# Wells-Group/pmg-dolfinx

Measured on AMD Instinct MI355X. Metric: DoFs/sec per p-MG V-cycle (Poisson, hex, p=4), higher is better.
Workload: dtype f64; 1 GPU; Poisson p=4 V-cycle p=4->2->1, Chebyshev(3)/Jacobi, 64^3 hexes per GPU; fine_dofs_global=16974593, partition=1x1x1 bricks, 1 ghost-cell layer, exchange=none (single rank), rccl_ranks=1, comm_ranks=1

## Files before the change

include/pmg_amd.h:

```cpp
#ifndef PMG_AMD_H
#define PMG_AMD_H

#include <stddef.h>
#include <stdint.h>

#ifdef __cplusplus
extern "C" {
#endif

#define PMG_OK 0
#define PMG_ERR_INVALID -1
#define PMG_ERR_HIP -2
#define PMG_ERR_NUMERIC -3
#define PMG_MAX_DEGREE 8

typedef void* pmg_stream;

typedef struct pmg_layout_s* pmg_layout;
typedef struct pmg_comm_s* pmg_comm;
typedef struct pmg_laplacian_s* pmg_laplacian;
typedef struct pmg_chebyshev_s* pmg_chebyshev;
typedef struct pmg_cg_s* pmg_cg;
typedef struct pmg_interpolator_s* pmg_interpolator;
typedef struct pmg_multigrid_s* pmg_multigrid;
// ... 23 lines not shown
int pmg_layout_create(pmg_layout* out, int32_t size_local, int32_t num_ghosts, int32_t n_send,
                      const int32_t* send_indices, double* send_buffer, int32_t n_recv,
                      const int32_t* recv_indices, double* recv_buffer, pmg_exchange_fn exchange,
                      pmg_allreduce_fn allreduce_sum, void* user);
int pmg_layout_destroy(pmg_layout l);
int32_t pmg_layout_size_local(pmg_layout l);
int32_t pmg_layout_num_ghosts(pmg_layout l);
int pmg_layout_set_allreduce_max(pmg_layout l, pmg_allreduce_fn allreduce_max);

#define PMG_COMM_ID_BYTES 128
int pmg_comm_unique_id(char* id );
int pmg_comm_create(pmg_comm* out, int rank, int nranks, const char* id);
int pmg_comm_destroy(pmg_comm comm);
int pmg_comm_capture_overlaps(void);
int pmg_comm_allgather(pmg_comm comm, const void* send, size_t bytes, void* recv);
int pmg_comm_allreduce_sum(pmg_comm comm, double* values, int n, pmg_stream stream);
int pmg_comm_rank(pmg_comm comm);
int pmg_comm_size(pmg_comm comm);
int pmg_layout_set_comm(pmg_layout l, pmg_comm comm, int32_t n_neighbors, const int32_t* neighbor_ranks,
                        const int32_t* send_counts, const int32_t* recv_counts);

#define PMG_WINDOW_HANDLE_BYTES 64
#define PMG_WINDOW_MAX_NEIGHBORS 64
#define PMG_WINDOW_FLAG_WORDS (4 * PMG_WINDOW_MAX_NEIGHBORS + 8)
#define PMG_WINDOW_ERR_NO_ARRIVAL 1
#define PMG_WINDOW_ERR_SLOT_BUSY 2
int pmg_window_alloc(size_t bytes, void** ptr, char* handle );
int pmg_window_fine_grained(void);
int pmg_window_open(const char* handle, void** ptr);
int pmg_window_close(void* ptr);
int pmg_window_free(void* ptr);
#define PMG_COMM_WINDOW_MAX_RANKS 16
#define PMG_COMM_WINDOW_CHUNK 16384
#define PMG_COMM_WINDOW_BYTES \
  (8 * (2 * PMG_COMM_WINDOW_MAX_RANKS + 8 + 2 * PMG_COMM_WINDOW_MAX_RANKS * PMG_COMM_WINDOW_CHUNK))
int pmg_comm_create_windows(pmg_comm* out, int rank, int nranks, void* const* windows );
int pmg_layout_window_describe(int32_t n_neighbors, const int32_t* send_counts, const int32_t* recv_counts,
                               int64_t* window_doubles, int64_t* fwd_offsets, int64_t* rev_offsets);
int pmg_layout_set_windows(pmg_layout l, int32_t n_neighbors, const int32_t* send_counts, const int32_t* recv_counts,
                           double* window, uint64_t* flags, double* const* nb_window, uint64_t* const* nb_flags,
                           const int64_t* nb_window_doubles, const int64_t* nb_fwd_offset, const int64_t* nb_rev_offset,
                           const int32_t* nb_slot);

int pmg_scatter_fwd_begin(pmg_layout l, const double* x, pmg_stream stream);
long long pmg_layout_forward_scatters(pmg_layout l);
int pmg_scatter_fwd_end(pmg_layout l, double* x, pmg_stream stream);
int pmg_scatter_rev_begin(pmg_layout l, const double* x, pmg_stream stream);
int pmg_scatter_rev_end(pmg_layout l, double* x, pmg_stream stream);

int pmg_vec_set(pmg_layout l, double* x, double value, pmg_stream stream);
int pmg_vec_scale(pmg_layout l, double* x, double alpha, pmg_stream stream);
int pmg_vec_copy(pmg_layout l, double* dst, const double* src, pmg_stream stream);
int pmg_vec_axpy(pmg_layout l, double* r, double alpha, const double* x, const double* y,
                 pmg_stream stream);
int pmg_vec_pointwise_mult(pmg_layout l, double* w, const double* x, const double* y,
                           pmg_stream stream);
int pmg_vec_inner_product(pmg_layout l, const double* a, const double* b, double* result,
                          pmg_stream stream);
int pmg_vec_squared_norm(pmg_layout l, const double* a, double* result, pmg_stream stream);
int pmg_vec_norm(pmg_layout l, const double* a, int norm_type, double* result, pmg_stream stream);

int pmg_laplacian_create(pmg_laplacian* out, pmg_layout layout, int degree, int32_t ncells,
                         const double* kappa, const int32_t* dofmap, const double* xgeom,
                         int32_t npoints, const int32_t* geom_dofmap, const int32_t* lcells,
                         int32_t n_lcells, const int32_t* bcells, int32_t n_bcells,
                         const int8_t* bc_marker, pmg_stream stream);
int pmg_laplacian_create_with_tables(pmg_laplacian* out, pmg_layout layout, int degree,
                                     int32_t ncells, const double* kappa, const int32_t* dofmap,
                                     const double* xgeom, int32_t npoints,
                                     const int32_t* geom_dofmap, const double* dphi_geometry,
                                     const double* G_weights, const int32_t* lcells,
                                     int32_t n_lcells, const int32_t* bcells, int32_t n_bcells,
                                     const int8_t* bc_marker, pmg_stream stream);
int pmg_laplacian_create_ordered(pmg_laplacian* out, pmg_layout layout, int degree, int32_t ncells,
                                 const double* kappa, const int32_t* dofmap, const double* xgeom, int32_t npoints,
                                 const int32_t* geom_dofmap, const double* dphi_geometry, const double* G_weights,
                                 const int32_t* lcells, int32_t n_lcells, const int32_t* bcells, int32_t n_bcells,
                                 const int8_t* bc_marker, int node_order, const int32_t* custom_perm1d,
                                 pmg_stream stream);
int pmg_laplacian_node_order(pmg_laplacian op);
int pmg_laplacian_destroy(pmg_laplacian op);
int pmg_laplacian_apply(pmg_laplacian op, double* in, double* out, pmg_stream stream);
int pmg_laplacian_apply_f32(pmg_laplacian op, float* in, float* out, pmg_stream stream);
int pmg_laplacian_get_diag_inverse(pmg_laplacian op, double* diag_inv, pmg_stream stream);
int pmg_laplacian_set_diag_inverse(pmg_laplacian op, const double* diag_inv, pmg_stream stream);
int pmg_laplacian_compute_diag_inverse(pmg_laplacian op, pmg_stream stream);
int pmg_laplacian_get_geometry(pmg_laplacian op, double* G_out, pmg_stream stream);
int pmg_laplacian_set_coefficient_field(pmg_laplacian op, const double* kq, pmg_stream stream);
int pmg_laplacian_has_coefficient_field(pmg_laplacian op);
int pmg_laplacian_set_coefficient_tensor(pmg_laplacian op, const double* kt, pmg_stream stream);
int pmg_laplacian_has_coefficient_tensor(pmg_laplacian op);
int pmg_laplacian_set_reaction(pmg_laplacian op, const double* sigma, pmg_stream stream);
int pmg_laplacian_has_reaction(pmg_laplacian op);
int pmg_laplacian_assemble_rhs(pmg_laplacian op, const double* f, double* b, pmg_stream stream);
int pmg_laplacian_apply_lifting(pmg_laplacian op, double* g, const double* x0, double alpha, double* b, pmg_stream stream);
int pmg_laplacian_set_bc(pmg_laplacian op, const double* g, const double* x0, double alpha, double* b, pmg_stream stream);
int pmg_laplacian_assemble_neumann(pmg_laplacian op, int32_t nfacets, const int32_t* facet_cells,
                                   const int8_t* facet_local, const double* h, double* b, pmg_stream stream);
int pmg_laplacian_lift_cell_count(pmg_laplacian op);
int pmg_laplacian_degree(pmg_laplacian op);
int pmg_laplacian_is_affine(pmg_laplacian op);
int pmg_laplacian_set_geometry_mode(pmg_laplacian op, int mode);
int pmg_laplacian_set_geometry_batch(pmg_laplacian op, long long batch_cells);
long long pmg_laplacian_geometry_bytes(pmg_laplacian op);
int pmg_laplacian_launches_per_apply(pmg_laplacian op);
int pmg_laplacian_apply_streams(pmg_laplacian op);
int pmg_laplacian_chain_available(pmg_laplacian op);
int pmg_laplacian_chain_form(pmg_laplacian op);
int pmg_laplacian_set_chain_form(pmg_laplacian op, int on);
int pmg_set_merge_threshold(long long patch_dofs);
int pmg_laplacian_time_kernel(pmg_laplacian op, const double* in, double* out, int reps,
                              double* ms_per_launch, pmg_stream stream);

int pmg_laplacian_set_profiling(pmg_laplacian op, int flag);
int pmg_laplacian_read_profile(pmg_laplacian op, double* total_ms, long long* launches);

int pmg_chebyshev_create(pmg_chebyshev* out, pmg_layout layout, double eig_min, double eig_max);
int pmg_chebyshev_destroy(pmg_chebyshev s);
int pmg_chebyshev_set_max_iterations(pmg_chebyshev s, int max_iter);
int pmg_chebyshev_solve(pmg_chebyshev s, pmg_laplacian A, double* x, const double* b,
                        pmg_stream stream);

int pmg_cg_create(pmg_cg* out, pmg_layout layout);
int pmg_cg_destroy(pmg_cg s);
int pmg_cg_set_max_iterations(pmg_cg s, int max_iter);
int pmg_cg_set_tolerance(pmg_cg s, double rtol);
int pmg_cg_store_coefficients(pmg_cg s, int flag);
int pmg_cg_solve(pmg_cg s, pmg_laplacian A, double* x, const double* b, pmg_multigrid precond,
                 int* iterations, pmg_stream stream);
int pmg_cg_set_flexible(pmg_cg s, int flag);
int pmg_cg_coefficients(pmg_cg s, double* alphas, double* betas, int capacity);
int pmg_cg_compute_eigenvalues(pmg_cg s, double* eigs, int capacity);
int pmg_cg_residual(pmg_cg s, double* rnorm);

int pmg_matrix_create_from_laplacian(pmg_matrix* out, pmg_laplacian op, pmg_stream stream);
int pmg_matrix_destroy(pmg_matrix M);
int pmg_matrix_update_values(pmg_matrix M, pmg_stream stream);
int pmg_matrix_apply(pmg_matrix M, const double* in, double* out, pmg_stream stream);
int pmg_matrix_get_diag_inverse(pmg_matrix M, double* diag_inv, pmg_stream stream);
long long pmg_matrix_rows(pmg_matrix M);
long long pmg_matrix_nnz(pmg_matrix M);
long long pmg_matrix_bytes(pmg_matrix M);
int pmg_matrix_frobenius_norm(pmg_matrix M, double* norm);
int pmg_matrix_export(pmg_matrix M, long long* rows, long long* nnz, int32_t* row_ptr, int32_t* cols, double* values);
int pmg_chebyshev_solve_matrix(pmg_chebyshev s, pmg_matrix M, double* x, const double* b, pmg_stream stream);
int pmg_cg_solve_matrix(pmg_cg s, pmg_matrix M, double* x, const double* b, pmg_multigrid precond, int* iterations,
                        pmg_stream stream);

int pmg_interpolator_create(pmg_interpolator* out, pmg_layout layout_coarse,
                            pmg_layout layout_fine, int degree_coarse, int degree_fine,
                            int32_t ncells, const int32_t* dofmap_coarse,
                            const int32_t* dofmap_fine, const int32_t* lcells, int32_t n_lcells,
                            const int32_t* bcells, int32_t n_bcells, pmg_stream stream);
int pmg_interpolator_create_with_operator(pmg_interpolator* out, pmg_layout layout_coarse,
                                          pmg_layout layout_fine, int degree_coarse,
                                          int degree_fine, int32_t ncells,
                                          const int32_t* dofmap_coarse, const int32_t* dofmap_fine,
                                          const int32_t* lcells, int32_t n_lcells,
                                          const int32_t* bcells, int32_t n_bcells,
                                          pmg_laplacian fine_operator, pmg_stream stream);
int pmg_interpolator_create_ordered(pmg_interpolator* out, pmg_layout layout_coarse, pmg_layout layout_fine,
                                    int degree_coarse, int degree_fine, int32_t ncells,
                                    const int32_t* dofmap_coarse, const int32_t* dofmap_fine,
                                    const int32_t* lcells, int32_t n_lcells, const int32_t* bcells,
                                    int32_t n_bcells, pmg_laplacian fine_operator, int node_order,
                                    const int32_t* custom_coarse, const int32_t* custom_fine, pmg_stream stream);
int pmg_interpolator_destroy(pmg_interpolator ip);
int pmg_interpolator_interpolate(pmg_interpolator ip, double* coarse, double* fine,
                                 pmg_stream stream);
int pmg_interpolator_interpolate_add(pmg_interpolator ip, double* coarse, double* fine,
                                     pmg_stream stream);
int pmg_interpolator_reverse_interpolate(pmg_interpolator ip, double* fine, double* coarse,
                                         pmg_stream stream);
int pmg_interpolator_restrict_residual(pmg_interpolator ip, pmg_laplacian op, const double* z, const double* r,
                                       double* coarse, pmg_stream stream);
int pmg_interpolator_interpolate_add_f32(pmg_interpolator ip, const float* coarse, float* fine, pmg_stream stream);
int pmg_interpolator_reverse_interpolate_f32(pmg_interpolator ip, const float* fine, const float* fine_sub,
                                             float* coarse, pmg_stream stream);

int pmg_multigrid_create(pmg_multigrid* out, int nlevels, const pmg_layout* layouts,
                         const int8_t* bc_marker_coarsest);
int pmg_multigrid_destroy(pmg_multigrid mg);
int pmg_multigrid_set_operators(pmg_multigrid mg, const pmg_laplacian* ops);
int pmg_multigrid_set_solvers(pmg_multigrid mg, const pmg_chebyshev* smoothers);
int pmg_multigrid_set_interpolators(pmg_multigrid mg, const pmg_interpolator* interp);
int pmg_multigrid_set_coarse_solver(pmg_multigrid mg, pmg_cg coarse);
typedef int (*pmg_coarse_solve_fn)(void* user, double* x, double* b, pmg_stream stream);
int pmg_multigrid_set_coarse_callback(pmg_multigrid mg, pmg_coarse_solve_fn solve, void* user);
int pmg_amg_create(pmg_amg* out, pmg_laplacian op, pmg_stream stream);
int pmg_amg_create_replicated(pmg_amg* out, pmg_laplacian op, const int64_t* global_index, int64_t n_global,
                              pmg_stream stream);
int pmg_amg_create_distributed(pmg_amg* out, pmg_laplacian op, const int64_t* global_index, int64_t n_global,
                               pmg_stream stream);
int pmg_amg_destroy(pmg_amg amg);
int pmg_amg_set_smoother_iterations(pmg_amg amg, int k);
int pmg_amg_set_cycles(pmg_amg amg, int cycles);
int pmg_amg_set_krylov(pmg_amg amg, int max_iter, double rtol);
int pmg_amg_set_distributed_fine_level(pmg_amg amg, int enable);
int pmg_amg_solve(pmg_amg amg, double* x, const double* b, int* iterations, pmg_stream stream);
int pmg_amg_cycle(pmg_amg amg, double* x, const double* b, pmg_stream stream);
int pmg_amg_num_levels(pmg_amg amg);
int pmg_amg_level_info(pmg_amg amg, int level, long long* rows, long long* nnz, double* lambda_max);
int pmg_amg_export(pmg_amg amg, int level, int which, long long* rows, long long* cols, long long* nnz,
                   int32_t* rowptr, int32_t* colidx, double* values);
int pmg_multigrid_set_coarse_amg(pmg_multigrid mg, pmg_amg amg);

int pmg_multigrid_apply(pmg_multigrid mg, const double* rhs, double* y, double* rnorm,
                        pmg_stream stream);
int pmg_multigrid_set_graph(pmg_multigrid mg, int enable);
long long pmg_multigrid_graph_replays(pmg_multigrid mg);
int pmg_multigrid_apply_counts(pmg_multigrid mg, int* counts, int capacity);
int pmg_multigrid_set_fused_restriction(pmg_multigrid mg, int mode);
int pmg_multigrid_fused_restrictions(pmg_multigrid mg);
#define PMG_PRECISION_FP64 0
#define PMG_PRECISION_FP32 1
int pmg_multigrid_set_precision(pmg_multigrid mg, int precision);
int pmg_multigrid_set_level_matrix(pmg_multigrid mg, int level, pmg_matrix M);
int pmg_multigrid_precision(pmg_multigrid mg);

#ifdef __cplusplus
}
#endif
#endif
```

pmg-dolfinx_amd/_lib.py:

```python
from __future__ import annotations

import ctypes as C
import os

_HERE = os.path.dirname(os.path.abspath(__file__))
LIB_PATH = os.environ.get("PMG_AMD_LIB") or os.path.join(_HERE, "lib", "libpmg_amd.so")

c_dp = C.POINTER(C.c_double)
c_ip = C.POINTER(C.c_int32)
c_bp = C.POINTER(C.c_int8)
c_lp = C.POINTER(C.c_int64)
vp = C.c_void_p

EXCHANGE_FN = C.CFUNCTYPE(C.c_int, vp, C.c_int, vp)
ALLREDUCE_FN = C.CFUNCTYPE(C.c_int, vp, c_dp, C.c_int)
COARSE_FN = C.CFUNCTYPE(C.c_int, vp, vp, vp, vp)


class PmgError(RuntimeError):
    """A pmg_* call returned non-zero; the message is ``pmg_last_error()``."""


_SIGS = {
    "pmg_last_error": (C.c_char_p, []),
# ... 91 lines not shown
    "pmg_set_merge_threshold": (C.c_int, [C.c_longlong]),
    "pmg_laplacian_set_profiling": (C.c_int, [vp, C.c_int]),
    "pmg_laplacian_read_profile": (C.c_int, [vp, c_dp, C.POINTER(C.c_longlong)]),
    "pmg_laplacian_time_kernel": (C.c_int, [vp, vp, vp, C.c_int, c_dp, vp]),
    "pmg_chebyshev_create": (C.c_int, [C.POINTER(vp), vp, C.c_double, C.c_double]),
    "pmg_chebyshev_destroy": (C.c_int, [vp]),
    "pmg_chebyshev_set_max_iterations": (C.c_int, [vp, C.c_int]),
    "pmg_chebyshev_solve": (C.c_int, [vp, vp, vp, vp, vp]),
    "pmg_cg_create": (C.c_int, [C.POINTER(vp), vp]),
    "pmg_cg_destroy": (C.c_int, [vp]),
    "pmg_cg_set_max_iterations": (C.c_int, [vp, C.c_int]),
    "pmg_cg_set_tolerance": (C.c_int, [vp, C.c_double]),
    "pmg_cg_store_coefficients": (C.c_int, [vp, C.c_int]),
    "pmg_cg_set_flexible": (C.c_int, [vp, C.c_int]),
    "pmg_cg_solve": (C.c_int, [vp, vp, vp, vp, vp, C.POINTER(C.c_int), vp]),
    "pmg_cg_coefficients": (C.c_int, [vp, c_dp, c_dp, C.c_int]),
    "pmg_cg_compute_eigenvalues": (C.c_int, [vp, c_dp, C.c_int]),
    "pmg_cg_residual": (C.c_int, [vp, c_dp]),
    "pmg_interpolator_create": (
        C.c_int,
        [C.POINTER(vp), vp, vp, C.c_int, C.c_int, C.c_int32, vp, vp, c_ip, C.c_int32, c_ip, C.c_int32, vp],
    ),
    "pmg_interpolator_create_with_operator": (
        C.c_int,
        [C.POINTER(vp), vp, vp, C.c_int, C.c_int, C.c_int32, vp, vp, c_ip, C.c_int32, c_ip, C.c_int32, vp, vp],
    ),
    "pmg_interpolator_create_ordered": (
        C.c_int,
        [C.POINTER(vp), vp, vp, C.c_int, C.c_int, C.c_int32, vp, vp, c_ip, C.c_int32, c_ip, C.c_int32, vp, C.c_int,
         c_ip, c_ip, vp],
    ),
    "pmg_interpolator_interpolate_add": (C.c_int, [vp, vp, vp, vp]),
    "pmg_interpolator_destroy": (C.c_int, [vp]),
    "pmg_interpolator_interpolate": (C.c_int, [vp, vp, vp, vp]),
    "pmg_interpolator_reverse_interpolate": (C.c_int, [vp, vp, vp, vp]),
    "pmg_interpolator_restrict_residual": (C.c_int, [vp, vp, vp, vp, vp, vp]),
    "pmg_interpolator_interpolate_add_f32": (C.c_int, [vp, vp, vp, vp]),
    "pmg_interpolator_reverse_interpolate_f32": (C.c_int, [vp, vp, vp, vp, vp]),
    "pmg_multigrid_create": (C.c_int, [C.POINTER(vp), C.c_int, C.POINTER(vp), vp]),
    "pmg_multigrid_destroy": (C.c_int, [vp]),
    "pmg_multigrid_set_operators": (C.c_int, [vp, C.POINTER(vp)]),
    "pmg_multigrid_set_solvers": (C.c_int, [vp, C.POINTER(vp)]),
    "pmg_multigrid_set_interpolators": (C.c_int, [vp, C.POINTER(vp)]),
    "pmg_multigrid_set_coarse_solver": (C.c_int, [vp, vp]),
    "pmg_multigrid_set_coarse_callback": (C.c_int, [vp, COARSE_FN, vp]),
    "pmg_multigrid_set_coarse_amg": (C.c_int, [vp, vp]),
    "pmg_multigrid_set_precision": (C.c_int, [vp, C.c_int]),
    "pmg_multigrid_precision": (C.c_int, [vp]),
    "pmg_amg_create": (C.c_int, [C.POINTER(vp), vp, vp]),
    "pmg_amg_create_replicated": (C.c_int, [C.POINTER(vp), vp, C.POINTER(C.c_int64), C.c_int64, vp]),
    "pmg_amg_create_distributed": (C.c_int, [C.POINTER(vp), vp, C.POINTER(C.c_int64), C.c_int64, vp]),
    "pmg_amg_destroy": (C.c_int, [vp]),
    "pmg_amg_set_smoother_iterations": (C.c_int, [vp, C.c_int]),
    "pmg_amg_set_cycles": (C.c_int, [vp, C.c_int]),
    "pmg_amg_set_krylov": (C.c_int, [vp, C.c_int, C.c_double]),
    "pmg_amg_set_distributed_fine_level": (C.c_int, [vp, C.c_int]),
    "pmg_amg_solve": (C.c_int, [vp, vp, vp, C.POINTER(C.c_int), vp]),
    "pmg_amg_cycle": (C.c_int, [vp, vp, vp, vp]),
    "pmg_amg_num_levels": (C.c_int, [vp]),
    "pmg_amg_level_info": (C.c_int, [vp, C.c_int, C.POINTER(C.c_longlong), C.POINTER(C.c_longlong), c_dp]),
    "pmg_amg_export": (C.c_int, [vp, C.c_int, C.c_int, C.POINTER(C.c_longlong), C.POINTER(C.c_longlong),
                                 C.POINTER(C.c_longlong), c_ip, c_ip, c_dp]),
    "pmg_laplacian_set_geometry_batch": (C.c_int, [vp, C.c_longlong]),
    "pmg_laplacian_geometry_bytes": (C.c_longlong, [vp]),
    "pmg_multigrid_apply": (C.c_int, [vp, vp, vp, c_dp, vp]),
    "pmg_multigrid_apply_counts": (C.c_int, [vp, C.POINTER(C.c_int), C.c_int]),
    "pmg_multigrid_set_graph": (C.c_int, [vp, C.c_int]),
    "pmg_multigrid_graph_replays": (C.c_longlong, [vp]),
    "pmg_multigrid_set_fused_restriction": (C.c_int, [vp, C.c_int]),
    "pmg_multigrid_fused_restrictions": (C.c_int, [vp]),
    "pmg_matrix_create_from_laplacian": (C.c_int, [C.POINTER(vp), vp, vp]),
    "pmg_matrix_destroy": (C.c_int, [vp]),
    "pmg_matrix_update_values": (C.c_int, [vp, vp]),
    "pmg_matrix_apply": (C.c_int, [vp, vp, vp, vp]),
    "pmg_matrix_get_diag_inverse": (C.c_int, [vp, vp, vp]),
    "pmg_matrix_rows": (C.c_longlong, [vp]),
    "pmg_matrix_nnz": (C.c_longlong, [vp]),
    "pmg_matrix_bytes": (C.c_longlong, [vp]),
    "pmg_matrix_frobenius_norm": (C.c_int, [vp, c_dp]),
    "pmg_matrix_export": (C.c_int, [vp, C.POINTER(C.c_longlong), C.POINTER(C.c_longlong), c_ip, c_ip, c_dp]),
    "pmg_chebyshev_solve_matrix": (C.c_int, [vp, vp, vp, vp, vp]),
    "pmg_cg_solve_matrix": (C.c_int, [vp, vp, vp, vp, vp, C.POINTER(C.c_int), vp]),
    "pmg_multigrid_set_level_matrix": (C.c_int, [vp, C.c_int, vp]),
}

_COUNT_FUNCS = {"pmg_multigrid_graph_replays", "pmg_amg_num_levels", "pmg_laplacian_geometry_bytes", "pmg_comm_rank", "pmg_comm_size", "pmg_comm_capture_overlaps", "pmg_cg_coefficients", "pmg_cg_compute_eigenvalues", "pmg_multigrid_apply_counts", "pmg_version",
                "pmg_laplacian_degree", "pmg_multigrid_precision", "pmg_laplacian_launches_per_apply", "pmg_laplacian_apply_streams", "pmg_laplacian_is_affine",
                "pmg_laplacian_has_coefficient_field", "pmg_laplacian_has_coefficient_tensor", "pmg_laplacian_has_reaction", "pmg_laplacian_lift_cell_count",
                "pmg_laplacian_chain_available", "pmg_laplacian_chain_form",
                "pmg_laplacian_node_order", "pmg_layout_forward_scatters",
                "pmg_matrix_rows", "pmg_matrix_nnz", "pmg_matrix_bytes", "pmg_multigrid_fused_restrictions"}

_lib = None


def exported_symbols():
    return sorted(_SIGS)


def lib():
    global _lib
    if _lib is None:
        if not os.path.exists(LIB_PATH):
            raise RuntimeError(
                f"{LIB_PATH} is missing: the HIP library has not been built. "
                "Run `python -c 'import __graft_entry__ as g; g.build()'` at the repo root. "
                "There is no CPU fallback."
            )
        import torch

        L = C.CDLL(LIB_PATH)
        for name, (res, args) in _SIGS.items():
            if os.environ.get("PMG_AMD_LIB_ALLOW_MISSING") and not hasattr(L, name):
                continue
            f = getattr(L, name)
            f.restype = res
            f.argtypes = args
        _lib = L
    return _lib


def check(rc: int, what: str = ""):
    if rc != 0:
        msg = lib().pmg_last_error().decode("utf-8", "replace")
        raise PmgError(f"{what}: {msg} (code {rc})" if what else f"{msg} (code {rc})")


def call(name: str, *args):
    rc = getattr(lib(), name)(*args)
    if name in _COUNT_FUNCS:
        if rc < 0:
            check(rc, name)
        return rc
    check(rc, name)
    return rc


def ptr(t):
    if t is None:
        return vp(0)
    if hasattr(t, "data_ptr"):
        return vp(t.data_ptr())
    return vp(t.ctypes.data)


def current_stream():
    import torch

    return vp(torch.cuda.current_stream().cuda_stream)
```

pmg-dolfinx_amd/chebyshev.py:

```python
from __future__ import annotations

import ctypes as C

from . import _lib
from ._lib import call, current_stream, ptr, vp
from .vector import Layout, Vector


class Chebyshev:
    def __init__(self, layout: Layout, eig_range, bs: int = 1):
        self.layout = layout
        self.eig_range = (float(eig_range[0]), float(eig_range[1]))
        h = vp()
        call("pmg_chebyshev_create", C.byref(h), layout.handle, self.eig_range[0], self.eig_range[1])
        self._handle = h

    @property
    def handle(self):
        return self._handle

    def set_max_iterations(self, max_iter: int):
        call("pmg_chebyshev_set_max_iterations", self._handle, int(max_iter))

    def solve(self, A, x: Vector, b: Vector, verbose: bool = False):
        from .matrix import MatrixOperator

        fn = "pmg_chebyshev_solve_matrix" if isinstance(A, MatrixOperator) else "pmg_chebyshev_solve"
        call(fn, self._handle, A.handle, ptr(x.data), ptr(b.data), current_stream())

    def __del__(self):
        try:
            if getattr(self, "_handle", None) is not None:
                _lib.lib().pmg_chebyshev_destroy(self._handle)
                self._handle = None
        except Exception:
            pass
```

pmg-dolfinx_amd/csrc/common.hpp:

```cpp
#pragma once

#include "../../include/pmg_amd.h"

#include <hip/hip_runtime.h>

#include <cstdarg>
#include <cstdio>
#include <functional>
#include <string>
#include <type_traits>
#include <vector>

namespace pmg
{
extern thread_local std::string g_last_error;

int fail(int code, const char* fmt, ...);

#define PMG_HIP(call)                                                                              \
  do                                                                                               \
  {                                                                                                \
    hipError_t e_ = (call);                                                                        \
    if (e_ != hipSuccess)                                                                          \
      return pmg::fail(PMG_ERR_HIP, "%s failed: %s (%s:%d)", #call, hipGetErrorString(e_),         \
// ... 102 lines not shown
  hipStream_t stream = nullptr;
  hipEvent_t ev_in = nullptr, ev_out = nullptr;
  bool reduced_eagerly = false;
};

struct pmg_layout_s
{
  int32_t size_local = 0, num_ghosts = 0, n_send = 0, n_recv = 0;
  pmg_comm_s* comm = nullptr;
  std::vector<int32_t> nb_rank, nb_send, nb_recv;
  hipEvent_t ev_packed = nullptr, ev_arrived = nullptr;
  double *c_send = nullptr, *c_recv = nullptr;
  int32_t *send_pos = nullptr, *recv_pos = nullptr;
  std::vector<size_t> send_off, recv_off;
  pmg_window_s* win = nullptr;
  bool exchange_inline = false;
  bool exchanged_eagerly = false;
  const int32_t* send_idx = nullptr;
  const int32_t* recv_idx = nullptr;
  double* send_buf = nullptr;
  double* recv_buf = nullptr;
  pmg_exchange_fn exchange = nullptr;
  pmg_allreduce_fn allreduce = nullptr;
  pmg_allreduce_fn allreduce_max = nullptr;
  void* user = nullptr;
  double* d_partials = nullptr;
  double* h_result = nullptr;
  long long fwd_scatters = 0;
  bool multi_rank() const { return comm != nullptr || allreduce != nullptr; }
  int32_t total() const { return size_local + num_ghosts; }
};

namespace pmg
{
constexpr int RED_BLOCKS = 1024;
constexpr int RED_THREADS = 256;
constexpr int RED_SLOTS = 8;

int comm_exchange_begin(pmg_layout l, bool reverse, hipStream_t s);
int comm_exchange_end(pmg_layout l, hipStream_t s);
int comm_allreduce(pmg_layout l, double* d_values, int n, bool max, hipStream_t s);
int comm_allreduce(pmg_comm c, double* d_values, int n, bool max, hipStream_t s);
bool comm_capture_ready(pmg_layout l, bool with_allreduce);

int window_exchange_begin(pmg_layout l, bool reverse, const double* x, hipStream_t s);
int window_exchange_end(pmg_layout l, bool reverse, double* x, hipStream_t s);
int window_exchange_whole(pmg_layout l, double* x, hipStream_t s);
int scatter_fwd_whole(pmg_layout l, double* x, hipStream_t s);
bool layout_exchanges_whole(pmg_layout l);
void window_destroy(pmg_layout l);
int wcomm_allreduce(pmg_comm c, double* d_values, int n, bool max, hipStream_t s);
int wcomm_allgather(pmg_comm c, const void* send, size_t bytes, void* recv);
void wcomm_destroy(pmg_comm c);

void range_push(const char* name);
void range_pop();
struct Range
{
  explicit Range(const char* name) { range_push(name); }
  Range(const Range&) = delete;
  Range& operator=(const Range&) = delete;
  ~Range() { range_pop(); }
};

template <typename T>
struct ChebWork
{
  T *r = nullptr, *z = nullptr, *q = nullptr;
};
template <typename T>
using ApplyFnT = std::function<int(T* in, T* out)>;
using ApplyFn = ApplyFnT<double>;
using PrecondFn = std::function<int(double* z, const double* r)>;
int cg_iterate(pmg_cg cg, const ApplyFn& A, const double* dinv, const PrecondFn* M, bool flexible, double* x,
               const double* b, int* iterations, hipStream_t s);
enum : int
{
  ResidualNone = 0,
  ResidualUpdated = 1,
  ResidualSplit = 2,
  ResidualFused = 3
};
template <typename T>
int cheb_iterate(const ChebWork<T>& w, const ApplyFnT<T>& A, const T* dinv, int n, double lmax, int max_iter, T* x,
                 const T* b, int need_r, bool x_zero, hipStream_t s, bool* split = nullptr,
                 const ApplyFnT<T>* A_zeroed = nullptr, int n_total = 0, bool track_ghosts = false,
                 const ApplyFnT<T>* A_first = nullptr);

int dot_async(pmg_layout l, const double* a, const double* b, int slot, hipStream_t s);
double* red_slot(pmg_layout l, int slot);
int reduce_slots_async(pmg_layout l, int slot, int n, bool max, hipStream_t s);
int fetch_slots(pmg_layout l, int slot, int n, double* host_out, hipStream_t s);
int dot_host(pmg_layout l, const double* a, const double* b, double* result, hipStream_t s);
void launch_axpy(int n, double* r, double alpha, const double* x, const double* y, hipStream_t s);
void launch_pointwise(int n, double* w, const double* x, const double* y, hipStream_t s);
void launch_cheb_init(int n, double* r, double* z, const double* b, const double* q, const double* dinv, double c0,
                      hipStream_t s, double* clear_q = nullptr, int n_total = 0);
void launch_cheb_step(int n, double* x, double* r, double* z, const double* q, const double* dinv, double c1, double c2,
                      bool both, int x_final, hipStream_t s, double* clear_q = nullptr, int n_total = 0);
void launch_cheb_first(int n, double* x, double* r, double* z, const double* q, const double* dinv, double c1,
                       double c2, int x_final, hipStream_t s, double* clear_q = nullptr, int n_total = 0);
void launch_cheb_residual(int n, double* r, const double* q, hipStream_t s);
void launch_add(int n, double* x, const double* z, hipStream_t s);
void launch_cheb_last(int n, double* x, double* r, const double* z, const double* q, bool assign, hipStream_t s);
void launch_zero(int n, double* x, hipStream_t s);
void launch_mask_bc(int n, double* b, const int8_t* bc, hipStream_t s);
void launch_cheb_init(int n, float* r, float* z, const float* b, const float* q, const float* dinv, float c0,
                      hipStream_t s, float* clear_q = nullptr, int n_total = 0);
void launch_cheb_step(int n, float* x, float* r, float* z, const float* q, const float* dinv, float c1, float c2,
                      bool both, int x_final, hipStream_t s, float* clear_q = nullptr, int n_total = 0);
void launch_cheb_first(int n, float* x, float* r, float* z, const float* q, const float* dinv, float c1,
                       float c2, int x_final, hipStream_t s, float* clear_q = nullptr, int n_total = 0);
void launch_cheb_residual(int n, float* r, const float* q, hipStream_t s);
void launch_add(int n, float* x, const float* z, hipStream_t s);
void launch_cheb_last(int n, float* x, float* r, const float* z, const float* q, bool assign, hipStream_t s);
void launch_zero(int n, float* x, hipStream_t s);
void launch_mask_bc(int n, float* b, const int8_t* bc, hipStream_t s);
void launch_cg_update(int n, double* x, double* r, double* y, const double* p, const double* dinv,
                      double rnorm, const double* d_py, hipStream_t s);
void launch_cg_update2(int n, double* x, double* r, const double* p, const double* y, double rnorm,
                       const double* d_py, hipStream_t s);
void launch_cg_direction(int n, double* p, const double* y, double rnorm, const double* d_new,
                         const double* d_sub, hipStream_t s);

int laplacian_apply(pmg_laplacian op, double* in, double* out, hipStream_t s);
int laplacian_apply_zeroed(pmg_laplacian op, double* in, double* out, hipStream_t s);
int laplacian_apply_ghosts_current(pmg_laplacian op, double* in, double* out, hipStream_t s);
bool laplacian_wants_zeroed_output(pmg_laplacian op);
const double* laplacian_diag_inv(pmg_laplacian op);
const double* laplacian_reaction(pmg_laplacian op);
pmg_layout laplacian_layout(pmg_laplacian op);
long long laplacian_launches(pmg_laplacian op);
long long laplacian_capture_state(pmg_laplacian op);
int laplacian_geometry_ascending(pmg_laplacian op, double* G_out, hipStream_t s);
struct LaplacianInputs
{
  int degree;
  int32_t ncells;
  const int32_t* dofmap;
  const int8_t* bc;
  const double* kappa;
};
LaplacianInputs laplacian_inputs(pmg_laplacian op);
int interp_prolong(pmg_interpolator ip, double* coarse, double* fine, hipStream_t s);
int interp_restrict(pmg_interpolator ip, double* fine, double* coarse, hipStream_t s);
int interp_prolong_add(pmg_interpolator ip, double* coarse, double* fine, hipStream_t s);
bool interp_is_patched(pmg_interpolator ip);
bool interp_restricts_difference(pmg_interpolator ip);
int interp_restrict_difference(pmg_interpolator ip, double* fine, const double* fine_sub, double* coarse,
                               hipStream_t s);
bool interp_fuses_residual(pmg_interpolator ip, pmg_laplacian op);
int interp_restrict_residual(pmg_interpolator ip, pmg_laplacian op, const double* z, const double* r, double* coarse,
                             hipStream_t s);
int amg_solve(pmg_amg amg, double* x, const double* b, hipStream_t s);
pmg_layout amg_layout(pmg_amg amg);
long long amg_capture_state(pmg_amg amg);
int matrix_apply(pmg_matrix M, const double* in, double* out, hipStream_t s);
const double* matrix_diag_inv(pmg_matrix M);
pmg_layout matrix_layout(pmg_matrix M);

int laplacian_f32_supported(pmg_laplacian op, const char* who);
int laplacian_f32_prepare(pmg_laplacian op, hipStream_t s);
int laplacian_f32_reaction(pmg_laplacian op, hipStream_t s);
int laplacian_f32_refresh(pmg_laplacian op, hipStream_t s);
int laplacian_f32_diag(pmg_laplacian op, const float** d, hipStream_t s, bool* changed);
long long laplacian_diag_version(pmg_laplacian op);
int laplacian_apply_f32(pmg_laplacian op, const float* in, float* out, hipStream_t s);
int transfer_f32_prepare(pmg_interpolator ip, const float** M1);
int prolong_add_f32(pmg_interpolator ip, const float* M1, const float* coarse, float* fine, hipStream_t s);
int restrict_f32(pmg_interpolator ip, const float* M1, const float* fine, const float* fine_sub, float* coarse,
                 hipStream_t s);
void launch_to_f32(int n, const double* in, const double* sub, float* out, hipStream_t s);
void launch_from_f32(int n, const float* in, double* out, bool add, hipStream_t s);
}
```

pmg-dolfinx_amd/csrc/laplacian.hip:

```cpp
#include "laplacian.hpp"
#include "stiffness_layer.hpp"

#include <algorithm>
#include <cmath>
#include <cstdlib>
#include <type_traits>

using namespace pmg;


namespace
{
#include "geometry_kernels.hpp"
#include "stiffness_column.hpp"
#include "stiffness_chain.hpp"
#include "stiffness_restrict.hpp"

__global__ void zero_list_kernel(int n, const int32_t* __restrict__ idx, double* __restrict__ y)
{
  for (int i = blockIdx.x * blockDim.x + threadIdx.x; i < n; i += gridDim.x * blockDim.x)
    y[idx[i]] = 0.0;
}

const double2* batch_geometry(pmg_laplacian op, int first, int count, hipStream_t s)
{
  double2* base = op->G - (size_t)first * gpatch(op->nd, op->K);
  const long long nslots = (long long)count * op->K, n = nslots * op->N;
  if (n > 0)
    geometry_kernel<<<(unsigned)((n + 255) / 256), 256, 0, s>>>((long long)first * op->K, nslots, op->nd, op->K,
                                                              op->pcell, op->xgeom, op->geom_dofmap,
                                                              op->dphi_geom, op->gweights, op->kfield, op->dofmap,
                                                              op->ktensor, base);
  return base;
}

template <typename F>
int for_each_geometry_chunk(pmg_laplacian op, hipStream_t s, F f)
{
  if (op->npatch == 0)
    return PMG_OK;
  if (op->batch_patches <= 0)
    f(0, op->npatch, op->G);
  else
    for (int first = 0; first < op->npatch; first += op->batch_patches)
    {
      const int count = std::min(op->batch_patches, op->npatch - first);
      f(first, count, batch_geometry(op, first, count, s));
    }
  PMG_HIP(hipGetLastError());
  return PMG_OK;
}

template <int P, bool AFFINE_NT, typename F>
void apply_variant(pmg_laplacian op, F launch)
{
  if (op->geometry_mode == 1)
    launch(std::true_type{}, std::bool_constant<AFFINE_NT>{});
  else if (P >= NT_FROM && op->stream_policy)
    launch(std::false_type{}, std::true_type{});
  else
    launch(std::false_type{}, std::false_type{});
}

template <int P>
int launch_stiffness(pmg_laplacian op, const double* x, double* y, int first, int count,
                     int atomic_out, hipStream_t s)
{
  if (count <= 0)
    return PMG_OK;
  if (op->batch_patches > 0 && op->geometry_mode == 0 && count > op->batch_patches)
  {
    for (int f = first; f < first + count; f += op->batch_patches)
      PMG_TRY(launch_stiffness<P>(op, x, y, f, std::min(op->batch_patches, first + count - f), atomic_out, s));
    return PMG_OK;
  }
  const double2* G = op->G;
  if (op->batch_patches > 0 && op->geometry_mode == 0)
    G = batch_geometry(op, first, count, s);
  apply_variant<P, (P >= NT_FROM)>(op, [&](auto aff, auto nt) {
    constexpr bool AFF = decltype(aff)::value, NT = decltype(nt)::value;
    stiffness_column_kernel<P, AFF, NT><<<count, Shape<P>::WTHREADS, 0, s>>>(
        x, y, G, op->Gaff, op->W1, op->poff, op->pdofs, op->lmap_id, op->lmaps, op->pcell, op->pncell, op->kappa, op->D,
        op->react, first, atomic_out);
  });
  op->launches++;
  return PMG_OK;
}

static int launch_chains(pmg_laplacian op, const double* x, double* y, int first, int count, hipStream_t s)
{
  if constexpr (chain_form(4))
  {
    if (op->P != 4)
      return fail(PMG_ERR_INVALID, "internal: chain form at degree %d", op->P);
    auto launch = [&](auto nt) {
      stiffness_chain_kernel<4, decltype(nt)::value><<<count, ChainShape<4>::THREADS, 0, s>>>(
          x, y, op->G, op->poff, op->cdofs, op->ccar, op->lmap_id, op->lmaps, op->pcell, op->pncell, op->kappa, op->D,
          op->chain_off, op->chain_patch, first);
    };
    op->stream_policy ? launch(std::true_type{}) : launch(std::false_type{});
    op->launches++;
  }
  return PMG_OK;
}

ApplyForm apply_form(pmg_laplacian op)
{
  const bool resident = op->batch_patches == 0;
  return {resident && !op->launch_stream.empty(),
          resident && op->chain_on && op->geometry_mode == 0 && !op->react, resident};
}

int run_launches(pmg_laplacian op, const double* x, double* y, int l0, int l1, hipStream_t s)
{
  return walk_launches(op, l0, l1, apply_form(op), s, [&](const LaunchStep& st, hipStream_t sl) {
    if (st.kind == LaunchStep::CHAINS)
      return launch_chains(op, x, y, st.first, st.count, sl);
    return with_degree(op->P, [&](auto P) {
      return launch_stiffness<decltype(P)::value>(op, x, y, st.first, st.count, st.atomic_out, sl);
    });
  });
}

#define PMG_FOR_FUSED_PAIRS(X) X(2, 1) X(4, 2) X(3, 1) X(6, 3)

template <int P, int PC>
int launch_stiffness_restrict(pmg_laplacian op, const TransferView& tv, const double* z, const double* r,
                              double* coarse, hipStream_t s)
{
  constexpr int cm = RestrictShape<P, PC>::CM;
  PMG_REQUIRE(tv.cmax_m <= cm, "internal: a patch holds %d coarse dofs, the fused kernel %d", tv.cmax_m, cm);
  const RestrictLists R{tv.cpoff, tv.clmap_id, tv.cpdofs, tv.clmaps, tv.pmult, tv.M1};
  apply_variant<P, false>(op, [&](auto aff, auto nt) {
    constexpr bool AFF = decltype(aff)::value, NT = decltype(nt)::value;
    stiffness_restrict_kernel<P, PC, AFF, NT><<<op->npatch, Shape<P>::WTHREADS, 0, s>>>(
        z, r, coarse, op->G, op->Gaff, op->W1, op->poff, op->pdofs, op->lmap_id, op->lmaps, op->pcell, op->pncell,
        op->kappa, op->D, op->react, R);
  });
  PMG_HIP(hipGetLastError());
  return PMG_OK;
}

}

namespace pmg
{
bool streams_past_the_cache(long long tensor_bytes)
{
  if (const char* e = std::getenv("PMG_STREAM_POLICY"))
    return e[0] != '0';
  return tensor_bytes > (128LL << 20);
}

bool laplacian_fuses_restriction(pmg_laplacian op, int coarse_degree)
{
  if (op->layout->num_ghosts != 0 || op->batch_patches != 0)
    return false;
#define X(F, C)                                                                                                      \
  if (op->P == F && coarse_degree == C)                                                                              \
    return true;
  PMG_FOR_FUSED_PAIRS(X)
#undef X
  return false;
}

int laplacian_apply_restrict(pmg_laplacian op, const TransferView& tv, const double* z, const double* r,
                             double* coarse, hipStream_t s)
{
  PMG_REQUIRE(laplacian_fuses_restriction(op, tv.ndc - 1) && tv.ndf == op->nd && tv.fv.pdofs == op->pdofs
// ... 26 lines not shown
  const long long field = op->batch_patches > 0 ? (op->kfield_epoch & 0x3fff) << 44 : 0;
  return ((long long)op->geometry_mode << 40) ^ ((long long)op->batch_patches << 8) ^ (long long)(op->have_diag ? 1 : 0)
         ^ (long long)(op->chain_on ? 2 : 0) ^ (long long)(op->react ? 4 : 0) ^ field;
}

PatchView laplacian_patches(pmg_laplacian op)
{
  PatchView v;
  v.P = op->P;
  v.K = op->K;
  v.N = op->N;
  v.npatch = op->npatch;
  v.max_m = op->max_m;
  v.pcell_h = &op->pcell_h;
  v.pncell_h = &op->pncell_h;
  v.launch_first = &op->launch_first;
  v.launch_count = &op->launch_count;
  v.n_launch_l = op->n_launch_l;
  v.merged = op->n_plain == 0;
  v.pcell = op->pcell;
  v.pncell = op->pncell;
  v.poff = op->poff;
  v.pdofs = op->pdofs;
  v.lmap_id = op->lmap_id;
  v.lmaps = op->lmaps;
  v.npdofs = op->npdofs;
  return v;
}

bool laplacian_wants_zeroed_output(pmg_laplacian op)
{
  return zero_fills_output(op->needs_zero, op->launch_first.size(), op->n_bzero, op->layout->total());
}

bool laplacian_single_launch(pmg_laplacian op)
{
  if (op->launch_first.size() != 2)
    return false;
  int steps = 0, all = 0;
  for_each_launch_step(*op, op->chain_first, op->chain_count, 0, 2, apply_form(op), [&](const LaunchStep& st) {
    steps += st.launches();
    all += st.kind == LaunchStep::PATCHES && st.atomic_out && st.count == op->npatch;
    return PMG_OK;
  });
  return steps == 1 && all == 1 && layout_exchanges_whole(op->layout);
}

static int apply_impl(pmg_laplacian op, double* in, double* out, bool out_is_zero, hipStream_t s,
                      bool exchange = true)
{
  pmg_layout l = op->layout;
  const int nl = (int)op->launch_first.size();
  const bool zero_all = laplacian_wants_zeroed_output(op);
  if (zero_all && !out_is_zero)
    launch_zero(l->total(), out, s);
  if (op->n_bzero > 0 && !zero_all)
    zero_list_kernel<<<(op->n_bzero + 255) / 256 > 1024 ? 1024 : (op->n_bzero + 255) / 256, 256, 0, s>>>(
        op->n_bzero, op->bzero, out);
  if (laplacian_single_launch(op))
  {
    if (exchange)
      PMG_TRY(scatter_fwd_whole(l, in, s));
    PMG_TRY(run_launches(op, in, out, 0, nl, s));
    op->applies++;
    return PMG_OK;
  }
  if (exchange)
    PMG_TRY(pmg_scatter_fwd_begin(l, in, (pmg_stream)s));
  PMG_TRY(run_launches(op, in, out, 0, op->n_launch_l, s));
  if (exchange)
    PMG_TRY(pmg_scatter_fwd_end(l, in, (pmg_stream)s));
  PMG_TRY(run_launches(op, in, out, op->n_launch_l, nl, s));
  op->applies++;
  return PMG_OK;
}
int laplacian_apply(pmg_laplacian op, double* in, double* out, hipStream_t s) { return apply_impl(op, in, out, false, s); }
int laplacian_apply_ghosts_current(pmg_laplacian op, double* in, double* out, hipStream_t s)
{
  return apply_impl(op, in, out, false, s, false);
}
int laplacian_apply_zeroed(pmg_laplacian op, double* in, double* out, hipStream_t s)
{
  return apply_impl(op, in, out, laplacian_wants_zeroed_output(op), s);
}
}

extern "C" int pmg_laplacian_create_ordered(
    pmg_laplacian* out, pmg_layout layout, int degree, int32_t ncells, const double* kappa,
    const int32_t* dofmap, const double* xgeom, int32_t npoints, const int32_t* geom_dofmap,
    const double* dphi_geometry, const double* G_weights, const int32_t* lcells, int32_t n_lcells,
    const int32_t* bcells, int32_t n_bcells, const int8_t* bc_marker, int node_order, const int32_t* custom_perm1d,
    pmg_stream stream)
{
  PMG_REQUIRE(out && layout, "pmg_laplacian_create: NULL handle");
  if (degree < 1 || degree > PMG_MAX_DEGREE)
    return fail(PMG_ERR_INVALID, "Unsupported degree");
  PMG_REQUIRE(ncells >= 0 && n_lcells >= 0 && n_bcells >= 0 && n_lcells + n_bcells <= ncells,
              "pmg_laplacian_create: cell lists (%d + %d) exceed ncells (%d)", n_lcells, n_bcells,
              ncells);
  PMG_REQUIRE(ncells == 0 || (kappa && dofmap && xgeom && geom_dofmap && bc_marker),
              "pmg_laplacian_create: NULL array");
  PMG_REQUIRE((n_lcells == 0 || lcells) && (n_bcells == 0 || bcells),
              "pmg_laplacian_create: NULL cell list");
  PMG_REQUIRE(npoints >= 0, "pmg_laplacian_create: negative npoints");
  {
    std::vector<char> seen(ncells, 0);
    for (int set = 0; set < 2; ++set)
    {
      const int32_t* list = set ? bcells : lcells;
      const int n = set ? n_bcells : n_lcells;
      for (int i = 0; i < n; ++i)
      {
        PMG_REQUIRE(list[i] >= 0 && list[i] < ncells,
                    "pmg_laplacian_create: cell list entry %d out of range", list[i]);
        PMG_REQUIRE(!seen[list[i]], "pmg_laplacian_create: cell %d listed twice", list[i]);
        seen[list[i]] = 1;
      }
    }
  }

  hipStream_t s = S(stream);
  auto* op = new pmg_laplacian_s;
  HandleGuard<pmg_laplacian> guard(op, pmg_laplacian_destroy);
  op->layout = layout;
  op->P = degree;
  op->nd = degree + 1;
  op->N = op->nd * op->nd * op->nd;
  op->K = patch_shape(degree).K();
  {
    const int kk[9] = {0, Shape<1>::K, Shape<2>::K, Shape<3>::K, Shape<4>::K, Shape<5>::K,
                       Shape<6>::K, Shape<7>::K, Shape<8>::K};
    PMG_REQUIRE(kk[degree] == op->K, "internal: patch shape / kernel shape mismatch");
  }
  op->ncells = ncells;
  op->npoints = npoints;
  op->kappa = kappa;
  op->dofmap = dofmap;
  op->xgeom = xgeom;
  op->geom_dofmap = geom_dofmap;
  op->bc = bc_marker;
  const int nd = op->nd, N = op->N;
  const int total = layout->total();

  std::vector<int32_t> perm1d;
  PMG_TRY(node_permutation(node_order, degree, custom_perm1d, perm1d));
  op->node_order = node_order;
  if (!is_identity(perm1d))
  {
    const std::vector<int32_t> p3 = cell_permutation(nd, perm1d);
    PMG_TRY(upload(&op->qperm, p3.data(), p3.size(), s));
    PMG_HIP(hipMalloc(&op->dofmap_own, sizeof(int32_t) * ((size_t)ncells * N ? (size_t)ncells * N : 1)));
    PMG_TRY(permute_rows_i32(ncells, N, op->qperm, dofmap, op->dofmap_own, s));
    PMG_HIP(hipStreamSynchronize(s));
    op->dofmap = dofmap = op->dofmap_own;
  }

  std::vector<double> pts(nd), wts(nd), D(nd * nd);
  gll_table(nd, pts.data(), wts.data());
  lagrange_derivative_table(nd, pts.data(), D.data());
  PMG_TRY(upload(&op->D, D.data(), D.size(), s));

  if (dphi_geometry && G_weights)
  {
    PMG_HIP(hipMalloc(&op->dphi_geom, sizeof(double) * 24 * N));
    PMG_HIP(hipMalloc(&op->gweights, sizeof(double) * N));
    if (op->qperm)
// ... 23 lines not shown
            for (int j = 0; j < 2; ++j)
              for (int k = 0; k < 2; ++k)
              {
                int v = i * 4 + j * 2 + k;
                dphi[((size_t)0 * N + q) * 8 + v] = dp[i] * ph[1][j] * ph[2][k];
                dphi[((size_t)1 * N + q) * 8 + v] = ph[0][i] * dp[j] * ph[2][k];
                dphi[((size_t)2 * N + q) * 8 + v] = ph[0][i] * ph[1][j] * dp[k];
              }
        }
    PMG_TRY(upload(&op->dphi_geom, dphi.data(), dphi.size(), s));
    PMG_TRY(upload(&op->gweights, w3.data(), w3.size(), s));
    PMG_HIP(hipStreamSynchronize(s));
  }

  PatchPlan plan;
  ChainPlan cplan;
  {
    std::vector<int32_t> h_dofmap((size_t)ncells * N), h_gd((size_t)ncells * 8);
    std::vector<int8_t> h_bc(total);
    std::vector<double> h_x((size_t)npoints * 3);
    PMG_HIP(hipMemcpyAsync(h_dofmap.data(), dofmap, sizeof(int32_t) * h_dofmap.size(),
                           hipMemcpyDeviceToHost, s));
    PMG_HIP(hipMemcpyAsync(h_gd.data(), geom_dofmap, sizeof(int32_t) * h_gd.size(),
                           hipMemcpyDeviceToHost, s));
    PMG_HIP(hipMemcpyAsync(h_bc.data(), bc_marker, sizeof(int8_t) * h_bc.size(),
                           hipMemcpyDeviceToHost, s));
    PMG_HIP(hipMemcpyAsync(h_x.data(), xgeom, sizeof(double) * h_x.size(), hipMemcpyDeviceToHost, s));
    PMG_HIP(hipStreamSynchronize(s));
    std::vector<float> centroid((size_t)ncells * 3);
    for (int32_t c = 0; c < ncells; ++c)
      for (int a = 0; a < 3; ++a)
      {
        double v = 0;
        for (int k = 0; k < 8; ++k)
        {
          int32_t g = h_gd[(size_t)c * 8 + k];
          PMG_REQUIRE(g >= 0 && g < npoints, "pmg_laplacian_create: geometry dofmap entry %d out of range", g);
          v += h_x[3 * (size_t)g + a];
        }
        centroid[(size_t)c * 3 + a] = (float)(v * 0.125);
      }
    PMG_TRY(build_patch_plan(plan, degree, ncells, h_dofmap.data(), h_bc.data(), total,
                             centroid.data(), lcells, n_lcells, bcells, n_bcells));
    op->all_affine = (n_lcells + n_bcells) > 0;
    for (int set = 0; set < 2 && op->all_affine; ++set)
    {
      const int32_t* list = set ? bcells : lcells;
      const int n = set ? n_bcells : n_lcells;
      for (int i = 0; i < n && op->all_affine; ++i)
      {
        const int32_t* gd = h_gd.data() + (size_t)list[i] * 8;
        const double* v[8];
        for (int k = 0; k < 8; ++k)
          v[k] = h_x.data() + 3 * (size_t)gd[k];
        double diam = 0, dev = 0;
        for (int a = 0; a < 3; ++a)
        {
          const double e1 = v[4][a] - v[0][a], e2 = v[2][a] - v[0][a], e3 = v[1][a] - v[0][a];
          diam += std::fabs(e1) + std::fabs(e2) + std::fabs(e3);
          dev += std::fabs(v[3][a] - (v[0][a] + e2 + e3)) + std::fabs(v[5][a] - (v[0][a] + e1 + e3))
                 + std::fabs(v[6][a] - (v[0][a] + e1 + e2)) + std::fabs(v[7][a] - (v[0][a] + e1 + e2 + e3));
        }
        if (dev > 1e-12 * diam)
          op->all_affine = false;
      }
    }
    if (chain_form(degree) && (unsigned long long)plan.npatch * (unsigned long long)gpatch(nd, op->K) < (1ull << 32))
    {
      const char* e = std::getenv("PMG_CHAIN");
      const int mode = e ? std::atoi(e) : 0;
      if (mode > 0)
      {
        int dev = 0, cus = 256;
        if (hipGetDevice(&dev) == hipSuccess)
          (void)hipDeviceGetAttribute(&cus, hipDeviceAttributeMultiprocessorCount, dev);
        PMG_TRY(build_chain_plan(cplan, plan, total, h_bc.data(), centroid.data(), mode >= 2 ? 1 : (cus * 3) / 4));
      }
    }
    std::vector<char> touched(total, 0);
    for (uint32_t v : plan.pdofs)
      touched[v & PD_MASK] = 1;
    for (int i = 0; i < total && !op->needs_zero; ++i)
      op->needs_zero = !touched[i];
  }
  op->npatch = plan.npatch;
  op->pcell_h = plan.pcell;
  op->pncell_h = plan.pncell;
  op->npdofs = (long long)plan.pdofs.size();
  op->max_m = plan.max_M;
  op->launch_first = plan.launch_first;
  op->launch_count = plan.launch_count;
  op->n_launch_l = plan.n_launch_l;
  op->n_plain = plan.n_plain;
  op->launch_stream = plan.launch_stream;
  op->launch_signal = plan.launch_signal;
  op->launch_wait = plan.launch_wait;
  if (!op->launch_stream.empty())
  {
    PMG_HIP(hipStreamCreateWithFlags(&op->stream2, hipStreamNonBlocking));
    PMG_HIP(hipEventCreateWithFlags(&op->ev_fork, hipEventDisableTiming));
    PMG_HIP(hipEventCreateWithFlags(&op->ev_order, hipEventDisableTiming));
    PMG_HIP(hipEventCreateWithFlags(&op->ev_join, hipEventDisableTiming));
  }
  PMG_TRY(upload(&op->pcell, plan.pcell.data(), plan.pcell.size(), s));
  PMG_TRY(upload(&op->pncell, plan.pncell.data(), plan.pncell.size(), s));
  op->n_bzero = (int32_t)plan.bzero.size();
  PMG_TRY(upload(&op->bzero, plan.bzero.data(), plan.bzero.size(), s));
  PMG_TRY(upload(&op->poff, plan.poff.data(), plan.poff.size(), s));
  PMG_TRY(upload(&op->pdofs, plan.pdofs.data(), plan.pdofs.size(), s));
  PMG_TRY(upload(&op->lmap_id, plan.lmap_id.data(), plan.lmap_id.size(), s));
  PMG_TRY(upload(&op->lmaps, plan.lmaps.data(), plan.lmaps.size(), s));
  if (cplan.ok)
  {
    PMG_TRY(upload(&op->cdofs, cplan.cdofs.data(), cplan.cdofs.size(), s));
    PMG_TRY(upload(&op->ccar, cplan.ccar.data(), cplan.ccar.size(), s));
    PMG_TRY(upload(&op->chain_off, cplan.chain_off.data(), cplan.chain_off.size(), s));
    PMG_TRY(upload(&op->chain_patch, cplan.chain_patch.data(), cplan.chain_patch.size(), s));
    op->chain_first = cplan.launch_first;
    op->chain_count = cplan.launch_count;
    op->chain_ok = op->chain_on = true;
  }

  const long long nslots = (long long)plan.npatch * op->K;
  const long long nq_total = nslots * N;
  PMG_TRY(upload(&op->W1, wts.data(), wts.size(), s));
  PMG_HIP(hipMalloc(&op->Gaff, sizeof(double) * 6 * (nslots ? nslots : 1)));
  if (nslots > 0)
    affine_geometry_kernel<<<(unsigned)((nslots + 255) / 256), 256, 0, s>>>(nslots, op->pcell, xgeom,
                                                                           geom_dofmap, nullptr, op->Gaff);
  {
    const size_t gsize = (size_t)op->npatch * gpatch(nd, op->K);
    PMG_HIP(hipMalloc(&op->G, sizeof(double2) * (gsize ? gsize : 1)));
    PMG_HIP(hipMemsetAsync(op->G, 0, sizeof(double2) * (gsize ? gsize : 1), s));
  }
  op->stream_policy = streams_past_the_cache((long long)sizeof(double2) * gpatch(nd, op->K) * op->npatch);
  PMG_HIP(hipMalloc(&op->diag_inv, sizeof(double) * (total ? total : 1)));
  PMG_HIP(hipEventCreate(&op->ev0));
  PMG_HIP(hipEventCreate(&op->ev1));
  if (nq_total > 0)
  {
    batch_geometry(op, 0, op->npatch, s);
    PMG_HIP(hipGetLastError());
  }
  PMG_HIP(hipStreamSynchronize(s));
  *out = guard.release();
  return PMG_OK;
}

extern "C" int pmg_laplacian_create_with_tables(
    pmg_laplacian* out, pmg_layout layout, int degree, int32_t ncells, const double* kappa,
    const int32_t* dofmap, const double* xgeom, int32_t npoints, const int32_t* geom_dofmap,
    const double* dphi_geometry, const double* G_weights, const int32_t* lcells, int32_t n_lcells,
    const int32_t* bcells, int32_t n_bcells, const int8_t* bc_marker, pmg_stream stream)
{
  return pmg_laplacian_create_ordered(out, layout, degree, ncells, kappa, dofmap, xgeom, npoints, geom_dofmap,
                                      dphi_geometry, G_weights, lcells, n_lcells, bcells, n_bcells, bc_marker,
                                      PMG_NODES_ASCENDING, nullptr, stream);
}

extern "C" int pmg_laplacian_node_order(pmg_laplacian op) { return op ? op->node_order : -1; }

extern "C" int pmg_laplacian_create(pmg_laplacian* out, pmg_layout layout, int degree,
                                    int32_t ncells, const double* kappa, const int32_t* dofmap,
                                    const double* xgeom, int32_t npoints,
                                    const int32_t* geom_dofmap, const int32_t* lcells,
                                    int32_t n_lcells, const int32_t* bcells, int32_t n_bcells,
                                    const int8_t* bc_marker, pmg_stream stream)
{
  return pmg_laplacian_create_with_tables(out, layout, degree, ncells, kappa, dofmap, xgeom,
                                          npoints, geom_dofmap, nullptr, nullptr, lcells, n_lcells,
                                          bcells, n_bcells, bc_marker, stream);
}

extern "C" int pmg_laplacian_destroy(pmg_laplacian op)
{
  if (!op)
    return PMG_OK;
  (void)hipFree(op->G);
  (void)hipFree(op->dofmap_own);
  (void)hipFree(op->qperm);
  (void)hipFree(op->D);
  (void)hipFree(op->Gaff);
  (void)hipFree(op->kfield);
  (void)hipFree(op->ktensor);
  (void)hipFree(op->react_buf);
  (void)hipFree(op->react32_buf);
  (void)hipFree(op->W1);
  (void)hipFree(op->dphi_geom);
  (void)hipFree(op->gweights);
  (void)hipFree(op->pcell);
  (void)hipFree(op->pncell);
  (void)hipFree(op->bzero);
  (void)hipFree(op->poff);
  (void)hipFree(op->pdofs);
  (void)hipFree(op->lmap_id);
  (void)hipFree(op->lmaps);
  (void)hipFree(op->cdofs);
  (void)hipFree(op->ccar);
  (void)hipFree(op->chain_off);
  (void)hipFree(op->chain_patch);
  (void)hipFree(op->diag_inv);
  (void)hipFree(op->G32);
  (void)hipFree(op->D32);
  (void)hipFree(op->diag32);
  (void)hipFree(op->lift_cells);
  for (hipEvent_t e : op->prof_events)
    (void)hipEventDestroy(e);
  for (hipEvent_t e : {op->ev_fork, op->ev_order, op->ev_join})
    if (e)
      (void)hipEventDestroy(e);
  if (op->stream2)
    (void)hipStreamDestroy(op->stream2);
  if (op->ev0)
    (void)hipEventDestroy(op->ev0);
  if (op->ev1)
    (void)hipEventDestroy(op->ev1);
  delete op;
  return PMG_OK;
}

#ifdef PMG_STAMPS
extern "C" int pmg_debug_set_stamp_buffer(unsigned long long* buffer, int workgroups)
{
  PMG_HIP(hipMemcpyToSymbol(HIP_SYMBOL(g_stamp_buffer), &buffer, sizeof(buffer)));
  PMG_HIP(hipMemcpyToSymbol(HIP_SYMBOL(g_stamp_capacity), &workgroups, sizeof(workgroups)));
  return PMG_OK;
}
#endif

extern "C" int pmg_laplacian_degree(pmg_laplacian op) { return op ? op->P : -1; }

extern "C" int pmg_laplacian_is_affine(pmg_laplacian op) { return op ? (op->all_affine ? 1 : 0) : -1; }

extern "C" int pmg_laplacian_set_geometry_mode(pmg_laplacian op, int mode)
{
  PMG_REQUIRE(op && (mode == 0 || mode == 1), "pmg_laplacian_set_geometry_mode: bad argument");
  if (mode == 1)
  {
    PMG_REQUIRE(op->all_affine, "pmg_laplacian_set_geometry_mode: the mesh has non-affine cells");
    PMG_REQUIRE(!op->kfield, "pmg_laplacian_set_geometry_mode: the affine mode streams one tensor per cell and cannot "
                             "carry the coefficient field (remove it with pmg_laplacian_set_coefficient_field(op, "
                             "NULL, stream) first)");
  }
  op->geometry_mode = mode;
  return PMG_OK;
}

extern "C" int pmg_laplacian_apply(pmg_laplacian op, double* in, double* out, pmg_stream stream)
{
  PMG_REQUIRE(op && in && out, "pmg_laplacian_apply: NULL argument");
  PMG_REQUIRE(in != out, "pmg_laplacian_apply: in and out alias");
  return laplacian_apply(op, in, out, S(stream));
}

extern "C" int pmg_laplacian_get_diag_inverse(pmg_laplacian op, double* diag_inv,
                                              pmg_stream stream)
{
  PMG_REQUIRE(op && diag_inv, "pmg_laplacian_get_diag_inverse: NULL argument");
  PMG_REQUIRE(op->have_diag, "pmg_laplacian_get_diag_inverse: diagonal not set");
  PMG_HIP(hipMemcpyAsync(diag_inv, op->diag_inv, sizeof(double) * op->layout->total(),
                         hipMemcpyDeviceToDevice, S(stream)));
  return PMG_OK;
}

extern "C" int pmg_laplacian_set_diag_inverse(pmg_laplacian op, const double* diag_inv,
                                              pmg_stream stream)
{
  PMG_REQUIRE(op && diag_inv, "pmg_laplacian_set_diag_inverse: NULL argument");
  PMG_HIP(hipMemcpyAsync(op->diag_inv, diag_inv, sizeof(double) * op->layout->total(),
                         hipMemcpyDeviceToDevice, S(stream)));
  op->have_diag = true;
  op->diag_computed = false;
  op->diag_version++;
  return PMG_OK;
}

extern "C" int pmg_laplacian_compute_diag_inverse(pmg_laplacian op, pmg_stream stream)
{
  PMG_REQUIRE(op, "pmg_laplacian_compute_diag_inverse: NULL argument");
  hipStream_t s = S(stream);
  const int total = op->layout->total();
  PMG_HIP(hipMemsetAsync(op->diag_inv, 0, sizeof(double) * total, s));
  PMG_TRY(for_each_geometry_chunk(op, s, [&](int first, int count, const double2* G) {
    const long long nslots = (long long)count * op->K, n = nslots * op->N;
    diagonal_kernel<<<(unsigned)((n + 255) / 256), 256, 0, s>>>((long long)first * op->K, nslots, op->nd, op->K,
                                                              op->pcell, G, op->dofmap, op->bc, op->kappa, op->D,
                                                              op->diag_inv);
  }));
  if (total > 0)
    diag_invert_kernel<<<(total + 255) / 256, 256, 0, s>>>(total, op->bc, op->react, op->diag_inv);
  PMG_HIP(hipGetLastError());
  op->have_diag = true;
  op->diag_computed = true;
  op->diag_version++;
  return PMG_OK;
}

__global__ void coefficient_check_kernel(int n, const double* __restrict__ kq, double* __restrict__ bad)
{
  int mine = 0;
  for (long long i = (long long)blockIdx.x * blockDim.x + threadIdx.x; i < n; i += (long long)gridDim.x * blockDim.x)
  {
    const double v = kq[i];
    mine += !(v > 0.0 && v <= 1.79769313486231570e308);
  }
  if (mine)
    atomicAdd(bad, (double)mine);
}

extern "C" int pmg_laplacian_has_coefficient_field(pmg_laplacian op) { return op ? (op->kfield ? 1 : 0) : -1; }

extern "C" int pmg_laplacian_set_coefficient_field(pmg_laplacian op, const double* kq, pmg_stream stream)
{
  PMG_REQUIRE(op, "pmg_laplacian_set_coefficient_field: NULL argument");
  hipStream_t s = S(stream);
  hipStreamCaptureStatus cap = hipStreamCaptureStatusNone;
  PMG_HIP(hipStreamIsCapturing(s, &cap));
  PMG_REQUIRE(cap == hipStreamCaptureStatusNone,
              "pmg_laplacian_set_coefficient_field: not inside a stream capture (it allocates and synchronises)");
  pmg_layout l = op->layout;
  double* released = nullptr;
  if (!kq)
  {
    if (!op->kfield)
      return PMG_OK;
    released = op->kfield;
    op->kfield = nullptr;
    op->kfield_epoch++;
  }
  else
  {
    PMG_REQUIRE(op->geometry_mode == 0,
                "pmg_laplacian_set_coefficient_field: the affine mode streams one tensor per cell and cannot carry a "
                "field (return to the stored tensor with pmg_laplacian_set_geometry_mode(op, 0) first)");
    double* bad = red_slot(l, 0);
// ... 333 lines not shown
```

pmg-dolfinx_amd/csrc/laplacian.hpp:

```cpp
#pragma once

#include "common.hpp"
#include "patches.hpp"

struct pmg_laplacian_s
{
  pmg_layout layout = nullptr;
  int P = 0, nd = 0, N = 0, K = 0;
  int32_t ncells = 0, npoints = 0;
  const double* kappa = nullptr;
  const int32_t* dofmap = nullptr;
  const double* xgeom = nullptr;
  const int32_t* geom_dofmap = nullptr;
  const int8_t* bc = nullptr;
  int node_order = PMG_NODES_ASCENDING;
  int32_t* dofmap_own = nullptr;
  int32_t* qperm = nullptr;
  double2* G = nullptr;
  double* kfield = nullptr;
  long long kfield_epoch = 0;
  double* ktensor = nullptr;
  double* react = nullptr;
  float* react32 = nullptr;
  double* react_buf = nullptr;
  float* react32_buf = nullptr;
  bool diag_computed = false;
  double* Gaff = nullptr;
  double* W1 = nullptr;
  bool all_affine = false;
  int geometry_mode = 0;
  double* D = nullptr;
  double* dphi_geom = nullptr;
  double* gweights = nullptr;
  int32_t* pcell = nullptr;
  int32_t* pncell = nullptr;
  int32_t* bzero = nullptr;
  int32_t n_bzero = 0;
  int32_t* poff = nullptr;
  uint32_t* pdofs = nullptr;
  int32_t* lmap_id = nullptr;
  uint16_t* lmaps = nullptr;
  int32_t npatch = 0;
  std::vector<int32_t> launch_first, launch_count;
  std::vector<int8_t> launch_stream;
  int launch_signal = -1, launch_wait = -1;
  hipStream_t stream2 = nullptr;
  hipEvent_t ev_fork = nullptr, ev_order = nullptr, ev_join = nullptr;
  std::vector<int32_t> pcell_h, pncell_h;
  long long npdofs = 0;
  int max_m = 0;
  int n_launch_l = 0;
  int n_plain = 0;
  bool needs_zero = false;
  bool chain_ok = false, chain_on = false;
  uint32_t* cdofs = nullptr;
  uint32_t* ccar = nullptr;
  int32_t* chain_off = nullptr;
  int32_t* chain_patch = nullptr;
  std::vector<int32_t> chain_first, chain_count;
  bool stream_policy = true;
  bool stream_policy32 = false;
  double* diag_inv = nullptr;
  bool have_diag = false;
  hipEvent_t ev0 = nullptr, ev1 = nullptr;
  long long launches = 0;
  long long applies = 0;
  int32_t batch_patches = 0;
  bool profiling = false;
  std::vector<hipEvent_t> prof_events;
  size_t prof_used = 0;
  long long prof_launches = 0;
  float2* G32 = nullptr;
  float* D32 = nullptr;
  float* diag32 = nullptr;
  long long diag_version = 0;
  long long diag32_version = -1;
  int32_t* lift_cells = nullptr;
  int32_t n_lift = -1;
  std::vector<char> listed;
};

namespace pmg
{
bool streams_past_the_cache(long long tensor_bytes);

template <typename L>
int walk_launches(pmg_laplacian op, int l0, int l1, ApplyForm form, hipStream_t s, L&& launch)
{
  const bool prof = op->profiling && l1 > l0;
  if (prof)
  {
    while (op->prof_events.size() < op->prof_used + 2)
    {
      hipEvent_t e;
      PMG_HIP(hipEventCreate(&e));
      op->prof_events.push_back(e);
    }
    PMG_HIP(hipEventRecord(op->prof_events[op->prof_used], s));
  }
  int issued = 0;
  PMG_TRY(for_each_launch_step(*op, op->chain_first, op->chain_count, l0, l1, form, [&](const LaunchStep& st) -> int {
    switch (st.kind)
    {
    case LaunchStep::FORK:
      PMG_HIP(hipEventRecord(op->ev_fork, s));
      PMG_HIP(hipStreamWaitEvent(op->stream2, op->ev_fork, 0));
      break;
    case LaunchStep::WAIT_ORDER:
      PMG_HIP(hipStreamWaitEvent(s, op->ev_order, 0));
      break;
    case LaunchStep::RECORD_ORDER:
      PMG_HIP(hipEventRecord(op->ev_order, op->stream2));
      break;
    case LaunchStep::JOIN:
      PMG_HIP(hipEventRecord(op->ev_join, op->stream2));
      PMG_HIP(hipStreamWaitEvent(s, op->ev_join, 0));
      break;
    default:
      PMG_TRY(launch(st, st.stream ? op->stream2 : s));
      ++issued;
    }
    return PMG_OK;
  }));
  PMG_HIP(hipGetLastError());
  if (prof)
  {
    PMG_HIP(hipEventRecord(op->prof_events[op->prof_used + 1], s));
    op->prof_used += 2;
    op->prof_launches += issued;
  }
  return PMG_OK;
}

__device__ inline void jacobian(const double* __restrict__ xgeom,
                                const int32_t* __restrict__ gdofs, const double* __restrict__ dphi,
                                int nq, int q, double K[3][3], double& detJ)
{
  double J[3][3] = {{0, 0, 0}, {0, 0, 0}, {0, 0, 0}};
  for (int k = 0; k < 8; ++k)
  {
    const double* xk = xgeom + 3 * (size_t)gdofs[k];
    double x0 = xk[0], x1 = xk[1], x2 = xk[2];
// ... 43 lines not shown
```

pmg-dolfinx_amd/csrc/solvers.hip:

```cpp
#include "common.hpp"

#include <cstdlib>

#include <algorithm>
#include <cmath>
#include <cstring>

using namespace pmg;

struct pmg_chebyshev_s
{
  pmg_layout layout = nullptr;
  double eig_min = 0, eig_max = 1;
  int max_iter = 1;
  double *r = nullptr, *z = nullptr, *q = nullptr;
};

struct pmg_cg_s
{
  pmg_layout layout = nullptr;
  int max_iter = 0;
  double rtol = 0;
  bool store = false;
  double *r = nullptr, *y = nullptr, *p = nullptr;
  double* zold = nullptr;
  bool flexible = false;
  std::vector<double> alphas, betas, residuals;
};

struct pmg_multigrid_s
{
  int L = 0;
  std::vector<pmg_layout> layouts;
  const int8_t* bc0 = nullptr;
  std::vector<pmg_laplacian> ops;
  std::vector<pmg_chebyshev> smoothers;
  std::vector<pmg_interpolator> interps;
  std::vector<double*> u, b;
  std::vector<int> counts;
  pmg_cg coarse = nullptr;
  pmg_coarse_solve_fn coarse_fn = nullptr;
  void* coarse_user = nullptr;
  pmg_amg coarse_amg = nullptr;
  std::vector<pmg_matrix> mats;
  std::vector<long long> mat_applies;
  struct GraphEntry
  {
    const double* rhs;
    double* y;
    bool y_zero;
    uint64_t config;
    hipGraphExec_t exec;
    std::vector<int> counts;
    int fused_count;
  };
  int graph_mode = -1;
  std::vector<GraphEntry> graphs;
  hipStream_t capture_stream = nullptr;
  long long graph_replays = 0;
  int fused_mode = -1;
  int fused_count = 0;
  int precision = PMG_PRECISION_FP64;
  std::vector<float*> u32, b32;
  std::vector<ChebWork<float>> w32;
  std::vector<const float*> dinv32;
  std::vector<const float*> M1_32;
};

namespace pmg
{
template <typename T>
int cheb_iterate(const ChebWork<T>& w, const ApplyFnT<T>& A, const T* dinv, int n, double lmax, int max_iter, T* x,
                 const T* b, int need_r, bool x_zero, hipStream_t s, bool* split, const ApplyFnT<T>* A_zeroed,
                 int n_total, bool track_ghosts, const ApplyFnT<T>* A_first)
{
  PMG_REQUIRE(sizeof(T) == 8 || !A_zeroed, "cheb_iterate: the FP32 passes have no zeroed-output form");
  if (split)
    *split = false;
  T* const clear_q = A_zeroed ? w.q : nullptr;
  const ApplyFnT<T>& An = A_zeroed ? *A_zeroed : A;
  const T c0 = (T)(4.0 / (3.0 * lmax));
  const int ng = track_ghosts && n_total > n ? n_total - n : 0;
  if (x_zero)
  {
    launch_cheb_init(n, w.r, w.z, b, nullptr, dinv, c0, s, clear_q, n_total);
    if (ng > 0)
      launch_zero(ng, x + n, s);
  }
  else
  {
    PMG_TRY(A_first ? (*A_first)(x, w.q) : A(x, w.q));
    launch_cheb_init(n, w.r, w.z, b, w.q, dinv, c0, s, clear_q, n_total);
  }
  for (int i = 1; i <= max_iter; ++i)
  {
    const bool last = (i == max_iter);
    if (last && !need_r)
    {
      if (max_iter == 1)
      {
        if (x_zero)
          PMG_HIP(hipMemcpyAsync(x, w.z, sizeof(T) * n, hipMemcpyDeviceToDevice, s));
        else
          launch_add(n, x, w.z, s);
      }
      break;
    }
    if (last && need_r == ResidualFused && split && max_iter > 1)
    {
      *split = true;
      break;
    }
    PMG_TRY(An(w.z, w.q));
    if (ng > 0)
      launch_add(ng, x + n, w.z + n, s);
    if (last)
    {
      if (max_iter == 1)
        launch_cheb_last(n, x, w.r, w.z, w.q, x_zero, s);
      else if (need_r == ResidualSplit && split)
        *split = true;
      else
        launch_cheb_residual(n, w.r, w.q, s);
      break;
    }
    const T c1 = (T)((2.0 * i - 1.0) / (2.0 * i + 3.0));
    const T c2 = (T)((8.0 * i + 4.0) / (2.0 * i + 3.0) / lmax);
    const int x_final = (i + 1 == max_iter) ? (need_r == ResidualNone ? 2 : 1) : 0;
    if (x_zero && i == 1)
      launch_cheb_first(n, x, w.r, w.z, w.q, dinv, c1, c2, x_final, s, clear_q, n_total);
    else
      launch_cheb_step(n, x, w.r, w.z, w.q, dinv, c1, c2, i == 1, x_final, s, clear_q, n_total);
  }
  if (max_iter == 0 && x_zero)
    launch_zero(n, x, s);
  PMG_HIP(hipGetLastError());
  return PMG_OK;
}
template int cheb_iterate<double>(const ChebWork<double>&, const ApplyFnT<double>&, const double*, int, double, int,
                                  double*, const double*, int, bool, hipStream_t, bool*, const ApplyFnT<double>*, int,
                                  bool, const ApplyFnT<double>*);
template int cheb_iterate<float>(const ChebWork<float>&, const ApplyFnT<float>&, const float*, int, double, int, float*,
                                 const float*, int, bool, hipStream_t, bool*, const ApplyFnT<float>*, int, bool,
                                 const ApplyFnT<float>*);
}

namespace
{
int mg_apply_graph(pmg_multigrid mg, const double* rhs, double* y, bool y_zero, hipStream_t s, bool* done);
bool use_graph(pmg_multigrid mg);
void drop_graphs(pmg_multigrid mg);

template <typename T>
int alloc_vec(pmg_layout l, T** p)
{
  size_t n = l->total() ? l->total() : 1;
  PMG_HIP(hipMalloc(p, sizeof(T) * n));
  PMG_HIP(hipMemset(*p, 0, sizeof(T) * n));
  PMG_HIP(hipStreamSynchronize(nullptr));
  return PMG_OK;
}

int cheb_solve(pmg_chebyshev sm, pmg_laplacian A, double* x, const double* b, int need_r,
               bool x_zero, hipStream_t s, bool* split = nullptr, bool track_ghosts = false,
               bool x_ghosts_current = false)
{
  pmg_layout l = sm->layout;
  PMG_REQUIRE(laplacian_layout(A) == l, "Chebyshev: operator and smoother layouts differ");
  const ChebWork<double> w{sm->r, sm->z, sm->q};
  const ApplyFn apply = [A, s](double* in, double* out) { return laplacian_apply(A, in, out, s); };
  const ApplyFn apply_zeroed = [A, s](double* in, double* out) { return laplacian_apply_zeroed(A, in, out, s); };
  const ApplyFn apply_local = [A, s](double* in, double* out) { return laplacian_apply_ghosts_current(A, in, out, s); };
  return cheb_iterate(w, apply, laplacian_diag_inv(A), l->size_local, sm->eig_max, sm->max_iter, x, b, need_r, x_zero,
                      s, split, laplacian_wants_zeroed_output(A) ? &apply_zeroed : nullptr, l->total(), track_ghosts,
                      x_ghosts_current ? &apply_local : nullptr);
}

int cheb_solve_matrix(pmg_chebyshev sm, pmg_matrix M, double* x, const double* b, int need_r, bool x_zero,
                      hipStream_t s, bool* split = nullptr, long long* applies = nullptr)
{
  pmg_layout l = sm->layout;
  PMG_REQUIRE(matrix_layout(M) == l, "Chebyshev: matrix and smoother layouts differ");
  const ChebWork<double> w{sm->r, sm->z, sm->q};
  const ApplyFn apply = [M, s, applies](double* in, double* out)
  {
    if (applies)
      ++*applies;
    return matrix_apply(M, in, out, s);
  };
  return cheb_iterate(w, apply, matrix_diag_inv(M), l->size_local, sm->eig_max, sm->max_iter, x, b, need_r, x_zero, s,
                      split);
}

bool fuses_restriction(pmg_multigrid mg, int i)
{
  if (mg->fused_mode == 0 || i <= 0 || mg->mats[i] || !interp_fuses_residual(mg->interps[i - 1], mg->ops[i]))
    return false;
  if (const char* e = std::getenv("PMG_FUSED_DEGREES"))
  {
    const int P = pmg_laplacian_degree(mg->ops[i]);
    for (const char* c = e; *c; ++c)
      if (*c - '0' == P)
        return true;
    return false;
  }
  return true;
}

int level_smooth(pmg_multigrid mg, int i, double* x, const double* b, int need_r, bool x_zero, hipStream_t s,
                 bool* split = nullptr, bool track_ghosts = false, bool x_ghosts_current = false)
{
  if (mg->mats[i])
    return cheb_solve_matrix(mg->smoothers[i], mg->mats[i], x, b, need_r, x_zero, s, split, &mg->mat_applies[i]);
  return cheb_solve(mg->smoothers[i], mg->ops[i], x, b, need_r, x_zero, s, split, track_ghosts, x_ghosts_current);
}

long long level_applies(pmg_multigrid mg, int i) { return laplacian_launches(mg->ops[i]) + mg->mat_applies[i]; }

bool local_correction(pmg_multigrid mg, int level)
{
  if (const char* e = std::getenv("PMG_LOCAL_CORRECTION"))
    if (e[0] == '0')
      return false;
  return level > 0 && mg->layouts[level]->num_ghosts > 0 && interp_is_patched(mg->interps[level - 1]);
}

int mg_check_f32(pmg_multigrid mg, const char* who)
{
  for (int i = 0; i < mg->L; ++i)
  {
    pmg_layout l = mg->layouts[i];
    PMG_REQUIRE(l->num_ghosts == 0 && !l->multi_rank() && !l->win,
                "%s: the FP32 cycle is single-domain only (level %d's layout has ghosts or a communicator)", who, i);
  }
  for (size_t i = 0; i < mg->interps.size(); ++i)
    PMG_REQUIRE(interp_is_patched(mg->interps[i]),
                "%s: the FP32 cycle needs patch-form interpolators (pmg_interpolator_create_with_operator; level %zu)",
                who, i);
  for (pmg_laplacian op : mg->ops)
    PMG_TRY(laplacian_f32_supported(op, who));
  return PMG_OK;
}

void free_f32(pmg_multigrid mg)
{
  for (float* p : mg->u32)
    (void)hipFree(p);
  for (float* p : mg->b32)
    (void)hipFree(p);
  for (const ChebWork<float>& w : mg->w32)
  {
    (void)hipFree(w.r);
    (void)hipFree(w.z);
    (void)hipFree(w.q);
  }
  mg->u32.clear();
  mg->b32.clear();
  mg->w32.clear();
}

int mg_prepare_f32(pmg_multigrid mg, hipStream_t s)
{
  const int L = mg->L;
  PMG_TRY(mg_check_f32(mg, "pmg_multigrid_apply"));
  if ((int)mg->u32.size() != L)
  {
    mg->u32.assign(L, nullptr);
    mg->b32.assign(L, nullptr);
    mg->w32.assign(L, ChebWork<float>{});
    for (int i = 0; i < L; ++i)
    {
      PMG_TRY(alloc_vec(mg->layouts[i], &mg->u32[i]));
      PMG_TRY(alloc_vec(mg->layouts[i], &mg->b32[i]));
      PMG_TRY(alloc_vec(mg->layouts[i], &mg->w32[i].r));
      PMG_TRY(alloc_vec(mg->layouts[i], &mg->w32[i].z));
      PMG_TRY(alloc_vec(mg->layouts[i], &mg->w32[i].q));
    }
  }
  mg->M1_32.assign(L - 1, nullptr);
  for (int i = 0; i < L - 1; ++i)
    PMG_TRY(transfer_f32_prepare(mg->interps[i], &mg->M1_32[i]));
  mg->dinv32.assign(L, nullptr);
  for (int i = 0; i < L; ++i)
  {
    PMG_TRY(laplacian_f32_prepare(mg->ops[i], s));
    PMG_TRY(laplacian_f32_diag(mg->ops[i], &mg->dinv32[i], s, nullptr));
  }
  return PMG_OK;
}

int level_smooth_f32(pmg_multigrid mg, int i, int need_r, bool x_zero, hipStream_t s, bool* split)
{
  pmg_laplacian op = mg->ops[i];
  const ApplyFnT<float> apply = [op, s](float* in, float* out) { return laplacian_apply_f32(op, in, out, s); };
  return cheb_iterate(mg->w32[i], apply, mg->dinv32[i], mg->layouts[i]->size_local, mg->smoothers[i]->eig_max,
                      mg->smoothers[i]->max_iter, mg->u32[i], mg->b32[i], need_r, x_zero, s, split);
}
// ... 110 lines not shown
    }
    else if (split)
      PMG_TRY(interp_restrict_difference(mg->interps[i - 1], mg->smoothers[i]->r, mg->smoothers[i]->q,
                                         mg->b[i - 1], s));
    else
      PMG_TRY(interp_restrict(mg->interps[i - 1], mg->smoothers[i]->r, mg->b[i - 1], s));
  }
  if (L > 1)
    launch_mask_bc(mg->layouts[0]->size_local, mg->b[0], mg->bc0, s);
  {
    Range rg("pmg:coarse_solve");
    const double* b0 = (L == 1) ? rhs : mg->b[0];
    const bool zero = (L == 1) ? y_zero : true;
    if (has_coarse_solver(mg) && L > 1)
      PMG_TRY(coarse_solve(mg, s));
    else
      PMG_TRY(level_smooth(mg, 0, mg->u[0], b0, ResidualNone, zero, s));
  }
  for (int i = 0; i < L - 1; ++i)
  {
    {
      Range rg("pmg:prolong");
      if (interp_is_patched(mg->interps[i]))
        PMG_TRY(interp_prolong_add(mg->interps[i], mg->u[i], mg->u[i + 1], s));
      else
      {
        double* du = mg->smoothers[i + 1]->q;
        PMG_TRY(interp_prolong(mg->interps[i], mg->u[i], du, s));
        launch_add(mg->layouts[i + 1]->size_local, mg->u[i + 1], du, s);
      }
    }
    Range rg("pmg:post_smooth");
    const double* bi = (i + 1 == L - 1) ? rhs : mg->b[i + 1];
    PMG_TRY(level_smooth(mg, i + 1, mg->u[i + 1], bi, ResidualNone, false, s, nullptr, false,
                         local_correction(mg, i + 1)));
  }
  for (int i = 0; i < L; ++i)
    mg->counts[i] = (int)(level_applies(mg, i) - before[i]);
  PMG_HIP(hipGetLastError());
  return PMG_OK;
}
}

extern "C" int pmg_chebyshev_create(pmg_chebyshev* out, pmg_layout layout, double eig_min,
                                    double eig_max)
{
  PMG_REQUIRE(out && layout, "pmg_chebyshev_create: NULL argument");
  PMG_REQUIRE(eig_max > 0.0, "pmg_chebyshev_create: eig_max must be positive");
  auto* sm = new pmg_chebyshev_s;
  HandleGuard<pmg_chebyshev> guard(sm, pmg_chebyshev_destroy);
  sm->layout = layout;
  sm->eig_min = eig_min;
  sm->eig_max = eig_max;
  PMG_TRY(alloc_vec(layout, &sm->r));
  PMG_TRY(alloc_vec(layout, &sm->z));
  PMG_TRY(alloc_vec(layout, &sm->q));
  *out = guard.release();
  return PMG_OK;
}

extern "C" int pmg_chebyshev_destroy(pmg_chebyshev sm)
{
  if (!sm)
    return PMG_OK;
  (void)hipFree(sm->r);
  (void)hipFree(sm->z);
  (void)hipFree(sm->q);
  delete sm;
  return PMG_OK;
}

extern "C" int pmg_chebyshev_set_max_iterations(pmg_chebyshev sm, int max_iter)
{
  PMG_REQUIRE(sm && max_iter >= 0, "pmg_chebyshev_set_max_iterations: bad argument");
  sm->max_iter = max_iter;
  return PMG_OK;
}

extern "C" int pmg_chebyshev_solve(pmg_chebyshev sm, pmg_laplacian A, double* x, const double* b,
                                   pmg_stream stream)
{
  PMG_REQUIRE(sm && A && x && b, "pmg_chebyshev_solve: NULL argument");
  return cheb_solve(sm, A, x, b, ResidualNone, false, S(stream));
}

extern "C" int pmg_chebyshev_solve_matrix(pmg_chebyshev sm, pmg_matrix M, double* x, const double* b,
                                          pmg_stream stream)
{
  PMG_REQUIRE(sm && M && x && b, "pmg_chebyshev_solve_matrix: NULL argument");
  return cheb_solve_matrix(sm, M, x, b, ResidualNone, false, S(stream));
}

extern "C" int pmg_cg_create(pmg_cg* out, pmg_layout layout)
{
  PMG_REQUIRE(out && layout, "pmg_cg_create: NULL argument");
  auto* cg = new pmg_cg_s;
  HandleGuard<pmg_cg> guard(cg, pmg_cg_destroy);
  cg->layout = layout;
  PMG_TRY(alloc_vec(layout, &cg->r));
  PMG_TRY(alloc_vec(layout, &cg->y));
  PMG_TRY(alloc_vec(layout, &cg->p));
  *out = guard.release();
  return PMG_OK;
}

extern "C" int pmg_cg_destroy(pmg_cg cg)
{
  if (!cg)
    return PMG_OK;
  (void)hipFree(cg->r);
  (void)hipFree(cg->y);
  (void)hipFree(cg->p);
  (void)hipFree(cg->zold);
  delete cg;
  return PMG_OK;
}

extern "C" int pmg_cg_set_max_iterations(pmg_cg cg, int max_iter)
{
  PMG_REQUIRE(cg && max_iter >= 0, "pmg_cg_set_max_iterations: bad argument");
  cg->max_iter = max_iter;
  cg->alphas.reserve(max_iter);
  cg->betas.reserve(max_iter);
  cg->residuals.reserve(max_iter);
  return PMG_OK;
}

extern "C" int pmg_cg_set_tolerance(pmg_cg cg, double rtol)
{
  PMG_REQUIRE(cg, "pmg_cg_set_tolerance: NULL argument");
  cg->rtol = rtol;
  return PMG_OK;
}

extern "C" int pmg_cg_store_coefficients(pmg_cg cg, int flag)
{
  PMG_REQUIRE(cg, "pmg_cg_store_coefficients: NULL argument");
  cg->store = flag != 0;
  return PMG_OK;
}

namespace pmg
{
int cg_iterate(pmg_cg cg, const ApplyFn& A, const double* dinv, const PrecondFn* M, bool flexible, double* x,
               const double* b, int* iterations, hipStream_t s)
{
  pmg_layout l = cg->layout;
  const int n = l->size_local;
  double *r = cg->r, *y = cg->y, *p = cg->p;
  const bool precond = M != nullptr;
  auto precondition = [&](double* out_z, const double* in_r) -> int
  {
    if (precond)
      return (*M)(out_z, in_r);
    launch_pointwise(n, out_z, in_r, dinv, s);
    return PMG_OK;
  };
  const bool flex = flexible && precond;
  if (flex && !cg->zold)
    PMG_TRY(alloc_vec(l, &cg->zold));
  PMG_TRY(A(x, y));
  launch_axpy(n, r, -1.0, y, b, s);
  PMG_TRY(precondition(p, r));
  if (flex)
    PMG_HIP(hipMemcpyAsync(cg->zold, p, sizeof(double) * n, hipMemcpyDeviceToDevice, s));
  double rnorm0;
// ... 248 lines not shown
  mg->smoothers.assign(smoothers, smoothers + mg->L);
  return PMG_OK;
}

extern "C" int pmg_multigrid_set_interpolators(pmg_multigrid mg, const pmg_interpolator* interp)
{
  PMG_REQUIRE(mg && (interp || mg->L == 1), "pmg_multigrid_set_interpolators: NULL argument");
  drop_graphs(mg);
  mg->interps.clear();
  for (int i = 0; i < mg->L - 1; ++i)
  {
    PMG_REQUIRE(interp[i], "pmg_multigrid_set_interpolators: level %d is NULL", i);
    mg->interps.push_back(interp[i]);
  }
  return PMG_OK;
}

namespace
{
void drop_graphs(pmg_multigrid mg)
{
  for (auto& g : mg->graphs)
    (void)hipGraphExecDestroy(g.exec);
  mg->graphs.clear();
}

bool use_graph(pmg_multigrid mg)
{
  if (mg->graph_mode >= 0)
    return mg->graph_mode == 1;
  const char* e = std::getenv("PMG_GRAPH_AUTO");
  if (e && e[0] == '0')
    return false;
  const bool rccl_too = e && std::string(e) == "rccl";
  bool several = false;
  for (int i = 0; i < mg->L; ++i)
  {
    pmg_layout l = mg->layouts[i];
    if (!l->multi_rank() && !l->win)
      continue;
    several = true;
    if (l->exchange && !l->comm && !l->win)
      return false;
    if (!l->win && !rccl_too)
      return false;
    if (mg->coarse_amg && i == 0 && l->comm && !l->comm->wcomm && !rccl_too)
      return false;
  }
  return several;
}

long long capture_config(pmg_multigrid mg)
{
  uint64_t h = 1469598103934665603ull;
  auto mix = [&h](uint64_t v) { h = (h ^ v) * 1099511628211ull; };
  for (int i = 0; i < mg->L; ++i)
  {
    pmg_layout l = mg->layouts[i];
    if (l->exchange && !l->comm && !l->win)
      return -1;
    if (!comm_capture_ready(l, i == 0 && mg->coarse_amg != nullptr))
      return -1;
    const long long st = laplacian_capture_state(mg->ops[i]);
    if (st < 0)
      return -1;
    mix((uint64_t)st);
    mix((uint64_t)(uintptr_t)mg->ops[i]);
    mix((uint64_t)(uintptr_t)mg->smoothers[i]);
    mix((uint64_t)(uintptr_t)mg->mats[i]);
    mix((uint64_t)(uintptr_t)l->comm);
    mix((uint64_t)(uintptr_t)l->win);
    if (i + 1 < mg->L)
      mix((uint64_t)(uintptr_t)mg->interps[i]);
    mix((uint64_t)mg->smoothers[i]->max_iter);
    uint64_t bits;
    static_assert(sizeof(bits) == sizeof(double), "");
    memcpy(&bits, &mg->smoothers[i]->eig_max, sizeof(bits));
    mix(bits);
  }
  if (mg->coarse || mg->coarse_fn)
    return -1;
  mix((uint64_t)mg->precision);
  mix((uint64_t)(mg->fused_mode + 1));
  if (mg->precision == PMG_PRECISION_FP32)
    for (int i = 0; i < mg->L; ++i)
      mix((uint64_t)laplacian_diag_version(mg->ops[i]));
  if (mg->coarse_amg)
  {
    const long long st = amg_capture_state(mg->coarse_amg);
    if (st < 0)
      return -1;
    mix((uint64_t)st);
    mix((uint64_t)(uintptr_t)mg->coarse_amg);
  }
  return (long long)(h >> 1);
}

int mg_apply_graph(pmg_multigrid mg, const double* rhs, double* y, bool y_zero, hipStream_t s, bool* done)
{
  *done = false;
  if ((int)mg->ops.size() != mg->L || (int)mg->smoothers.size() != mg->L || (int)mg->interps.size() != mg->L - 1)
    return PMG_OK;
  const long long cfg = capture_config(mg);
  if (cfg < 0)
    return PMG_OK;
  for (auto& g : mg->graphs)
    if (g.rhs == rhs && g.y == y && g.y_zero == y_zero && g.config == (uint64_t)cfg)
    {
      PMG_HIP(hipGraphLaunch(g.exec, s));
      mg->counts = g.counts;
      mg->fused_count = g.fused_count;
      mg->graph_replays++;
      *done = true;
      return PMG_OK;
    }
  if (mg->precision == PMG_PRECISION_FP32)
    PMG_TRY(mg_prepare_f32(mg, s));
  if (!mg->capture_stream)
    PMG_HIP(hipStreamCreateWithFlags(&mg->capture_stream, hipStreamNonBlocking));
  PMG_HIP(hipStreamBeginCapture(mg->capture_stream, hipStreamCaptureModeRelaxed));
  const int rc = mg_apply(mg, rhs, y, y_zero, mg->capture_stream);
  hipGraph_t graph = nullptr;
  const hipError_t e = hipStreamEndCapture(mg->capture_stream, &graph);
  if (rc != PMG_OK)
  {
    if (graph)
      (void)hipGraphDestroy(graph);
    return rc;
  }
  if (e != hipSuccess || !graph)
    return fail(PMG_ERR_HIP, "capturing the V-cycle failed: %s", hipGetErrorString(e));
  pmg_multigrid_s::GraphEntry g{rhs, y, y_zero, (uint64_t)cfg, nullptr, mg->counts, mg->fused_count};
  const hipError_t ei = hipGraphInstantiate(&g.exec, graph, nullptr, nullptr, 0);
  (void)hipGraphDestroy(graph);
  if (ei != hipSuccess)
    return fail(PMG_ERR_HIP, "instantiating the V-cycle graph failed: %s", hipGetErrorString(ei));
  if (mg->graphs.size() >= 16)
    drop_graphs(mg);
  mg->graphs.push_back(g);
  PMG_HIP(hipGraphLaunch(g.exec, s));
  mg->graph_replays++;
  *done = true;
  return PMG_OK;
}
}

extern "C" int pmg_multigrid_set_graph(pmg_multigrid mg, int enable)
{
  PMG_REQUIRE(mg, "pmg_multigrid_set_graph: NULL argument");
  drop_graphs(mg);
  mg->graph_mode = enable < 0 ? -1 : (enable != 0 ? 1 : 0);
  return PMG_OK;
}

extern "C" int pmg_multigrid_set_fused_restriction(pmg_multigrid mg, int mode)
{
  PMG_REQUIRE(mg, "pmg_multigrid_set_fused_restriction: NULL argument");
  PMG_REQUIRE(mode == -1 || mode == 0, "pmg_multigrid_set_fused_restriction: mode %d (-1 automatic, 0 never)", mode);
  drop_graphs(mg);
  mg->fused_mode = mode;
  return PMG_OK;
}

extern "C" int pmg_multigrid_fused_restrictions(pmg_multigrid mg) { return mg ? mg->fused_count : -1; }

extern "C" int pmg_multigrid_set_precision(pmg_multigrid mg, int precision)
{
  PMG_REQUIRE(mg, "pmg_multigrid_set_precision: NULL argument");
  PMG_REQUIRE(precision == PMG_PRECISION_FP64 || precision == PMG_PRECISION_FP32,
              "pmg_multigrid_set_precision: unknown precision %d (PMG_PRECISION_FP64 or PMG_PRECISION_FP32)", precision);
  if (precision == PMG_PRECISION_FP32)
  {
    for (int i = 0; i < mg->L; ++i)
      PMG_REQUIRE(!mg->mats[i],
                  "pmg_multigrid_set_precision: level %d has an assembled matrix and there is no FP32 matrix "
                  "(pmg_multigrid_set_level_matrix(mg, %d, NULL) removes it)", i, i);
    PMG_TRY(mg_check_f32(mg, "pmg_multigrid_set_precision"));
  }
  drop_graphs(mg);
  mg->precision = precision;
  return PMG_OK;
}

extern "C" int pmg_multigrid_set_level_matrix(pmg_multigrid mg, int level, pmg_matrix M)
{
  PMG_REQUIRE(mg, "pmg_multigrid_set_level_matrix: NULL argument");
  PMG_REQUIRE(level >= 0 && level < mg->L, "pmg_multigrid_set_level_matrix: level %d of %d", level, mg->L);
  if (M)
  {
    PMG_REQUIRE(matrix_layout(M) == mg->layouts[level],
                "pmg_multigrid_set_level_matrix: the matrix is not on level %d's layout", level);
    PMG_REQUIRE(mg->precision != PMG_PRECISION_FP32,
                "pmg_multigrid_set_level_matrix: the cycle runs in FP32 and there is no FP32 matrix "
                "(pmg_multigrid_set_precision(mg, PMG_PRECISION_FP64) first)");
  }
  drop_graphs(mg);
  mg->mats[level] = M;
  return PMG_OK;
}

extern "C" int pmg_multigrid_precision(pmg_multigrid mg) { return mg ? mg->precision : PMG_ERR_INVALID; }

extern "C" long long pmg_multigrid_graph_replays(pmg_multigrid mg) { return mg ? mg->graph_replays : -1; }

extern "C" int pmg_multigrid_apply(pmg_multigrid mg, const double* rhs, double* y, double* rnorm,
                                   pmg_stream stream)
{
  PMG_REQUIRE(mg && rhs && y, "pmg_multigrid_apply: NULL argument");
  hipStream_t s = S(stream);
  bool done = false;
  if (use_graph(mg))
    PMG_TRY(mg_apply_graph(mg, rhs, y, false, s, &done));
  if (!done)
    PMG_TRY(mg_apply(mg, rhs, y, false, s));
  if (rnorm)
  {
    const int L = mg->L;
    pmg_chebyshev sm = mg->smoothers[L - 1];
    if (mg->mats[L - 1])
      PMG_TRY(matrix_apply(mg->mats[L - 1], y, sm->q, s));
    else
      PMG_TRY(laplacian_apply(mg->ops[L - 1], y, sm->q, s));
    launch_axpy(mg->layouts[L - 1]->size_local, sm->r, -1.0, sm->q, rhs, s);
    double v;
    PMG_TRY(dot_host(mg->layouts[L - 1], sm->r, sm->r, &v, s));
    *rnorm = std::sqrt(v);
  }
  return PMG_OK;
}

extern "C" int pmg_multigrid_apply_counts(pmg_multigrid mg, int* counts, int capacity)
{
  PMG_REQUIRE(mg && counts, "pmg_multigrid_apply_counts: NULL argument");
  for (int i = 0; i < mg->L && i < capacity; ++i)
    counts[i] = mg->counts[i];
  return mg->L;
}
```

pmg-dolfinx_amd/csrc/stiffness_column.hpp:

```cpp

template <int P>
struct Shape
{
  static constexpr int ND = P + 1;
  static constexpr int N = ND * ND * ND;
  static constexpr PatchShape PS = patch_shape(P);
  static constexpr int K = PS.bx * PS.by * PS.bz;
  static constexpr int MAXM = PS.max_m;
  static constexpr int NQ2 = ND * ND;
  static constexpr bool SHARED_ITEM = P == 5 || P == 8;
  static constexpr int CW = P == 5 ? 7 : P == 8 ? 3 : (NQ2 <= 64 ? 64 / NQ2 : 1);
  static constexpr int WPC = SHARED_ITEM ? 4 : (NQ2 + 63) / 64;
  static_assert(CW * NQ2 <= 64 * WPC, "an item's columns need a lane each");
  static constexpr int ITEMS = (K + CW - 1) / CW;
  static constexpr int NWMAX = (P == 3 || P == 5 || P == 6 || P == 8) ? 4 : 8;
  static constexpr int NG = ITEMS < NWMAX / WPC ? ITEMS : NWMAX / WPC;
  static constexpr int NW = NG * WPC;
  static constexpr int WTHREADS = NW * 64;
  static constexpr int WITER = (MAXM + WTHREADS - 1) / WTHREADS;
  static_assert(MAXM <= 65535, "patch positions are 16-bit");
};

template <int ITER, int THREADS>
__device__ __forceinline__ void patch_list_reload(uint32_t (&mk)[ITER], const uint32_t* __restrict__ pd, int M, int t)
{
#pragma unroll
  for (int k = 0; k < ITER; ++k)
  {
    const int i = t + k * THREADS;
    mk[k] = pd[i < M ? i : M - 1];
  }
}
template <int ITER, int THREADS, bool NT>
__device__ __forceinline__ void patch_write_back(const uint32_t (&mk)[ITER], int M, int t, const double* sy,
                                                 const double* __restrict__ x, double* __restrict__ y, int atomic_out)
{
  bool bc_row = false;
#pragma unroll
  for (int k = 0; k < ITER; ++k)
  {
    const int i = t + k * THREADS;
    const uint32_t dof = mk[k] & PD_MASK;
    const bool mine = i < M;
    if (mine && !(mk[k] & PD_BC))
    {
      const double v = sy[i];
      if (atomic_out)
        atomicAdd(&y[dof], v);
      else if constexpr (NT)
        __builtin_nontemporal_store(v, &y[dof]);
      else
        y[dof] = v;
    }
    bc_row |= mine && (mk[k] & (PD_BC | PD_ACC)) == PD_BC;
  }
  if (__builtin_amdgcn_ballot_w64(bc_row) != 0)
  {
#pragma unroll
    for (int k = 0; k < ITER; ++k)
    {
      const int i = t + k * THREADS;
      if (i < M && (mk[k] & (PD_BC | PD_ACC)) == PD_BC)
        y[mk[k] & PD_MASK] = x[mk[k] & PD_MASK];
    }
  }
}

#ifdef PMG_STAMPS
__device__ unsigned long long* g_stamp_buffer = nullptr;
__device__ int g_stamp_capacity = 0;
#define PMG_STAMP_DECL unsigned long long stamp_[8] = {0, 0, 0, 0, 0, 0, 0, 0}
#define PMG_STAMP(i)                                                                                                  \
  do                                                                                                                  \
  {                                                                                                                   \
    __builtin_amdgcn_sched_barrier(0);                                                                                \
    stamp_[i] = __builtin_amdgcn_s_memrealtime();                                                                     \
    __builtin_amdgcn_sched_barrier(0);                                                                                \
  } while (0)
#define PMG_STAMP_FLUSH(nwaves)                                                                                       \
  do                                                                                                                  \
  {                                                                                                                   \
    asm volatile("s_waitcnt vmcnt(0)" ::: "memory");             \
    PMG_STAMP(7);                                                                                                     \
    if ((threadIdx.x & 63) == 0 && g_stamp_buffer && (int)blockIdx.x < g_stamp_capacity)                              \
      for (int i_ = 0; i_ < 8; ++i_)                                                                                  \
        g_stamp_buffer[((size_t)blockIdx.x * (nwaves) + (threadIdx.x >> 6)) * 8 + i_] = stamp_[i_];                   \
  } while (0)
#else
#define PMG_STAMP_DECL
#define PMG_STAMP(i)
#define PMG_STAMP_FLUSH(nwaves)
#endif

constexpr bool unpaired_slice_reads(int P) { return P == 5 || P == 8; }

constexpr bool list_in_lds(int P) { return P == 5 || P == 7 || P == 8; }
constexpr bool transposes_by_identity(int P) { return P == 5; }
template <int P>
constexpr int min_waves_per_simd()
{
  return P <= 4 ? (2 * Shape<P>::NW + 3) / 4 : transposes_by_identity(P) ? 4 : 1;
}
template <int P, bool AFF, bool NT>
__global__ void __launch_bounds__(Shape<P>::WTHREADS, min_waves_per_simd<P>())
    stiffness_column_kernel(const double* __restrict__ x, double* __restrict__ y,
                            const double2* __restrict__ G, const double* __restrict__ Gaff,
                            const double* __restrict__ W1, const int32_t* __restrict__ poff,
                            const uint32_t* __restrict__ pdofs,
                            const int32_t* __restrict__ lmap_id,
                            const uint16_t* __restrict__ lmaps, const int32_t* __restrict__ pcell,
                            const int32_t* __restrict__ pncell, const double* __restrict__ kappa,
                            const double* __restrict__ Dg, const double* __restrict__ react, int first,
                            int atomic_out)
{
  using Sh = Shape<P>;
  constexpr int ND = Sh::ND, N = Sh::N, K = Sh::K, NQ2 = Sh::NQ2, CW = Sh::CW, NG = Sh::NG, WPC = Sh::WPC;
  constexpr int MAXM = Sh::MAXM, THREADS = Sh::WTHREADS, ITER = Sh::WITER;
  constexpr int WL = CW * NQ2;
  constexpr bool UNPAIRED = unpaired_slice_reads(P);
  constexpr bool SHARED = WPC > 1;
  __shared__ double sD[ND * ND];
  __shared__ double skap[K];
  __shared__ double sx[MAXM];
  __shared__ double sy[MAXM];
  constexpr bool LIST_IN_LDS = list_in_lds(P);
  __shared__ uint32_t sm[LIST_IN_LDS ? MAXM : 1];
  __shared__ double sq[NG * WL];
  __shared__ double sgr[NG * WL];
  __shared__ double sgs[NG * WL];
  constexpr bool FLAT = !AFF && WPC == 1 && gflat(ND);
  constexpr int FL = 3 * WL, NJ = (FL + 63) / 64, LS = gls(ND);
  __shared__ double2 sgb[FLAT ? NG * NJ * 64 : 1];

  PMG_STAMP_DECL;
  PMG_STAMP(0);
  const int p = first + blockIdx.x;
  const int t = threadIdx.x;
  const int off = poff[p];
  const int M = poff[p + 1] - off;
  const int table = lmap_id[p];
  const int nc = pncell[p];

  {
    uint32_t m[ITER];
#pragma unroll
    for (int k = 0; k < ITER; ++k)
    {
      const int i = t + k * THREADS;
      m[k] = pdofs[off + (i < M ? i : M - 1)];
    }
    const int cellk = pcell[(size_t)p * K + (t < K ? t : K - 1)];
    const double dval = Dg[t < ND * ND ? t : ND * ND - 1];
    double xv[ITER], yv[ITER];
#pragma unroll
    for (int k = 0; k < ITER; ++k)
    {
      const uint32_t dof = m[k] & PD_MASK;
      const bool acc = !atomic_out && (m[k] & (PD_ACC | PD_BC)) == PD_ACC;
      xv[k] = x[dof];
      const double* ya = acc ? (const double*)(y + dof) : react ? (react + dof) : (x + dof);
      yv[k] = *ya;
    }
    const double kapk = kappa[cellk >= 0 ? cellk : 0];
#pragma unroll
    for (int k = 0; k < ITER; ++k)
    {
      const int i = t + k * THREADS;
      if (i < M)
      {
        const bool acc = !atomic_out && (m[k] & (PD_ACC | PD_BC)) == PD_ACC;
        sx[i] = (m[k] & PD_BC) ? 0.0 : xv[k];
        const bool starts = react && !(m[k] & (PD_ACC | PD_BC));
        sy[i] = acc ? yv[k] : starts ? yv[k] * xv[k] : 0.0;
        if constexpr (LIST_IN_LDS)
          sm[i] = m[k];
      }
    }
    if (t < ND * ND)
      sD[t] = dval;
    for (int i = t; i < K; i += THREADS)
      skap[i] = (i == t) ? kapk : kappa[pcell[(size_t)p * K + i] >= 0 ? pcell[(size_t)p * K + i] : 0];
  }
  PMG_STAMP(1);
  lds_barrier();
  PMG_STAMP(2);

  const int wave = (t >> 6) / WPC, lane = (t & 63) + 64 * ((t >> 6) % WPC);
  constexpr bool IDT = transposes_by_identity(P);
  const bool lane_ok = lane < WL;
  const int lw = lane_ok ? lane : WL - 1;
  const int cw = lw / NQ2;
  const int ab = lw - cw * NQ2;
  const int a = ab / ND, b = ab - a * ND;
  LaneTables<double, ND> T;
  T.fill((const __attribute__((address_space(3))) double*)sD, a, b);
  double rho_a = 1.0, irho_a = 1.0, d2a = 0.0, rho_b = 1.0, irho_b = 1.0, d2b = 0.0;
  if constexpr (IDT)
  {
    rho_a = a == 0 ? 1.0 : -sD[a] / sD[a * ND];
    rho_b = b == 0 ? 1.0 : -sD[b] / sD[b * ND];
    irho_a = 1.0 / rho_a;
    irho_b = 1.0 / rho_b;
    d2a = 2.0 * sD[a * ND + a];
    d2b = 2.0 * sD[b * ND + b];
  }
  const double wab = AFF ? W1[a] * W1[b] : 0.0;
  double* q_s = sq + wave * WL + cw * NQ2;
  double* gr_s = sgr + wave * WL + cw * NQ2;
  double* gs_s = sgs + wave * WL + cw * NQ2;
  double* gr_w = gr_s + ab;
  const int items = WPC > 1 ? (((nc + CW - 1) / CW + NG - 1) / NG) * NG : (nc + CW - 1) / CW;

  for (int it = wave; it < items; it += NG)
  {
#ifdef PMG_STAMPS
    if (it >= wave + NG)
      PMG_STAMP(3);
#endif
    const int slot = it * CW + cw;
    const int slotc = slot < K ? slot : K - 1;
    const uint16_t* lmb = lmaps + (size_t)table * (K * N);
    const unsigned lmo = (unsigned)(slotc * N + ab);
    int l[ND];
#pragma unroll
    for (int k = 0; k < ND; ++k)
      l[k] = lmb[lmo + (unsigned)(k * NQ2)];
    TensorStream<double2, ND, WL, AFF, FLAT, LS, NT, 1> gs;
    if constexpr (AFF)
      gs.prime_affine(Gaff + ((size_t)p * K + slotc) * 6, 1.0);
    else if constexpr (FLAT)
      gs.prime_flat(G + (size_t)p * gpatch(ND, K) + (size_t)__builtin_amdgcn_readfirstlane(it) * ND * LS,
                    sgb + wave * (NJ * 64), lane, lw);
    else
      gs.prime(G + (size_t)p * ((long long)K * 3 * N), (unsigned)(slotc * 3 * N + ab));
    const double kap = IDT ? 1.0 : skap[slotc];
    double u[ND], Aq[ND];
    {
      const double kin = IDT ? skap[slotc] : 1.0;
#pragma unroll
      for (int k = 0; k < ND; ++k)
      {
        u[k] = IDT ? kin * sx[l[k]] : sx[l[k]];
        Aq[k] = 0.0;
      }
    }
    unsigned lp[IDT ? (ND + 1) / 2 : 1];
    if constexpr (IDT)
      pack_positions(l, lp);
#pragma unroll
    for (int k = 0; k < ND; ++k)
    {
      double2 g01, g23, g45;
      gs.take(k, AFF ? wab * W1[k] : 0.0, g01, g23, g45);
      double fr, fs, ft;
      layer_forward<ND, UNPAIRED, SHARED>(k, u, T, Dg, q_s, a, b, ab, g01, g23, g45, kap, fr, fs, ft);
      if constexpr (IDT)
      {
        *gr_w = fr * irho_a;
        gs_s[ab] = fs * irho_b;
        slice_sync<SHARED>();
        double sx_ = 0.0, sy_ = 0.0;
#pragma unroll
        for (int mm = 0; mm < ND; ++mm)
        {
          sx_ += T.Da[mm] * slice_load<UNPAIRED>(gr_s[mm * ND + b]);
          sy_ += T.Db[mm] * slice_load<UNPAIRED>(gs_s[a * ND + mm]);
          Aq[mm] += Dg[k * ND + mm] * ft;
        }
        Aq[k] += (d2a * fr + d2b * fs) - (rho_a * sx_ + rho_b * sy_);
        slice_sync<SHARED>();
      }
      else
        layer_backward<ND, UNPAIRED, SHARED>(k, fr, fs, ft, T, Dg, gr_s, gs_s, a, b, ab, Aq);
    }
    const bool contributes = lane_ok && slot < nc;
#pragma unroll
    for (int k = 0; k < ND; ++k)
    {
      const int lk = IDT ? (int)packed_position(lp, k) : l[k];
      const double Ak = Aq[k];
      atomicAdd(&sy[lk], contributes ? Ak : 0.0);
    }
  }
  {
    PMG_STAMP(4);
    int tw = t;
    asm volatile("" : "+v"(tw));
    uint32_t mk[ITER];
    if constexpr (!LIST_IN_LDS)
      patch_list_reload<ITER, THREADS>(mk, pdofs + off, M, tw);
    lds_barrier();
    if constexpr (LIST_IN_LDS)
    {
#pragma unroll
      for (int k = 0; k < ITER; ++k)
        mk[k] = sm[tw + k * THREADS < M ? tw + k * THREADS : M - 1];
    }
    PMG_STAMP(5);
    patch_write_back<ITER, THREADS, NT>(mk, M, tw, sy, x, y, atomic_out);
    PMG_STAMP(6);
    PMG_STAMP_FLUSH(Sh::NW);
  }
}
```

pmg-dolfinx_amd/csrc/vector.hip:

```cpp
#include "common.hpp"

#include <cstdlib>

using namespace pmg;

namespace
{
constexpr int EW_THREADS = 256;
constexpr int EW_MAX_BLOCKS = 256 * 8;

inline int ew_blocks(long long work)
{
  long long b = (work + EW_THREADS - 1) / EW_THREADS;
  if (b < 1)
    b = 1;
  return (int)(b > EW_MAX_BLOCKS ? EW_MAX_BLOCKS : b);
}

inline bool aligned16(const void* p) { return (reinterpret_cast<uintptr_t>(p) & 15u) == 0; }

__global__ void pack_kernel(int n, const int32_t* __restrict__ idx, const double* __restrict__ in,
                            double* __restrict__ out)
{
  for (int i = blockIdx.x * blockDim.x + threadIdx.x; i < n; i += gridDim.x * blockDim.x)
// ... 103 lines not shown

#define D2(p) reinterpret_cast<double2*>(p)
#define CD2(p) reinterpret_cast<const double2*>(p)

template <typename T>
struct SetF
{
  T* x;
  T v;
  __device__ void pair(int i) const { D2(x)[i] = make_double2(v, v); }
  __device__ void one(int i) const { x[i] = v; }
};
struct ScaleF
{
  double* x;
  double a;
  __device__ void pair(int i) const
  {
    double2 t = D2(x)[i];
    t.x *= a;
    t.y *= a;
    D2(x)[i] = t;
  }
  __device__ void one(int i) const { x[i] *= a; }
};
struct CopyF
{
  double* d;
  const double* s;
  __device__ void pair(int i) const { D2(d)[i] = CD2(s)[i]; }
  __device__ void one(int i) const { d[i] = s[i]; }
};
struct AxpyF
{
  double* r;
  double a;
  const double* x;
  const double* y;
  __device__ void pair(int i) const
  {
    double2 vx = CD2(x)[i], vy = CD2(y)[i];
    D2(r)[i] = make_double2(vx.x * a + vy.x, vx.y * a + vy.y);
  }
  __device__ void one(int i) const { r[i] = x[i] * a + y[i]; }
};
struct MulF
{
  double* w;
  const double* x;
  const double* y;
  __device__ void pair(int i) const
  {
    double2 vx = CD2(x)[i], vy = CD2(y)[i];
    D2(w)[i] = make_double2(vx.x * vy.x, vx.y * vy.y);
  }
  __device__ void one(int i) const { w[i] = x[i] * y[i]; }
};
typedef double ntv2 __attribute__((ext_vector_type(2)));
template <bool NT>
__device__ __forceinline__ double2 ld2(const double* p, int i)
{
  if constexpr (NT)
  {
    ntv2 v = __builtin_nontemporal_load(reinterpret_cast<const ntv2*>(p) + i);
    return make_double2(v.x, v.y);
  }
  else
    return CD2(p)[i];
}
template <bool NT>
__device__ __forceinline__ void st2(double* p, int i, double2 v)
{
  if constexpr (NT)
  {
    ntv2 w;
    w.x = v.x;
    w.y = v.y;
    __builtin_nontemporal_store(w, reinterpret_cast<ntv2*>(p) + i);
  }
  else
    D2(p)[i] = v;
}

template <typename T, bool NT>
struct ChebInitF
{
  T* r;
  T* z;
  const T* b;
  const T* q;
  const T* dinv;
  T c0;
  __device__ void pair(int i) const
  {
    double2 vb = ld2<NT>(b, i), vd = ld2<NT>(dinv, i);
    double2 vr = vb;
    if (q)
    {
      double2 vq = ld2<NT>(q, i);
      vr.x -= vq.x;
      vr.y -= vq.y;
    }
    st2<NT>(r, i, vr);
    D2(z)[i] = make_double2(c0 * vd.x * vr.x, c0 * vd.y * vr.y);
  }
  __device__ void one(int i) const
  {
    T vr = b[i] - (q ? q[i] : T(0));
    r[i] = vr;
    z[i] = c0 * dinv[i] * vr;
  }
};
template <typename T, bool NT, bool BOTH>
struct ChebStepF
{
  T* x;
  T* r;
  T* z;
  const T* q;
  const T* dinv;
  T c1, c2;
  int x_final;
  __device__ void pair(int i) const
  {
    double2 vx = ld2<NT>(x, i), vr = ld2<NT>(r, i), vz = D2(z)[i];
    double2 vq = ld2<NT>(q, i), vd = ld2<NT>(dinv, i);
    if constexpr (BOTH)
    {
      vx.x += vz.x;
      vx.y += vz.y;
    }
    vr.x -= vq.x;
    vr.y -= vq.y;
    vz.x = c1 * vz.x + c2 * vd.x * vr.x;
    vz.y = c1 * vz.y + c2 * vd.y * vr.y;
    vx.x += vz.x;
    vx.y += vz.y;
    if (x_final)
      D2(x)[i] = vx;
    else
      st2<NT>(x, i, vx);
    if (x_final != 2)
    {
      st2<NT>(r, i, vr);
      D2(z)[i] = vz;
    }
  }
  __device__ void one(int i) const
  {
    T vz = z[i], vx = x[i];
    if constexpr (BOTH)
      vx += vz;
    T vr = r[i] - q[i];
    vz = c1 * vz + c2 * dinv[i] * vr;
    if (x_final != 2)
    {
      r[i] = vr;
      z[i] = vz;
    }
    x[i] = vx + vz;
  }
};
template <typename T, bool NT>
struct ChebFirstF
{
  T* x;
  T* r;
  T* z;
  const T* q;
  const T* dinv;
  T c1, c2;
  int x_final;
  __device__ void pair(int i) const
  {
    double2 vr = ld2<NT>(r, i), vz = D2(z)[i];
    double2 vq = ld2<NT>(q, i), vd = ld2<NT>(dinv, i);
    double2 vx = vz;
    vr.x -= vq.x;
    vr.y -= vq.y;
    vz.x = c1 * vz.x + c2 * vd.x * vr.x;
    vz.y = c1 * vz.y + c2 * vd.y * vr.y;
    if (x_final)
      D2(x)[i] = make_double2(vx.x + vz.x, vx.y + vz.y);
    else
      st2<NT>(x, i, make_double2(vx.x + vz.x, vx.y + vz.y));
    if (x_final != 2)
    {
      st2<NT>(r, i, vr);
      D2(z)[i] = vz;
    }
  }
  __device__ void one(int i) const
  {
    T vz = z[i];
    const T vx = vz;
    T vr = r[i] - q[i];
    vz = c1 * vz + c2 * dinv[i] * vr;
    if (x_final != 2)
    {
      r[i] = vr;
      z[i] = vz;
    }
    x[i] = vx + vz;
  }
};
template <typename T, bool NT>
struct ChebResidualF
{
  T* r;
  const T* q;
  __device__ void pair(int i) const
  {
    double2 vr = ld2<NT>(r, i), vq = ld2<NT>(q, i);
    D2(r)[i] = make_double2(vr.x - vq.x, vr.y - vq.y);
  }
  __device__ void one(int i) const { r[i] -= q[i]; }
};
template <typename T, bool NT>
struct ChebLastF
{
  T* x;
  T* r;
  const T* z;
  const T* q;
  int assign;
  __device__ void pair(int i) const
  {
    double2 vr = ld2<NT>(r, i), vz = ld2<NT>(z, i), vq = ld2<NT>(q, i);
    double2 vx = assign ? make_double2(0.0, 0.0) : ld2<NT>(x, i);
    D2(x)[i] = make_double2(vx.x + vz.x, vx.y + vz.y);
    st2<NT>(r, i, make_double2(vr.x - vq.x, vr.y - vq.y));
  }
  __device__ void one(int i) const
  {
    x[i] = (assign ? T(0) : x[i]) + z[i];
    r[i] -= q[i];
  }
};
template <typename T, bool NT>
struct AddF
{
  T* x;
  const T* z;
  __device__ void pair(int i) const
  {
    double2 vx = ld2<NT>(x, i), vz = ld2<NT>(z, i);
    D2(x)[i] = make_double2(vx.x + vz.x, vx.y + vz.y);
  }
  __device__ void one(int i) const { x[i] += z[i]; }
};
template <typename T>
struct MaskBcF
{
  T* b;
  const int8_t* bc;
  __device__ void pair(int i) const
  {
    if (bc[2 * i])
      b[2 * i] = T(0);
    if (bc[2 * i + 1])
      b[2 * i + 1] = T(0);
  }
  __device__ void one(int i) const
  {
    if (bc[i])
      b[i] = T(0);
  }
};
struct ToF32
{
  float* out;
  const double *in, *sub;
  __device__ void one(int i) const { out[i] = (float)(sub ? in[i] - sub[i] : in[i]); }
};
struct FromF32
{
  double* out;
  const float* in;
  int add;
  __device__ void one(int i) const { out[i] = (add ? out[i] : 0.0) + (double)in[i]; }
};
struct CgUpdateF
{
  double* x;
  double* r;
  double* y;
  const double* p;
  const double* dinv;
  double rnorm;
  const double* d_py;
  __device__ void pair(int i) const
  {
    const double alpha = rnorm / *d_py;
    double2 vx = D2(x)[i], vr = D2(r)[i], vy = D2(y)[i];
    double2 vp = CD2(p)[i], vd = CD2(dinv)[i];
    vx.x += alpha * vp.x;
    vx.y += alpha * vp.y;
    vr.x -= alpha * vy.x;
    vr.y -= alpha * vy.y;
    D2(x)[i] = vx;
    D2(r)[i] = vr;
    D2(y)[i] = make_double2(vd.x * vr.x, vd.y * vr.y);
  }
  __device__ void one(int i) const
  {
    const double alpha = rnorm / *d_py;
    x[i] += alpha * p[i];
    double vr = r[i] - alpha * y[i];
    r[i] = vr;
    y[i] = dinv[i] * vr;
  }
};
struct CgUpdate2F
{
  double* x;
  double* r;
  const double* p;
  const double* y;
  double rnorm;
// ... 42 lines not shown
__device__ inline double wave_max(double v)
{
  for (int off = 32; off > 0; off >>= 1)
    v = nan_max(v, __shfl_down(v, off, 64));
  return v;
}

template <bool MAX>
__device__ inline double block_reduce(double v)
{
  __shared__ double sm[RED_THREADS / 64];
  v = MAX ? wave_max(v) : wave_sum(v);
  int lane = threadIdx.x & 63, w = threadIdx.x >> 6;
  if (lane == 0)
    sm[w] = v;
  __syncthreads();
  if (w == 0)
  {
    v = lane < RED_THREADS / 64 ? sm[lane] : (MAX ? 0.0 : 0.0);
    v = MAX ? wave_max(v) : wave_sum(v);
  }
  return v;
}

__global__ void dot_partial_kernel(int n, const double* __restrict__ a,
                                   const double* __restrict__ b, double* __restrict__ partials,
                                   int vec)
{
  double acc = 0.0;
  if (vec)
  {
    int n2 = n / 2;
    for (int i = blockIdx.x * blockDim.x + threadIdx.x; i < n2; i += gridDim.x * blockDim.x)
    {
      double2 va = CD2(a)[i], vb = CD2(b)[i];
      acc += va.x * vb.x + va.y * vb.y;
    }
    if ((n & 1) && blockIdx.x == 0 && threadIdx.x == 0)
      acc += a[n - 1] * b[n - 1];
  }
  else
    for (int i = blockIdx.x * blockDim.x + threadIdx.x; i < n; i += gridDim.x * blockDim.x)
      acc += a[i] * b[i];
  acc = block_reduce<false>(acc);
  if (threadIdx.x == 0)
    partials[blockIdx.x] = acc;
}

__global__ void absmax_partial_kernel(int n, const double* __restrict__ a,
                                      double* __restrict__ partials)
{
  double acc = 0.0;
  for (int i = blockIdx.x * blockDim.x + threadIdx.x; i < n; i += gridDim.x * blockDim.x)
    acc = nan_max(acc, fabs(a[i]));
  acc = block_reduce<true>(acc);
  if (threadIdx.x == 0)
    partials[blockIdx.x] = acc;
}

template <bool MAX>
__global__ void fold_kernel(int nb, const double* __restrict__ partials, double* __restrict__ out)
{
  double acc = 0.0;
  for (int i = threadIdx.x; i < nb; i += blockDim.x)
    acc = MAX ? nan_max(acc, partials[i]) : acc + partials[i];
  acc = block_reduce<MAX>(acc);
  if (threadIdx.x == 0)
    out[0] = acc;
}
}

namespace pmg
{
static inline bool streams(int n) { return n >= (4 << 20); }

void launch_axpy(int n, double* r, double alpha, const double* x, const double* y, hipStream_t s)
{
  ew_launch(n, aligned16(r) && aligned16(x) && aligned16(y), AxpyF{r, alpha, x, y}, s);
}
void launch_pointwise(int n, double* w, const double* x, const double* y, hipStream_t s)
{
  ew_launch(n, aligned16(w) && aligned16(x) && aligned16(y), MulF{w, x, y}, s);
}
void launch_cheb_init(int n, double* r, double* z, const double* b, const double* q,
                      const double* dinv, double c0, hipStream_t s, double* clear_q, int n_total)
{
  bool v = aligned16(r) && aligned16(z) && aligned16(b) && aligned16(dinv) && (!q || aligned16(q));
  if (clear_q)
  {
    if (streams(n))
      ew_launch_clear(n, n_total, v, ChebInitF<double, true>{r, z, b, q, dinv, c0}, clear_q, s);
    else
      ew_launch_clear(n, n_total, v, ChebInitF<double, false>{r, z, b, q, dinv, c0}, clear_q, s);
  }
  else if (streams(n))
    ew_launch(n, v, ChebInitF<double, true>{r, z, b, q, dinv, c0}, s);
  else
    ew_launch(n, v, ChebInitF<double, false>{r, z, b, q, dinv, c0}, s);
}
void launch_cheb_step(int n, double* x, double* r, double* z, const double* q, const double* dinv,
                      double c1, double c2, bool both, int x_final, hipStream_t s, double* clear_q, int n_total)
{
  bool v = aligned16(x) && aligned16(r) && aligned16(z) && aligned16(q) && aligned16(dinv);
  const int xf = x_final;
  if (clear_q)
  {
    if (both)
      ew_launch_clear(n, n_total, v, ChebStepF<double, false, true>{x, r, z, q, dinv, c1, c2, xf}, clear_q, s);
    else
      ew_launch_clear(n, n_total, v, ChebStepF<double, false, false>{x, r, z, q, dinv, c1, c2, xf}, clear_q, s);
    return;
  }
  if (streams(n))
  {
    if (both)
      ew_launch(n, v, ChebStepF<double, true, true>{x, r, z, q, dinv, c1, c2, xf}, s);
    else
      ew_launch(n, v, ChebStepF<double, true, false>{x, r, z, q, dinv, c1, c2, xf}, s);
  }
  else if (both)
    ew_launch(n, v, ChebStepF<double, false, true>{x, r, z, q, dinv, c1, c2, xf}, s);
  else
    ew_launch(n, v, ChebStepF<double, false, false>{x, r, z, q, dinv, c1, c2, xf}, s);
}
void launch_cheb_residual(int n, double* r, const double* q, hipStream_t s)
{
  if (streams(n))
    ew_launch(n, aligned16(r) && aligned16(q), ChebResidualF<double, true>{r, q}, s);
  else
    ew_launch(n, aligned16(r) && aligned16(q), ChebResidualF<double, false>{r, q}, s);
}
void launch_cheb_first(int n, double* x, double* r, double* z, const double* q, const double* dinv,
                       double c1, double c2, int x_final, hipStream_t s, double* clear_q, int n_total)
{
  bool v = aligned16(x) && aligned16(r) && aligned16(z) && aligned16(q) && aligned16(dinv);
  const int xf = x_final;
  if (clear_q)
    ew_launch_clear(n, n_total, v, ChebFirstF<double, false>{x, r, z, q, dinv, c1, c2, xf}, clear_q, s);
  else if (streams(n))
    ew_launch(n, v, ChebFirstF<double, true>{x, r, z, q, dinv, c1, c2, xf}, s);
  else
    ew_launch(n, v, ChebFirstF<double, false>{x, r, z, q, dinv, c1, c2, xf}, s);
}
void launch_cheb_last(int n, double* x, double* r, const double* z, const double* q, bool assign,
                      hipStream_t s)
{
  bool v = aligned16(x) && aligned16(r) && aligned16(z) && aligned16(q);
  if (streams(n))
    ew_launch(n, v, ChebLastF<double, true>{x, r, z, q, assign ? 1 : 0}, s);
  else
    ew_launch(n, v, ChebLastF<double, false>{x, r, z, q, assign ? 1 : 0}, s);
}
void launch_add(int n, double* x, const double* z, hipStream_t s)
{
  if (streams(n))
    ew_launch(n, aligned16(x) && aligned16(z), AddF<double, true>{x, z}, s);
  else
    ew_launch(n, aligned16(x) && aligned16(z), AddF<double, false>{x, z}, s);
}
void launch_zero(int n, double* x, hipStream_t s) { ew_launch(n, aligned16(x), SetF<double>{x, 0.0}, s); }
void launch_mask_bc(int n, double* b, const int8_t* bc, hipStream_t s)
{
  ew_launch(n, true, MaskBcF<double>{b, bc}, s);
}
static void refuse_clear_q(const float* clear_q)
{
  if (clear_q)
  {
    std::fprintf(stderr, "pmg_amd: the FP32 smoother passes have no zeroed-output form (clear_q given)\n");
    std::abort();
  }
}
void launch_cheb_init(int n, float* r, float* z, const float* b, const float* q, const float* dinv, float c0,
                      hipStream_t s, float* clear_q, int)
{
  refuse_clear_q(clear_q);
  ew_launch1(n, ChebInitF<float, false>{r, z, b, q, dinv, c0}, s);
}
void launch_cheb_step(int n, float* x, float* r, float* z, const float* q, const float* dinv, float c1, float c2,
                      bool both, int x_final, hipStream_t s, float* clear_q, int)
{
  refuse_clear_q(clear_q);
  if (both)
    ew_launch1(n, ChebStepF<float, false, true>{x, r, z, q, dinv, c1, c2, x_final}, s);
  else
    ew_launch1(n, ChebStepF<float, false, false>{x, r, z, q, dinv, c1, c2, x_final}, s);
}
void launch_cheb_first(int n, float* x, float* r, float* z, const float* q, const float* dinv, float c1, float c2,
                       int x_final, hipStream_t s, float* clear_q, int)
{
  refuse_clear_q(clear_q);
  ew_launch1(n, ChebFirstF<float, false>{x, r, z, q, dinv, c1, c2, x_final}, s);
}
void launch_cheb_residual(int n, float* r, const float* q, hipStream_t s)
{
  ew_launch1(n, ChebResidualF<float, false>{r, q}, s);
}
void launch_cheb_last(int n, float* x, float* r, const float* z, const float* q, bool assign, hipStream_t s)
{
  ew_launch1(n, ChebLastF<float, false>{x, r, z, q, assign ? 1 : 0}, s);
}
void launch_add(int n, float* x, const float* z, hipStream_t s) { ew_launch1(n, AddF<float, false>{x, z}, s); }
void launch_zero(int n, float* x, hipStream_t s) { ew_launch1(n, SetF<float>{x, 0.0f}, s); }
void launch_mask_bc(int n, float* b, const int8_t* bc, hipStream_t s) { ew_launch1(n, MaskBcF<float>{b, bc}, s); }
void launch_to_f32(int n, const double* in, const double* sub, float* out, hipStream_t s)
{
  ew_launch1(n, ToF32{out, in, sub}, s);
}
void launch_from_f32(int n, const float* in, double* out, bool add, hipStream_t s)
{
  ew_launch1(n, FromF32{out, in, add ? 1 : 0}, s);
}

void launch_cg_update(int n, double* x, double* r, double* y, const double* p, const double* dinv,
                      double rnorm, const double* d_py, hipStream_t s)
{
  bool v = aligned16(x) && aligned16(r) && aligned16(y) && aligned16(p) && aligned16(dinv);
  ew_launch(n, v, CgUpdateF{x, r, y, p, dinv, rnorm, d_py}, s);
}
void launch_cg_update2(int n, double* x, double* r, const double* p, const double* y, double rnorm,
                       const double* d_py, hipStream_t s)
{
  bool v = aligned16(x) && aligned16(r) && aligned16(y) && aligned16(p);
  ew_launch(n, v, CgUpdate2F{x, r, p, y, rnorm, d_py}, s);
}
void launch_cg_direction(int n, double* p, const double* y, double rnorm, const double* d_new,
                         const double* d_sub, hipStream_t s)
{
  ew_launch(n, aligned16(p) && aligned16(y), CgDirectionF{p, y, rnorm, d_new, d_sub}, s);
}

double* red_slot(pmg_layout l, int slot) { return l->d_partials + RED_BLOCKS + slot; }

int dot_async(pmg_layout l, const double* a, const double* b, int slot, hipStream_t s)
{
  PMG_REQUIRE(slot >= 0 && slot < RED_SLOTS, "dot_async: bad slot");
  int n = l->size_local;
  int nb = ew_blocks((n + 1) / 2);
  if (nb > RED_BLOCKS)
    nb = RED_BLOCKS;
  int vec = aligned16(a) && aligned16(b);
  dot_partial_kernel<<<nb, RED_THREADS, 0, s>>>(n, a, b, l->d_partials, vec);
  fold_kernel<false><<<1, RED_THREADS, 0, s>>>(nb, l->d_partials, red_slot(l, slot));
  PMG_HIP(hipGetLastError());
  return PMG_OK;
}

int reduce_slots_async(pmg_layout l, int slot, int n, bool max, hipStream_t s)
{
  PMG_REQUIRE(slot >= 0 && n >= 1 && slot + n <= RED_SLOTS, "reduce_slots_async: bad slot range");
  if (l->comm)
    return comm_allreduce(l, red_slot(l, slot), n, max, s);
  pmg_allreduce_fn fn = max ? l->allreduce_max : l->allreduce;
  if (!fn)
    return PMG_OK;
  PMG_HIP(hipMemcpyAsync(l->h_result, red_slot(l, slot), sizeof(double) * n, hipMemcpyDeviceToHost, s));
  PMG_HIP(hipStreamSynchronize(s));
  if (fn(l->user, l->h_result, n) != 0)
    return fail(PMG_ERR_INVALID, "allreduce callback failed");
  PMG_HIP(hipMemcpyAsync(red_slot(l, slot), l->h_result, sizeof(double) * n, hipMemcpyHostToDevice, s));
  PMG_HIP(hipStreamSynchronize(s));
  return PMG_OK;
}

int fetch_slots(pmg_layout l, int slot, int n, double* host_out, hipStream_t s)
{
  PMG_REQUIRE(slot >= 0 && n >= 1 && slot + n <= RED_SLOTS, "fetch_slots: bad slot range");
  PMG_HIP(hipMemcpyAsync(l->h_result, red_slot(l, slot), sizeof(double) * n, hipMemcpyDeviceToHost, s));
  PMG_HIP(hipStreamSynchronize(s));
  for (int i = 0; i < n; ++i)
    host_out[i] = l->h_result[i];
  return PMG_OK;
}

int dot_host(pmg_layout l, const double* a, const double* b, double* result, hipStream_t s)
{
  PMG_TRY(dot_async(l, a, b, 0, s));
  PMG_TRY(reduce_slots_async(l, 0, 1, false, s));
  return fetch_slots(l, 0, 1, result, s);
}
}

// ... 275 lines not shown
```

pmg-dolfinx_amd/laplacian.py:

```python
from __future__ import annotations

import ctypes as C

import numpy as np

from . import _lib
from ._lib import call, current_stream, ptr, vp
from .vector import Layout, Vector


def _dev_i32(a, device):
    import torch

    if hasattr(a, "data_ptr"):
        return a
    return torch.from_numpy(np.ascontiguousarray(a, dtype=np.int32)).to(device)


def _dev_f64(a, device):
    import torch

    if hasattr(a, "data_ptr"):
        return a
    return torch.from_numpy(np.ascontiguousarray(a, dtype=np.float64)).to(device)
# ... 7 lines not shown
    return torch.from_numpy(np.ascontiguousarray(a, dtype=np.int8)).to(device)


NODE_ORDERS = {"ascending": 0, "endpoints_first": 1, "basix": 1, "custom": 2}


def node_order_args(node_order, degree, perm1d=None):
    code = NODE_ORDERS[node_order] if isinstance(node_order, str) else int(node_order)
    perm = None
    if code == 2:
        perm = np.ascontiguousarray(perm1d, dtype=np.int32)
        if perm.size != degree + 1:
            raise ValueError("perm1d needs degree + 1 entries")
    return code, perm


def node_permutation(node_order, degree, perm1d=None):
    code, perm = node_order_args(node_order, degree, perm1d)
    out = np.zeros(degree + 1, dtype=np.int32)
    call("pmg_node_permutation", code, int(degree), perm.ctypes.data_as(_lib.c_ip) if perm is not None else None,
         out.ctypes.data_as(_lib.c_ip))
    return out


def set_merge_threshold(patch_dofs: int):
    call("pmg_set_merge_threshold", int(patch_dofs))


class MatFreeLaplacian:

    value_type = np.float64

    def __init__(self, degree, coefficients, dofmap, xgeom, geometry_dofmap, lcells, bcells, bc_marker,
                 layout: Layout, batch_size: int = 0, node_order="ascending", perm1d=None, dphi_geometry=None,
                 G_weights=None):
        if batch_size != 0:
            raise ValueError("geometry batching is not supported: G is kept resident in HBM")
        dev = layout.device
        self.layout = layout
        self.degree = int(degree)
        N = (self.degree + 1) ** 3
        self.dofmap = _dev_i32(dofmap, dev)
        self.ncells = int(self.dofmap.numel() // N) if self.degree >= 1 else 0
        self.kappa = _dev_f64(np.broadcast_to(np.asarray(coefficients, dtype=np.float64), (self.ncells,)).copy()
                              if not hasattr(coefficients, "data_ptr") else coefficients, dev)
        self.xgeom = _dev_f64(xgeom, dev)
        self.geom_dofmap = _dev_i32(geometry_dofmap, dev)
        self.bc_marker = _dev_i8(bc_marker, dev)
        if self.bc_marker.numel() != layout.total:
            raise ValueError("bc_marker must have size_local + num_ghosts entries")
        lc = np.ascontiguousarray(lcells, dtype=np.int32)
        bc_ = np.ascontiguousarray(bcells, dtype=np.int32)
        h = vp()
        self.node_order, perm = node_order_args(node_order, self.degree, perm1d)
        self.dphi_geometry = _dev_f64(dphi_geometry, dev) if dphi_geometry is not None else None
        self.G_weights = _dev_f64(G_weights, dev) if G_weights is not None else None
        if (self.dphi_geometry is None) != (self.G_weights is None):
            raise ValueError("dphi_geometry and G_weights come together (src/laplacian.hpp:293-294)")
        call("pmg_laplacian_create_ordered", C.byref(h), layout.handle, self.degree, self.ncells, ptr(self.kappa),
             ptr(self.dofmap), ptr(self.xgeom), int(self.xgeom.numel() // 3), ptr(self.geom_dofmap),
             ptr(self.dphi_geometry), ptr(self.G_weights),
             lc.ctypes.data_as(_lib.c_ip), lc.size, bc_.ctypes.data_as(_lib.c_ip), bc_.size, ptr(self.bc_marker),
             self.node_order, perm.ctypes.data_as(_lib.c_ip) if perm is not None else None, current_stream())
        self._handle = h

    @property
    def handle(self):
        return self._handle

    def __call__(self, x: Vector, y: Vector):
        call("pmg_laplacian_apply", self._handle, ptr(x.data), ptr(y.data), current_stream())

    def apply_fp32(self, x, y):
        import torch

        n = self.layout.size_local + self.layout.num_ghosts
        for name, t in (("x", x), ("y", y)):
            if not isinstance(t, torch.Tensor) or t.dtype != torch.float32 or not t.is_contiguous():
                raise TypeError(f"{name} must be a contiguous float32 torch tensor")
            if t.numel() != n:
                raise ValueError(f"{name} has {t.numel()} entries, the layout {n}")
        call("pmg_laplacian_apply_f32", self._handle, vp(x.data_ptr()), vp(y.data_ptr()), current_stream())

    def get_diag_inverse(self, diag_inv: Vector):
        call("pmg_laplacian_get_diag_inverse", self._handle, ptr(diag_inv.data), current_stream())

    def set_diag_inverse(self, diag_inv: Vector):
        call("pmg_laplacian_set_diag_inverse", self._handle, ptr(diag_inv.data), current_stream())

    def compute_diag_inverse(self):
        call("pmg_laplacian_compute_diag_inverse", self._handle, current_stream())

    def set_coefficient_field(self, v):
        if v is None:
            call("pmg_laplacian_set_coefficient_field", self._handle, None, current_stream())
            return
        if not isinstance(v, Vector):
            raise TypeError("set_coefficient_field takes a Vector of the operator's layout, or None")
        n = self.layout.size_local + self.layout.num_ghosts
        if v.data.numel() != n:
            raise ValueError(f"the field has {v.data.numel()} entries, the operator's layout {n}")
        call("pmg_laplacian_set_coefficient_field", self._handle, ptr(v.data), current_stream())

    def has_coefficient_field(self) -> bool:
        return bool(call("pmg_laplacian_has_coefficient_field", self._handle))

    def set_coefficient_tensor(self, t):
        import torch

        if t is None:
            call("pmg_laplacian_set_coefficient_tensor", self._handle, None, current_stream())
            return
        if not isinstance(t, (np.ndarray, torch.Tensor)):
            raise TypeError("set_coefficient_tensor takes a float64 numpy array or torch tensor, or None")
        if t.dtype not in (np.float64, torch.float64):
            raise TypeError(f"the coefficient tensor must be float64, not {t.dtype}")
        if tuple(t.shape) != (self.ncells, 6):
            raise ValueError(f"the coefficient tensor has shape {tuple(t.shape)}, the operator needs "
                             f"({self.ncells}, 6)")
        if isinstance(t, np.ndarray):
            t = torch.from_numpy(np.ascontiguousarray(t))
        t = t.to(self.layout.device).contiguous()
        call("pmg_laplacian_set_coefficient_tensor", self._handle, ptr(t), current_stream())

    def has_coefficient_tensor(self) -> bool:
        return bool(call("pmg_laplacian_has_coefficient_tensor", self._handle))

    def set_reaction(self, sigma):
        import torch

        if sigma is None:
            call("pmg_laplacian_set_reaction", self._handle, None, current_stream())
            return
        if not isinstance(sigma, (np.ndarray, torch.Tensor)):
            raise TypeError("set_reaction takes a float64 numpy array or torch tensor, or None")
        if sigma.dtype not in (np.float64, torch.float64):
            raise TypeError(f"the reaction coefficient must be float64, not {sigma.dtype}")
        if tuple(sigma.shape) != (self.ncells,):
            raise ValueError(f"the reaction coefficient has shape {tuple(sigma.shape)}, the operator needs "
                             f"({self.ncells},)")
        if isinstance(sigma, np.ndarray):
            sigma = torch.from_numpy(np.ascontiguousarray(sigma))
        sigma = sigma.to(self.layout.device).contiguous()
        call("pmg_laplacian_set_reaction", self._handle, ptr(sigma), current_stream())

    def has_reaction(self) -> bool:
        return bool(call("pmg_laplacian_has_reaction", self._handle))

    def geometry(self):
        import torch

        N = (self.degree + 1) ** 3
        out = torch.empty((self.ncells, N, 6), dtype=torch.float64, device=self.layout.device)
        call("pmg_laplacian_get_geometry", self._handle, ptr(out), current_stream())
        return out

    def assemble_rhs(self, f: Vector, b: Vector):
        call("pmg_laplacian_assemble_rhs", self._handle, ptr(f.data), ptr(b.data), current_stream())

    def _boundary_vectors(self, what, g, b, x0):
        n = self.layout.size_local + self.layout.num_ghosts
        for name, v in (("g", g), ("b", b)) + ((("x0", x0),) if x0 is not None else ()):
            if not isinstance(v, Vector):
                raise TypeError(f"{what}: {name} must be a Vector of the operator's layout")
            if v.data.numel() != n:
                raise ValueError(f"{what}: {name} has {v.data.numel()} entries, the operator's layout {n}")
# ... 76 lines not shown
```

pmg-dolfinx_amd/pmg.py:

```python
from __future__ import annotations

import ctypes as C

from . import _lib
from ._lib import call, current_stream, ptr, vp
from .laplacian import _dev_i8
from .vector import Vector


class MultigridPreconditioner:

    def __init__(self, layouts, bc_marker_coarsest, bs: int = 1):
        self.layouts = list(layouts)
        self.bc0 = _dev_i8(bc_marker_coarsest, self.layouts[0].device)
        arr = (vp * len(self.layouts))(*[l.handle for l in self.layouts])
        h = vp()
        call("pmg_multigrid_create", C.byref(h), len(self.layouts), arr, ptr(self.bc0))
        self._handle = h
        self._keep = {}

    @property
    def handle(self):
        return self._handle

    def _set(self, fn, objs, key):
        objs = list(objs)
        self._keep[key] = objs
        arr = (vp * max(len(objs), 1))(*[o.handle for o in objs])
        call(fn, self._handle, arr)

    def set_solvers(self, solvers):
        self._set("pmg_multigrid_set_solvers", solvers, "solvers")

    def set_operators(self, operators):
        self._set("pmg_multigrid_set_operators", operators, "operators")

    def set_interpolators(self, interpolators):
        self._set("pmg_multigrid_set_interpolators", interpolators, "interpolators")

    def set_level_matrix(self, level: int, matrix):
        level = int(level)
        if level < 0:
            level += len(self.layouts)
        call("pmg_multigrid_set_level_matrix", self._handle, level, matrix.handle if matrix is not None else None)
        self._keep.setdefault("matrices", {})[level] = matrix

    def set_coarse_solver(self, solver):
        from .amg import AmgSolver
        from .cg import CGSolver

        self._keep["coarse"] = solver
        if solver is None:
            call("pmg_multigrid_set_coarse_callback", self._handle, _lib.COARSE_FN(), None)
            call("pmg_multigrid_set_coarse_solver", self._handle, None)
            call("pmg_multigrid_set_coarse_amg", self._handle, None)
        elif isinstance(solver, AmgSolver):
            call("pmg_multigrid_set_coarse_amg", self._handle, solver.handle)
        elif isinstance(solver, CGSolver):
            call("pmg_multigrid_set_coarse_solver", self._handle, solver.handle)
        elif hasattr(solver, "solve"):
            cx, cb = Vector(self.layouts[0]), Vector(self.layouts[0])
            lay = self.layouts[0].handle

            def bridge(user, x, b, stream):
                try:
                    call("pmg_vec_copy", lay, ptr(cb.data), vp(b), vp(stream))
                    call("pmg_vec_copy", lay, ptr(cx.data), vp(x), vp(stream))
                    solver.solve(cx, cb)
                    call("pmg_vec_copy", lay, vp(x), ptr(cx.data), vp(stream))
                    return 0
                except Exception:
                    import sys
                    import traceback

                    traceback.print_exc(file=sys.stderr)
                    return 1

            self._keep["coarse_cb"] = _lib.COARSE_FN(bridge)
            self._keep["coarse_vecs"] = (cx, cb)
            call("pmg_multigrid_set_coarse_callback", self._handle, self._keep["coarse_cb"], None)
        else:
            raise TypeError("the coarse solver needs a solve(x, b) method")

    def apply(self, x: Vector, y: Vector, verbose: bool = False):
        if verbose:
            rn = C.c_double()
            call("pmg_multigrid_apply", self._handle, ptr(x.data), ptr(y.data), C.byref(rn), current_stream())
            return rn.value
        call("pmg_multigrid_apply", self._handle, ptr(x.data), ptr(y.data), None, current_stream())
        return None

    def set_graph(self, enable=True):
        call("pmg_multigrid_set_graph", self._handle, -1 if enable is None else (1 if enable else 0))

    def set_fused_restriction(self, mode=None):
        code = -1 if mode is None or mode is True else int(mode)
        call("pmg_multigrid_set_fused_restriction", self._handle, code)

    def fused_restrictions(self) -> int:
        return call("pmg_multigrid_fused_restrictions", self._handle)

    PRECISIONS = {"fp64": 0, "fp32": 1}

    def set_precision(self, precision: str):
        if precision not in self.PRECISIONS:
            raise ValueError(f"precision must be one of {sorted(self.PRECISIONS)}, not {precision!r}")
        call("pmg_multigrid_set_precision", self._handle, self.PRECISIONS[precision])

    @property
    def precision(self) -> str:
        code = call("pmg_multigrid_precision", self._handle)
        return {v: k for k, v in self.PRECISIONS.items()}[code]

    def graph_replays(self) -> int:
        return call("pmg_multigrid_graph_replays", self._handle)

    def apply_counts(self):
        n = len(self.layouts)
        arr = (C.c_int * n)()
        call("pmg_multigrid_apply_counts", self._handle, arr, n)
        return list(arr)

    def __del__(self):
        try:
            if getattr(self, "_handle", None) is not None:
                _lib.lib().pmg_multigrid_destroy(self._handle)
                self._handle = None
        except Exception:
            pass
```

Baseline: 3.656 billion DoF/s.

## Add ordered-output stiffness apply with permuted reads in Chebyshev smoother passes

```diff
diff --git a/include/pmg_amd.h b/include/pmg_amd.h
--- a/include/pmg_amd.h
+++ b/include/pmg_amd.h
@@ -129,6 +129,8 @@
 int pmg_laplacian_destroy(pmg_laplacian op);
 int pmg_laplacian_apply(pmg_laplacian op, double* in, double* out, pmg_stream stream);
 int pmg_laplacian_apply_f32(pmg_laplacian op, float* in, float* out, pmg_stream stream);
+int pmg_laplacian_ordered_output(pmg_laplacian op, long long* n_ordered, int32_t* perm, pmg_stream stream);
+int pmg_laplacian_apply_ordered(pmg_laplacian op, const double* in, double* out_ordered, pmg_stream stream);
 int pmg_laplacian_get_diag_inverse(pmg_laplacian op, double* diag_inv, pmg_stream stream);
 int pmg_laplacian_set_diag_inverse(pmg_laplacian op, const double* diag_inv, pmg_stream stream);
 int pmg_laplacian_compute_diag_inverse(pmg_laplacian op, pmg_stream stream);
@@ -167,6 +169,8 @@
 int pmg_chebyshev_set_max_iterations(pmg_chebyshev s, int max_iter);
 int pmg_chebyshev_solve(pmg_chebyshev s, pmg_laplacian A, double* x, const double* b,
                         pmg_stream stream);
+int pmg_chebyshev_smooth(pmg_chebyshev s, pmg_laplacian A, double* x, const double* b, double* residual,
+                         int x_is_zero, int ordered_output, pmg_stream stream);
 
 int pmg_cg_create(pmg_cg* out, pmg_layout layout);
 int pmg_cg_destroy(pmg_cg s);
@@ -259,6 +263,8 @@
 int pmg_multigrid_apply_counts(pmg_multigrid mg, int* counts, int capacity);
 int pmg_multigrid_set_fused_restriction(pmg_multigrid mg, int mode);
 int pmg_multigrid_fused_restrictions(pmg_multigrid mg);
+int pmg_multigrid_set_ordered_output(pmg_multigrid mg, int mode);
+int pmg_multigrid_ordered_levels(pmg_multigrid mg, pmg_stream stream);
 #define PMG_PRECISION_FP64 0
 #define PMG_PRECISION_FP32 1
 int pmg_multigrid_set_precision(pmg_multigrid mg, int precision);
diff --git a/pmg-dolfinx_amd/_lib.py b/pmg-dolfinx_amd/_lib.py
--- a/pmg-dolfinx_amd/_lib.py
+++ b/pmg-dolfinx_amd/_lib.py
@@ -197,6 +197,11 @@
     "pmg_chebyshev_solve_matrix": (C.c_int, [vp, vp, vp, vp, vp]),
     "pmg_cg_solve_matrix": (C.c_int, [vp, vp, vp, vp, vp, C.POINTER(C.c_int), vp]),
     "pmg_multigrid_set_level_matrix": (C.c_int, [vp, C.c_int, vp]),
+    "pmg_laplacian_ordered_output": (C.c_int, [vp, C.POINTER(C.c_longlong), vp, vp]),
+    "pmg_laplacian_apply_ordered": (C.c_int, [vp, vp, vp, vp]),
+    "pmg_chebyshev_smooth": (C.c_int, [vp, vp, vp, vp, vp, C.c_int, C.c_int, vp]),
+    "pmg_multigrid_set_ordered_output": (C.c_int, [vp, C.c_int]),
+    "pmg_multigrid_ordered_levels": (C.c_int, [vp, vp]),
 }
 
 _COUNT_FUNCS = {"pmg_multigrid_graph_replays", "pmg_amg_num_levels", "pmg_laplacian_geometry_bytes", "pmg_comm_rank", "pmg_comm_size", "pmg_comm_capture_overlaps", "pmg_cg_coefficients", "pmg_cg_compute_eigenvalues", "pmg_multigrid_apply_counts", "pmg_version",
@@ -204,7 +209,8 @@
                 "pmg_laplacian_has_coefficient_field", "pmg_laplacian_has_coefficient_tensor", "pmg_laplacian_has_reaction", "pmg_laplacian_lift_cell_count",
                 "pmg_laplacian_chain_available", "pmg_laplacian_chain_form",
                 "pmg_laplacian_node_order", "pmg_layout_forward_scatters",
-                "pmg_matrix_rows", "pmg_matrix_nnz", "pmg_matrix_bytes", "pmg_multigrid_fused_restrictions"}
+                "pmg_matrix_rows", "pmg_matrix_nnz", "pmg_matrix_bytes", "pmg_multigrid_fused_restrictions",
+                "pmg_multigrid_ordered_levels"}
 
 _lib = None
 
diff --git a/pmg-dolfinx_amd/chebyshev.py b/pmg-dolfinx_amd/chebyshev.py
--- a/pmg-dolfinx_amd/chebyshev.py
+++ b/pmg-dolfinx_amd/chebyshev.py
@@ -28,6 +28,11 @@
         fn = "pmg_chebyshev_solve_matrix" if isinstance(A, MatrixOperator) else "pmg_chebyshev_solve"
         call(fn, self._handle, A.handle, ptr(x.data), ptr(b.data), current_stream())
 
+    def smooth(self, A, x: Vector, b: Vector, residual: Vector = None, x_is_zero: bool = False, ordered=None):
+        code = -1 if ordered is None else (1 if ordered else 0)
+        call("pmg_chebyshev_smooth", self._handle, A.handle, ptr(x.data), ptr(b.data),
+             ptr(residual.data) if residual is not None else None, 1 if x_is_zero else 0, code, current_stream())
+
     def __del__(self):
         try:
             if getattr(self, "_handle", None) is not None:
diff --git a/pmg-dolfinx_amd/csrc/common.hpp b/pmg-dolfinx_amd/csrc/common.hpp
--- a/pmg-dolfinx_amd/csrc/common.hpp
+++ b/pmg-dolfinx_amd/csrc/common.hpp
@@ -208,10 +208,17 @@
   ResidualFused = 3
 };
 template <typename T>
+struct ChebOrdered
+{
+  const int32_t* perm = nullptr;
+  T* q = nullptr;
+  const ApplyFnT<T>* A = nullptr;
+};
+template <typename T>
 int cheb_iterate(const ChebWork<T>& w, const ApplyFnT<T>& A, const T* dinv, int n, double lmax, int max_iter, T* x,
                  const T* b, int need_r, bool x_zero, hipStream_t s, bool* split = nullptr,
                  const ApplyFnT<T>* A_zeroed = nullptr, int n_total = 0, bool track_ghosts = false,
-                 const ApplyFnT<T>* A_first = nullptr);
+                 const ApplyFnT<T>* A_first = nullptr, const ChebOrdered<T>* ord = nullptr);
 
 int dot_async(pmg_layout l, const double* a, const double* b, int slot, hipStream_t s);
 double* red_slot(pmg_layout l, int slot);
@@ -221,25 +228,31 @@
 void launch_axpy(int n, double* r, double alpha, const double* x, const double* y, hipStream_t s);
 void launch_pointwise(int n, double* w, const double* x, const double* y, hipStream_t s);
 void launch_cheb_init(int n, double* r, double* z, const double* b, const double* q, const double* dinv, double c0,
-                      hipStream_t s, double* clear_q = nullptr, int n_total = 0);
+                      hipStream_t s, double* clear_q = nullptr, int n_total = 0, const int32_t* q_perm = nullptr);
 void launch_cheb_step(int n, double* x, double* r, double* z, const double* q, const double* dinv, double c1, double c2,
-                      bool both, int x_final, hipStream_t s, double* clear_q = nullptr, int n_total = 0);
+                      bool both, int x_final, hipStream_t s, double* clear_q = nullptr, int n_total = 0,
+                      const int32_t* q_perm = nullptr);
 void launch_cheb_first(int n, double* x, double* r, double* z, const double* q, const double* dinv, double c1,
-                       double c2, int x_final, hipStream_t s, double* clear_q = nullptr, int n_total = 0);
-void launch_cheb_residual(int n, double* r, const double* q, hipStream_t s);
+                       double c2, int x_final, hipStream_t s, double* clear_q = nullptr, int n_total = 0,
+                       const int32_t* q_perm = nullptr);
+void launch_cheb_residual(int n, double* r, const double* q, hipStream_t s, const int32_t* q_perm = nullptr);
 void launch_add(int n, double* x, const double* z, hipStream_t s);
-void launch_cheb_last(int n, double* x, double* r, const double* z, const double* q, bool assign, hipStream_t s);
+void launch_cheb_last(int n, double* x, double* r, const double* z, const double* q, bool assign, hipStream_t s,
+                      const int32_t* q_perm = nullptr);
 void launch_zero(int n, double* x, hipStream_t s);
 void launch_mask_bc(int n, double* b, const int8_t* bc, hipStream_t s);
 void launch_cheb_init(int n, float* r, float* z, const float* b, const float* q, const float* dinv, float c0,
-                      hipStream_t s, float* clear_q = nullptr, int n_total = 0);
+                      hipStream_t s, float* clear_q = nullptr, int n_total = 0, const int32_t* q_perm = nullptr);
 void launch_cheb_step(int n, float* x, float* r, float* z, const float* q, const float* dinv, float c1, float c2,
-                      bool both, int x_final, hipStream_t s, float* clear_q = nullptr, int n_total = 0);
+                      bool both, int x_final, hipStream_t s, float* clear_q = nullptr, int n_total = 0,
+                      const int32_t* q_perm = nullptr);
 void launch_cheb_first(int n, float* x, float* r, float* z, const float* q, const float* dinv, float c1,
-                       float c2, int x_final, hipStream_t s, float* clear_q = nullptr, int n_total = 0);
-void launch_cheb_residual(int n, float* r, const float* q, hipStream_t s);
+                       float c2, int x_final, hipStream_t s, float* clear_q = nullptr, int n_total = 0,
+                       const int32_t* q_perm = nullptr);
+void launch_cheb_residual(int n, float* r, const float* q, hipStream_t s, const int32_t* q_perm = nullptr);
 void launch_add(int n, float* x, const float* z, hipStream_t s);
-void launch_cheb_last(int n, float* x, float* r, const float* z, const float* q, bool assign, hipStream_t s);
+void launch_cheb_last(int n, float* x, float* r, const float* z, const float* q, bool assign, hipStream_t s,
+                      const int32_t* q_perm = nullptr);
 void launch_zero(int n, float* x, hipStream_t s);
 void launch_mask_bc(int n, float* b, const int8_t* bc, hipStream_t s);
 void launch_cg_update(int n, double* x, double* r, double* y, const double* p, const double* dinv,
@@ -253,6 +266,16 @@
 int laplacian_apply_zeroed(pmg_laplacian op, double* in, double* out, hipStream_t s);
 int laplacian_apply_ghosts_current(pmg_laplacian op, double* in, double* out, hipStream_t s);
 bool laplacian_wants_zeroed_output(pmg_laplacian op);
+struct OrderedOutput
+{
+  const int32_t* perm = nullptr;
+  double* q = nullptr;
+  long long n = 0;
+};
+bool laplacian_offers_ordered_output(pmg_laplacian op);
+int laplacian_ordered_prepare(pmg_laplacian op, hipStream_t s);
+bool laplacian_ordered_output(pmg_laplacian op, OrderedOutput* out);
+int laplacian_apply_ordered(pmg_laplacian op, const double* in, double* out_ordered, hipStream_t s);
 const double* laplacian_diag_inv(pmg_laplacian op);
 const double* laplacian_reaction(pmg_laplacian op);
 pmg_layout laplacian_layout(pmg_laplacian op);
diff --git a/pmg-dolfinx_amd/csrc/laplacian.hip b/pmg-dolfinx_amd/csrc/laplacian.hip
--- a/pmg-dolfinx_amd/csrc/laplacian.hip
+++ b/pmg-dolfinx_amd/csrc/laplacian.hip
@@ -1,4 +1,5 @@
 #include "laplacian.hpp"
+#include "output_order.hpp"
 #include "stiffness_layer.hpp"
 
 #include <algorithm>
@@ -85,6 +86,25 @@
   });
   op->launches++;
   return PMG_OK;
+}
+
+template <int P>
+int launch_stiffness_ordered(pmg_laplacian op, const double* x, double* y, int first, int count, hipStream_t s)
+{
+  if constexpr (P <= ORDERED_MAX_DEGREE)
+  {
+    auto launch = [&](auto nt) {
+      stiffness_column_kernel<P, false, decltype(nt)::value, true, const uint32_t*>
+          <<<count, Shape<P>::WTHREADS, 0, s>>>(
+          x, y, op->G, op->Gaff, op->W1, op->poff, op->pdofs, op->lmap_id, op->lmaps, op->pcell, op->pncell, op->kappa,
+          op->D, nullptr, first, 0, (const uint32_t*)op->qpos);
+    };
+    (P >= NT_FROM && op->stream_policy) ? launch(std::true_type{}) : launch(std::false_type{});
+    op->launches++;
+    return PMG_OK;
+  }
+  else
+    return fail(PMG_ERR_INVALID, "internal: ordered form at degree %d", P);
 }
 
 static int launch_chains(pmg_laplacian op, const double* x, double* y, int first, int count, hipStream_t s)
@@ -277,6 +297,75 @@
 int laplacian_apply_zeroed(pmg_laplacian op, double* in, double* out, hipStream_t s)
 {
   return apply_impl(op, in, out, laplacian_wants_zeroed_output(op), s);
+}
+
+bool laplacian_offers_ordered_output(pmg_laplacian op)
+{
+  const ApplyForm f = apply_form(op);
+  return op->order_offered && op->geometry_mode == 0 && op->batch_patches == 0 && !op->react && !f.chains
+         && !f.two_streams;
+}
+
+int laplacian_ordered_prepare(pmg_laplacian op, hipStream_t s)
+{
+  if (!op->order_offered || op->qpos)
+    return PMG_OK;
+  hipStreamCaptureStatus cap = hipStreamCaptureStatusNone;
+  PMG_HIP(hipStreamIsCapturing(s, &cap));
+  if (cap != hipStreamCaptureStatusNone)
+    return PMG_OK;
+  PatchPlan plan;
+  plan.npatch = op->npatch;
+  plan.launch_first = op->launch_first;
+  plan.launch_count = op->launch_count;
+  plan.n_launch_l = op->n_launch_l;
+  plan.n_plain = op->n_plain;
+  plan.launch_stream = op->launch_stream;
+  plan.bzero.assign(op->n_bzero, 0);
+  plan.poff.resize((size_t)op->npatch + 1);
+  plan.pdofs.resize((size_t)op->npdofs);
+  PMG_HIP(hipMemcpyAsync(plan.poff.data(), op->poff, sizeof(int32_t) * plan.poff.size(), hipMemcpyDeviceToHost, s));
+  PMG_HIP(hipMemcpyAsync(plan.pdofs.data(), op->pdofs, sizeof(uint32_t) * plan.pdofs.size(), hipMemcpyDeviceToHost, s));
+  PMG_HIP(hipStreamSynchronize(s));
+  OutputOrder oo;
+  PMG_TRY(build_output_order(oo, plan, op->layout->total()));
+  if (!oo.ok)
+  {
+    op->order_offered = false;
+    return PMG_OK;
+  }
+  PMG_TRY(upload(&op->qpos, oo.qpos.data(), oo.qpos.size(), s));
+  PMG_TRY(upload(&op->order_perm, oo.perm.data(), oo.perm.size(), s));
+  PMG_HIP(hipMalloc(&op->q_ordered, sizeof(double) * (size_t)oo.n_ordered));
+  PMG_HIP(hipMemsetAsync(op->q_ordered, 0, sizeof(double) * (size_t)oo.n_ordered, s));
+  op->n_ordered = oo.n_ordered;
+  PMG_HIP(hipStreamSynchronize(s));
+  return PMG_OK;
+}
+
+bool laplacian_ordered_output(pmg_laplacian op, OrderedOutput* out)
+{
+  if (!op->qpos || !laplacian_offers_ordered_output(op))
+    return false;
+  *out = OrderedOutput{op->order_perm, op->q_ordered, op->n_ordered};
+  return true;
+}
+
+int laplacian_apply_ordered(pmg_laplacian op, const double* in, double* out_ordered, hipStream_t s)
+{
+  PMG_REQUIRE(op->qpos && laplacian_offers_ordered_output(op),
+              "laplacian_apply_ordered: the ordered form is not available on this operator");
+  PMG_TRY(walk_launches(op, 0, (int)op->launch_first.size(), apply_form(op), s,
+                        [&](const LaunchStep& st, hipStream_t sl) {
+                          PMG_REQUIRE(st.kind == LaunchStep::PATCHES && !st.atomic_out,
+                                      "internal: the ordered form met a launch that is not a coloured patch launch");
+                          return with_degree(op->P, [&](auto P) {
+                            return launch_stiffness_ordered<decltype(P)::value>(op, in, out_ordered, st.first,
+                                                                                st.count, sl);
+                          });
+                        }));
+  op->applies++;
+  return PMG_OK;
 }
 }
 
@@ -466,6 +555,8 @@
       touched[v & PD_MASK] = 1;
     for (int i = 0; i < total && !op->needs_zero; ++i)
       op->needs_zero = !touched[i];
+    op->order_offered = plan_offers_output_order(plan) && !op->needs_zero && layout->num_ghosts == 0
+                        && degree <= ORDERED_MAX_DEGREE && total > 0;
   }
   op->npatch = plan.npatch;
   op->pcell_h = plan.pcell;
@@ -584,6 +675,9 @@
   (void)hipFree(op->chain_off);
   (void)hipFree(op->chain_patch);
   (void)hipFree(op->diag_inv);
+  (void)hipFree(op->qpos);
+  (void)hipFree(op->order_perm);
+  (void)hipFree(op->q_ordered);
   (void)hipFree(op->G32);
   (void)hipFree(op->D32);
   (void)hipFree(op->diag32);
@@ -635,6 +729,34 @@
   PMG_REQUIRE(op && in && out, "pmg_laplacian_apply: NULL argument");
   PMG_REQUIRE(in != out, "pmg_laplacian_apply: in and out alias");
   return laplacian_apply(op, in, out, S(stream));
+}
+
+extern "C" int pmg_laplacian_ordered_output(pmg_laplacian op, long long* n_ordered, int32_t* perm, pmg_stream stream)
+{
+  PMG_REQUIRE(op && n_ordered, "pmg_laplacian_ordered_output: NULL argument");
+  PMG_TRY(laplacian_ordered_prepare(op, S(stream)));
+  OrderedOutput oo;
+  if (!laplacian_ordered_output(op, &oo))
+  {
+    *n_ordered = 0;
+    return PMG_OK;
+  }
+  *n_ordered = oo.n;
+  if (perm)
+    PMG_HIP(hipMemcpyAsync(perm, oo.perm, sizeof(int32_t) * op->layout->total(), hipMemcpyDeviceToDevice, S(stream)));
+  return PMG_OK;
+}
+
+extern "C" int pmg_laplacian_apply_ordered(pmg_laplacian op, const double* in, double* out_ordered, pmg_stream stream)
+{
+  PMG_REQUIRE(op && in && out_ordered, "pmg_laplacian_apply_ordered: NULL argument");
+  PMG_REQUIRE(in != out_ordered, "pmg_laplacian_apply_ordered: in and out alias");
+  PMG_TRY(laplacian_ordered_prepare(op, S(stream)));
+  PMG_REQUIRE(op->qpos && laplacian_offers_ordered_output(op),
+              "pmg_laplacian_apply_ordered: this operator does not offer the ordered output (coloured interior "
+              "launches only, no ghosts, stored resident geometry, no reaction term, no chains, one stream, degree <= "
+              "%d)", ORDERED_MAX_DEGREE);
+  return laplacian_apply_ordered(op, in, out_ordered, S(stream));
 }
 
 extern "C" int pmg_laplacian_get_diag_inverse(pmg_laplacian op, double* diag_inv,
diff --git a/pmg-dolfinx_amd/csrc/laplacian.hpp b/pmg-dolfinx_amd/csrc/laplacian.hpp
--- a/pmg-dolfinx_amd/csrc/laplacian.hpp
+++ b/pmg-dolfinx_amd/csrc/laplacian.hpp
@@ -58,6 +58,11 @@
   int32_t* chain_off = nullptr;
   int32_t* chain_patch = nullptr;
   std::vector<int32_t> chain_first, chain_count;
+  bool order_offered = false;
+  uint32_t* qpos = nullptr;
+  int32_t* order_perm = nullptr;
+  double* q_ordered = nullptr;
+  long long n_ordered = 0;
   bool stream_policy = true;
   bool stream_policy32 = false;
   double* diag_inv = nullptr;
diff --git a/pmg-dolfinx_amd/csrc/output_order.hpp b/pmg-dolfinx_amd/csrc/output_order.hpp
--- /dev/null
+++ b/pmg-dolfinx_amd/csrc/output_order.hpp
@@ -0,0 +1,67 @@
+#pragma once
+
+#include "patches.hpp"
+
+namespace pmg
+{
+constexpr int ORDER_ALIGN = 16;
+
+struct OutputOrder
+{
+  bool ok = false;
+  std::vector<int32_t> qoff;
+  std::vector<uint32_t> qpos;
+  std::vector<int32_t> perm;
+  long long n_ordered = 0;
+};
+
+inline bool plan_offers_output_order(const PatchPlan& plan)
+{
+  const int nl = (int)plan.launch_first.size();
+  return plan.n_plain > 1 && plan.n_plain == nl && plan.n_launch_l == nl && plan.bzero.empty()
+         && plan.launch_stream.empty() && plan.npatch > 0;
+}
+
+inline int build_output_order(OutputOrder& oo, const PatchPlan& plan, int32_t ndofs)
+{
+  oo = OutputOrder();
+  if (!plan_offers_output_order(plan) || ndofs <= 0)
+    return PMG_OK;
+  const int np = plan.npatch;
+  oo.qoff.assign(np, 0);
+  oo.qpos.assign(plan.pdofs.size(), 0u);
+  oo.perm.assign(ndofs, -1);
+  long long cursor = 0;
+  for (int p = 0; p < np; ++p)
+  {
+    cursor = (cursor + ORDER_ALIGN - 1) / ORDER_ALIGN * ORDER_ALIGN;
+    if (cursor + (plan.poff[p + 1] - plan.poff[p]) > (long long)PD_MASK)
+      return PMG_OK;
+    oo.qoff[p] = (int32_t)cursor;
+    for (int e = plan.poff[p]; e < plan.poff[p + 1]; ++e)
+    {
+      const uint32_t v = plan.pdofs[e];
+      if (v & PD_ACC)
+        continue;
+      const uint32_t d = v & PD_MASK;
+      if (d >= (uint32_t)ndofs || oo.perm[d] >= 0)
+        return PMG_OK;
+      oo.perm[d] = (int32_t)cursor;
+      oo.qpos[e] = (uint32_t)cursor | (v & ~PD_MASK);
+      ++cursor;
+    }
+  }
+  for (int32_t d = 0; d < ndofs; ++d)
+    if (oo.perm[d] < 0)
+      return PMG_OK;
+  for (size_t e = 0; e < plan.pdofs.size(); ++e)
+  {
+    const uint32_t v = plan.pdofs[e];
+    if (v & PD_ACC)
+      oo.qpos[e] = (uint32_t)oo.perm[v & PD_MASK] | (v & ~PD_MASK);
+  }
+  oo.n_ordered = (cursor + ORDER_ALIGN - 1) / ORDER_ALIGN * ORDER_ALIGN;
+  oo.ok = true;
+  return PMG_OK;
+}
+}
diff --git a/pmg-dolfinx_amd/csrc/solvers.hip b/pmg-dolfinx_amd/csrc/solvers.hip
--- a/pmg-dolfinx_amd/csrc/solvers.hip
+++ b/pmg-dolfinx_amd/csrc/solvers.hip
@@ -60,6 +60,7 @@
   long long graph_replays = 0;
   int fused_mode = -1;
   int fused_count = 0;
+  int ordered_mode = -1;
   int precision = PMG_PRECISION_FP64;
   std::vector<float*> u32, b32;
   std::vector<ChebWork<float>> w32;
@@ -72,13 +73,17 @@
 template <typename T>
 int cheb_iterate(const ChebWork<T>& w, const ApplyFnT<T>& A, const T* dinv, int n, double lmax, int max_iter, T* x,
                  const T* b, int need_r, bool x_zero, hipStream_t s, bool* split, const ApplyFnT<T>* A_zeroed,
-                 int n_total, bool track_ghosts, const ApplyFnT<T>* A_first)
+                 int n_total, bool track_ghosts, const ApplyFnT<T>* A_first, const ChebOrdered<T>* ord)
 {
   PMG_REQUIRE(sizeof(T) == 8 || !A_zeroed, "cheb_iterate: the FP32 passes have no zeroed-output form");
+  PMG_REQUIRE(!ord || (sizeof(T) == 8 && !A_zeroed && n_total <= n && ord->perm && ord->q && ord->A),
+              "cheb_iterate: the ordered output is FP64, without a zeroed-output form and without ghosts");
   if (split)
     *split = false;
+  T* const q = ord ? ord->q : w.q;
+  const int32_t* const q_perm = ord ? ord->perm : nullptr;
   T* const clear_q = A_zeroed ? w.q : nullptr;
-  const ApplyFnT<T>& An = A_zeroed ? *A_zeroed : A;
+  const ApplyFnT<T>& An = ord ? *ord->A : A_zeroed ? *A_zeroed : A;
   const T c0 = (T)(4.0 / (3.0 * lmax));
   const int ng = track_ghosts && n_total > n ? n_total - n : 0;
   if (x_zero)
@@ -89,8 +94,8 @@
   }
   else
   {
-    PMG_TRY(A_first ? (*A_first)(x, w.q) : A(x, w.q));
-    launch_cheb_init(n, w.r, w.z, b, w.q, dinv, c0, s, clear_q, n_total);
+    PMG_TRY(ord ? (*ord->A)(x, q) : A_first ? (*A_first)(x, q) : A(x, q));
+    launch_cheb_init(n, w.r, w.z, b, q, dinv, c0, s, clear_q, n_total, q_perm);
   }
   for (int i = 1; i <= max_iter; ++i)
   {
@@ -111,26 +116,32 @@
       *split = true;
       break;
     }
-    PMG_TRY(An(w.z, w.q));
+    if (last && need_r == ResidualSplit && split && max_iter > 1)
+    {
+      PMG_TRY((A_zeroed ? *A_zeroed : A)(w.z, w.q));
+      if (ng > 0)
+        launch_add(ng, x + n, w.z + n, s);
+      *split = true;
+      break;
+    }
+    PMG_TRY(An(w.z, q));
     if (ng > 0)
       launch_add(ng, x + n, w.z + n, s);
     if (last)
     {
       if (max_iter == 1)
-        launch_cheb_last(n, x, w.r, w.z, w.q, x_zero, s);
-      else if (need_r == ResidualSplit && split)
-        *split = true;
+        launch_cheb_last(n, x, w.r, w.z, q, x_zero, s, q_perm);
       else
-        launch_cheb_residual(n, w.r, w.q, s);
+        launch_cheb_residual(n, w.r, q, s, q_perm);
       break;
     }
     const T c1 = (T)((2.0 * i - 1.0) / (2.0 * i + 3.0));
     const T c2 = (T)((8.0 * i + 4.0) / (2.0 * i + 3.0) / lmax);
     const int x_final = (i + 1 == max_iter) ? (need_r == ResidualNone ? 2 : 1) : 0;
     if (x_zero && i == 1)
-      launch_cheb_first(n, x, w.r, w.z, w.q, dinv, c1, c2, x_final, s, clear_q, n_total);
+      launch_cheb_first(n, x, w.r, w.z, q, dinv, c1, c2, x_final, s, clear_q, n_total, q_perm);
     else
-      launch_cheb_step(n, x, w.r, w.z, w.q, dinv, c1, c2, i == 1, x_final, s, clear_q, n_total);
+      launch_cheb_step(n, x, w.r, w.z, q, dinv, c1, c2, i == 1, x_final, s, clear_q, n_total, q_perm);
   }
   if (max_iter == 0 && x_zero)
     launch_zero(n, x, s);
@@ -139,10 +150,10 @@
 }
 template int cheb_iterate<double>(const ChebWork<double>&, const ApplyFnT<double>&, const double*, int, double, int,
                                   double*, const double*, int, bool, hipStream_t, bool*, const ApplyFnT<double>*, int,
-                                  bool, const ApplyFnT<double>*);
+                                  bool, const ApplyFnT<double>*, const ChebOrdered<double>*);
 template int cheb_iterate<float>(const ChebWork<float>&, const ApplyFnT<float>&, const float*, int, double, int, float*,
                                  const float*, int, bool, hipStream_t, bool*, const ApplyFnT<float>*, int, bool,
-                                 const ApplyFnT<float>*);
+                                 const ApplyFnT<float>*, const ChebOrdered<float>*);
 }
 
 namespace
@@ -161,19 +172,41 @@
   return PMG_OK;
 }
 
+bool ordered_by_default(pmg_laplacian)
+{
+  if (const char* e = std::getenv("PMG_ORDERED_OUTPUT"))
+    return e[0] != '0';
+  return false;
+}
+
+int ordered_output_of(pmg_laplacian A, int ordered, hipStream_t s, OrderedOutput* oo)
+{
+  *oo = OrderedOutput();
+  if (ordered == 0 || !laplacian_offers_ordered_output(A) || (ordered < 0 && !ordered_by_default(A)))
+    return PMG_OK;
+  PMG_TRY(laplacian_ordered_prepare(A, s));
+  if (!laplacian_ordered_output(A, oo))
+    *oo = OrderedOutput();
+  return PMG_OK;
+}
+
 int cheb_solve(pmg_chebyshev sm, pmg_laplacian A, double* x, const double* b, int need_r,
                bool x_zero, hipStream_t s, bool* split = nullptr, bool track_ghosts = false,
-               bool x_ghosts_current = false)
+               bool x_ghosts_current = false, int ordered = -1)
 {
   pmg_layout l = sm->layout;
   PMG_REQUIRE(laplacian_layout(A) == l, "Chebyshev: operator and smoother layouts differ");
   const ChebWork<double> w{sm->r, sm->z, sm->q};
+  OrderedOutput oo;
+  PMG_TRY(ordered_output_of(A, ordered, s, &oo));
+  const ApplyFn apply_ordered = [A, s](double* in, double* out) { return laplacian_apply_ordered(A, in, out, s); };
+  const ChebOrdered<double> ord{oo.perm, oo.q, &apply_ordered};
   const ApplyFn apply = [A, s](double* in, double* out) { return laplacian_apply(A, in, out, s); };
   const ApplyFn apply_zeroed = [A, s](double* in, double* out) { return laplacian_apply_zeroed(A, in, out, s); };
   const ApplyFn apply_local = [A, s](double* in, double* out) { return laplacian_apply_ghosts_current(A, in, out, s); };
   return cheb_iterate(w, apply, laplacian_diag_inv(A), l->size_local, sm->eig_max, sm->max_iter, x, b, need_r, x_zero,
                       s, split, laplacian_wants_zeroed_output(A) ? &apply_zeroed : nullptr, l->total(), track_ghosts,
-                      x_ghosts_current ? &apply_local : nullptr);
+                      x_ghosts_current ? &apply_local : nullptr, oo.q ? &ord : nullptr);
 }
 
 int cheb_solve_matrix(pmg_chebyshev sm, pmg_matrix M, double* x, const double* b, int need_r, bool x_zero,
@@ -212,7 +245,8 @@
 {
   if (mg->mats[i])
     return cheb_solve_matrix(mg->smoothers[i], mg->mats[i], x, b, need_r, x_zero, s, split, &mg->mat_applies[i]);
-  return cheb_solve(mg->smoothers[i], mg->ops[i], x, b, need_r, x_zero, s, split, track_ghosts, x_ghosts_current);
+  return cheb_solve(mg->smoothers[i], mg->ops[i], x, b, need_r, x_zero, s, split, track_ghosts, x_ghosts_current,
+                    mg->ordered_mode);
 }
 
 long long level_applies(pmg_multigrid mg, int i) { return laplacian_launches(mg->ops[i]) + mg->mat_applies[i]; }
@@ -489,6 +523,20 @@
 {
   PMG_REQUIRE(sm && A && x && b, "pmg_chebyshev_solve: NULL argument");
   return cheb_solve(sm, A, x, b, ResidualNone, false, S(stream));
+}
+
+extern "C" int pmg_chebyshev_smooth(pmg_chebyshev sm, pmg_laplacian A, double* x, const double* b, double* residual,
+                                    int x_is_zero, int ordered_output, pmg_stream stream)
+{
+  PMG_REQUIRE(sm && A && x && b, "pmg_chebyshev_smooth: NULL argument");
+  PMG_REQUIRE(ordered_output >= -1 && ordered_output <= 1,
+              "pmg_chebyshev_smooth: ordered_output %d (-1 automatic, 0 never, 1 wherever offered)", ordered_output);
+  PMG_TRY(cheb_solve(sm, A, x, b, residual ? ResidualUpdated : ResidualNone, x_is_zero != 0, S(stream), nullptr, false,
+                     false, ordered_output));
+  if (residual)
+    PMG_HIP(hipMemcpyAsync(residual, sm->r, sizeof(double) * sm->layout->size_local, hipMemcpyDeviceToDevice,
+                           S(stream)));
+  return PMG_OK;
 }
 
 extern "C" int pmg_chebyshev_solve_matrix(pmg_chebyshev sm, pmg_matrix M, double* x, const double* b,
@@ -903,6 +951,7 @@
     return -1;
   mix((uint64_t)mg->precision);
   mix((uint64_t)(mg->fused_mode + 1));
+  mix((uint64_t)(mg->ordered_mode + 1));
   if (mg->precision == PMG_PRECISION_FP32)
     for (int i = 0; i < mg->L; ++i)
       mix((uint64_t)laplacian_diag_version(mg->ops[i]));
@@ -937,6 +986,13 @@
     }
   if (mg->precision == PMG_PRECISION_FP32)
     PMG_TRY(mg_prepare_f32(mg, s));
+  else
+    for (int i = 0; i < mg->L; ++i)
+      if (!mg->mats[i])
+      {
+        OrderedOutput oo;
+        PMG_TRY(ordered_output_of(mg->ops[i], mg->ordered_mode, s, &oo));
+      }
   if (!mg->capture_stream)
     PMG_HIP(hipStreamCreateWithFlags(&mg->capture_stream, hipStreamNonBlocking));
   PMG_HIP(hipStreamBeginCapture(mg->capture_stream, hipStreamCaptureModeRelaxed));
@@ -985,6 +1041,32 @@
 
 extern "C" int pmg_multigrid_fused_restrictions(pmg_multigrid mg) { return mg ? mg->fused_count : -1; }
 
+extern "C" int pmg_multigrid_set_ordered_output(pmg_multigrid mg, int mode)
+{
+  PMG_REQUIRE(mg, "pmg_multigrid_set_ordered_output: NULL argument");
+  PMG_REQUIRE(mode >= -1 && mode <= 1,
+              "pmg_multigrid_set_ordered_output: mode %d (-1 automatic, 0 never, 1 wherever offered)", mode);
+  drop_graphs(mg);
+  mg->ordered_mode = mode;
+  return PMG_OK;
+}
+
+extern "C" int pmg_multigrid_ordered_levels(pmg_multigrid mg, pmg_stream stream)
+{
+  if (!mg || (int)mg->ops.size() != mg->L)
+    return -1;
+  int n = 0;
+  for (int i = 0; i < mg->L && mg->precision == PMG_PRECISION_FP64; ++i)
+    if (!mg->mats[i])
+    {
+      OrderedOutput oo;
+      if (ordered_output_of(mg->ops[i], mg->ordered_mode, S(stream), &oo) != PMG_OK)
+        return -1;
+      n += oo.q != nullptr;
+    }
+  return n;
+}
+
 extern "C" int pmg_multigrid_set_precision(pmg_multigrid mg, int precision)
 {
   PMG_REQUIRE(mg, "pmg_multigrid_set_precision: NULL argument");
diff --git a/pmg-dolfinx_amd/csrc/stiffness_column.hpp b/pmg-dolfinx_amd/csrc/stiffness_column.hpp
--- a/pmg-dolfinx_amd/csrc/stiffness_column.hpp
+++ b/pmg-dolfinx_amd/csrc/stiffness_column.hpp
@@ -31,9 +31,10 @@
     mk[k] = pd[i < M ? i : M - 1];
   }
 }
-template <int ITER, int THREADS, bool NT>
+template <int ITER, int THREADS, bool NT, bool ORD = false>
 __device__ __forceinline__ void patch_write_back(const uint32_t (&mk)[ITER], int M, int t, const double* sy,
-                                                 const double* __restrict__ x, double* __restrict__ y, int atomic_out)
+                                                 const double* __restrict__ x, double* __restrict__ y, int atomic_out,
+                                                 const uint32_t* __restrict__ pd = nullptr)
 {
   bool bc_row = false;
 #pragma unroll
@@ -61,7 +62,7 @@
     {
       const int i = t + k * THREADS;
       if (i < M && (mk[k] & (PD_BC | PD_ACC)) == PD_BC)
-        y[mk[k] & PD_MASK] = x[mk[k] & PD_MASK];
+        y[mk[k] & PD_MASK] = x[(ORD ? pd[i] : mk[k]) & PD_MASK];
     }
   }
 }
@@ -101,7 +102,10 @@
 {
   return P <= 4 ? (2 * Shape<P>::NW + 3) / 4 : transposes_by_identity(P) ? 4 : 1;
 }
-template <int P, bool AFF, bool NT>
+constexpr int ORDERED_MAX_DEGREE = 4;
+__device__ __forceinline__ const uint32_t* ordered_positions() { return nullptr; }
+__device__ __forceinline__ const uint32_t* ordered_positions(const uint32_t* qpos) { return qpos; }
+template <int P, bool AFF, bool NT, bool ORD = false, typename... QPOS>
 __global__ void __launch_bounds__(Shape<P>::WTHREADS, min_waves_per_simd<P>())
     stiffness_column_kernel(const double* __restrict__ x, double* __restrict__ y,
                             const double2* __restrict__ G, const double* __restrict__ Gaff,
@@ -111,9 +115,12 @@
                             const uint16_t* __restrict__ lmaps, const int32_t* __restrict__ pcell,
                             const int32_t* __restrict__ pncell, const double* __restrict__ kappa,
                             const double* __restrict__ Dg, const double* __restrict__ react, int first,
-                            int atomic_out)
+                            int atomic_out, QPOS... ordered)
 {
   using Sh = Shape<P>;
+  static_assert(sizeof...(QPOS) == (ORD ? 1 : 0), "qpos is the ordered form's argument, and only its");
+  [[maybe_unused]] const uint32_t* __restrict__ const qpos = ordered_positions(ordered...);
+  static_assert(!ORD || !list_in_lds(P), "the ordered form re-reads its positions from global memory");
   constexpr int ND = Sh::ND, N = Sh::N, K = Sh::K, NQ2 = Sh::NQ2, CW = Sh::CW, NG = Sh::NG, WPC = Sh::WPC;
   constexpr int MAXM = Sh::MAXM, THREADS = Sh::WTHREADS, ITER = Sh::WITER;
   constexpr int WL = CW * NQ2;
@@ -149,6 +156,16 @@
       const int i = t + k * THREADS;
       m[k] = pdofs[off + (i < M ? i : M - 1)];
     }
+    [[maybe_unused]] uint32_t mq[ORD ? ITER : 1];
+    if constexpr (ORD)
+    {
+#pragma unroll
+      for (int k = 0; k < ITER; ++k)
+      {
+        const int i = t + k * THREADS;
+        mq[k] = qpos[off + (i < M ? i : M - 1)];
+      }
+    }
     const int cellk = pcell[(size_t)p * K + (t < K ? t : K - 1)];
     const double dval = Dg[t < ND * ND ? t : ND * ND - 1];
     double xv[ITER], yv[ITER];
@@ -158,7 +175,11 @@
       const uint32_t dof = m[k] & PD_MASK;
       const bool acc = !atomic_out && (m[k] & (PD_ACC | PD_BC)) == PD_ACC;
       xv[k] = x[dof];
-      const double* ya = acc ? (const double*)(y + dof) : react ? (react + dof) : (x + dof);
+      const double* ya;
+      if constexpr (ORD)
+        ya = acc ? (const double*)(y + (mq[k] & PD_MASK)) : (x + dof);
+      else
+        ya = acc ? (const double*)(y + dof) : react ? (react + dof) : (x + dof);
       yv[k] = *ya;
     }
     const double kapk = kappa[cellk >= 0 ? cellk : 0];
@@ -287,7 +308,9 @@
     int tw = t;
     asm volatile("" : "+v"(tw));
     uint32_t mk[ITER];
-    if constexpr (!LIST_IN_LDS)
+    if constexpr (ORD)
+      patch_list_reload<ITER, THREADS>(mk, qpos + off, M, tw);
+    else if constexpr (!LIST_IN_LDS)
       patch_list_reload<ITER, THREADS>(mk, pdofs + off, M, tw);
     lds_barrier();
     if constexpr (LIST_IN_LDS)
@@ -297,7 +320,10 @@
         mk[k] = sm[tw + k * THREADS < M ? tw + k * THREADS : M - 1];
     }
     PMG_STAMP(5);
-    patch_write_back<ITER, THREADS, NT>(mk, M, tw, sy, x, y, atomic_out);
+    if constexpr (ORD)
+      patch_write_back<ITER, THREADS, NT, true>(mk, M, tw, sy, x, y, 0, pdofs + off);
+    else
+      patch_write_back<ITER, THREADS, NT>(mk, M, tw, sy, x, y, atomic_out);
     PMG_STAMP(6);
     PMG_STAMP_FLUSH(Sh::NW);
   }
diff --git a/pmg-dolfinx_amd/csrc/vector.hip b/pmg-dolfinx_amd/csrc/vector.hip
--- a/pmg-dolfinx_amd/csrc/vector.hip
+++ b/pmg-dolfinx_amd/csrc/vector.hip
@@ -209,7 +209,44 @@
     D2(p)[i] = v;
 }
 
-template <typename T, bool NT>
+template <bool ORD>
+struct QOrder
+{
+};
+template <>
+struct QOrder<true>
+{
+  const int32_t* perm;
+};
+typedef int nti2 __attribute__((ext_vector_type(2)));
+template <bool NT, bool ORD>
+__device__ __forceinline__ double2 ldq2(const double* q, QOrder<ORD> o, int i)
+{
+  if constexpr (ORD)
+  {
+    nti2 p;
+    if constexpr (NT)
+      p = __builtin_nontemporal_load(reinterpret_cast<const nti2*>(o.perm) + i);
+    else
+      p = reinterpret_cast<const nti2*>(o.perm)[i];
+    if constexpr (NT)
+      return make_double2(__builtin_nontemporal_load(q + p.x), __builtin_nontemporal_load(q + p.y));
+    else
+      return make_double2(q[p.x], q[p.y]);
+  }
+  else
+    return ld2<NT>(q, i);
+}
+template <typename T, bool ORD>
+__device__ __forceinline__ T ldq1(const T* q, QOrder<ORD> o, int i)
+{
+  if constexpr (ORD)
+    return q[o.perm[i]];
+  else
+    return q[i];
+}
+
+template <typename T, bool NT, bool ORD = false>
 struct ChebInitF
 {
   T* r;
@@ -218,13 +255,14 @@
   const T* q;
   const T* dinv;
   T c0;
+  [[no_unique_address]] QOrder<ORD> qo;
   __device__ void pair(int i) const
   {
     double2 vb = ld2<NT>(b, i), vd = ld2<NT>(dinv, i);
     double2 vr = vb;
     if (q)
     {
-      double2 vq = ld2<NT>(q, i);
+      double2 vq = ldq2<NT>(q, qo, i);
       vr.x -= vq.x;
       vr.y -= vq.y;
     }
@@ -233,12 +271,12 @@
   }
   __device__ void one(int i) const
   {
-    T vr = b[i] - (q ? q[i] : T(0));
+    T vr = b[i] - (q ? ldq1(q, qo, i) : T(0));
     r[i] = vr;
     z[i] = c0 * dinv[i] * vr;
   }
 };
-template <typename T, bool NT, bool BOTH>
+template <typename T, bool NT, bool BOTH, bool ORD = false>
 struct ChebStepF
 {
   T* x;
@@ -248,10 +286,11 @@
   const T* dinv;
   T c1, c2;
   int x_final;
+  [[no_unique_address]] QOrder<ORD> qo;
   __device__ void pair(int i) const
   {
     double2 vx = ld2<NT>(x, i), vr = ld2<NT>(r, i), vz = D2(z)[i];
-    double2 vq = ld2<NT>(q, i), vd = ld2<NT>(dinv, i);
+    double2 vq = ldq2<NT>(q, qo, i), vd = ld2<NT>(dinv, i);
     if constexpr (BOTH)
     {
       vx.x += vz.x;
@@ -278,7 +317,7 @@
     T vz = z[i], vx = x[i];
     if constexpr (BOTH)
       vx += vz;
-    T vr = r[i] - q[i];
+    T vr = r[i] - ldq1(q, qo, i);
     vz = c1 * vz + c2 * dinv[i] * vr;
     if (x_final != 2)
     {
@@ -288,7 +327,7 @@
     x[i] = vx + vz;
   }
 };
-template <typename T, bool NT>
+template <typename T, bool NT, bool ORD = false>
 struct ChebFirstF
 {
   T* x;
@@ -298,10 +337,11 @@
   const T* dinv;
   T c1, c2;
   int x_final;
+  [[no_unique_address]] QOrder<ORD> qo;
   __device__ void pair(int i) const
   {
     double2 vr = ld2<NT>(r, i), vz = D2(z)[i];
-    double2 vq = ld2<NT>(q, i), vd = ld2<NT>(dinv, i);
+    double2 vq = ldq2<NT>(q, qo, i), vd = ld2<NT>(dinv, i);
     double2 vx = vz;
     vr.x -= vq.x;
     vr.y -= vq.y;
@@ -321,7 +361,7 @@
   {
     T vz = z[i];
     const T vx = vz;
-    T vr = r[i] - q[i];
+    T vr = r[i] - ldq1(q, qo, i);
     vz = c1 * vz + c2 * dinv[i] * vr;
     if (x_final != 2)
     {
@@ -331,19 +371,20 @@
     x[i] = vx + vz;
   }
 };
-template <typename T, bool NT>
+template <typename T, bool NT, bool ORD = false>
 struct ChebResidualF
 {
   T* r;
   const T* q;
-  __device__ void pair(int i) const
-  {
-    double2 vr = ld2<NT>(r, i), vq = ld2<NT>(q, i);
+  [[no_unique_address]] QOrder<ORD> qo;
+  __device__ void pair(int i) const
+  {
+    double2 vr = ld2<NT>(r, i), vq = ldq2<NT>(q, qo, i);
     D2(r)[i] = make_double2(vr.x - vq.x, vr.y - vq.y);
   }
-  __device__ void one(int i) const { r[i] -= q[i]; }
-};
-template <typename T, bool NT>
+  __device__ void one(int i) const { r[i] -= ldq1(q, qo, i); }
+};
+template <typename T, bool NT, bool ORD = false>
 struct ChebLastF
 {
   T* x;
@@ -351,9 +392,10 @@
   const T* z;
   const T* q;
   int assign;
-  __device__ void pair(int i) const
-  {
-    double2 vr = ld2<NT>(r, i), vz = ld2<NT>(z, i), vq = ld2<NT>(q, i);
+  [[no_unique_address]] QOrder<ORD> qo;
+  __device__ void pair(int i) const
+  {
+    double2 vr = ld2<NT>(r, i), vz = ld2<NT>(z, i), vq = ldq2<NT>(q, qo, i);
     double2 vx = assign ? make_double2(0.0, 0.0) : ld2<NT>(x, i);
     D2(x)[i] = make_double2(vx.x + vz.x, vx.y + vz.y);
     st2<NT>(r, i, make_double2(vr.x - vq.x, vr.y - vq.y));
@@ -361,7 +403,7 @@
   __device__ void one(int i) const
   {
     x[i] = (assign ? T(0) : x[i]) + z[i];
-    r[i] -= q[i];
+    r[i] -= ldq1(q, qo, i);
   }
 };
 template <typename T, bool NT>
@@ -570,11 +612,20 @@
 {
   ew_launch(n, aligned16(w) && aligned16(x) && aligned16(y), MulF{w, x, y}, s);
 }
+static inline bool aligned8(const void* p) { return (reinterpret_cast<uintptr_t>(p) & 7u) == 0; }
 void launch_cheb_init(int n, double* r, double* z, const double* b, const double* q,
-                      const double* dinv, double c0, hipStream_t s, double* clear_q, int n_total)
+                      const double* dinv, double c0, hipStream_t s, double* clear_q, int n_total, const int32_t* q_perm)
 {
   bool v = aligned16(r) && aligned16(z) && aligned16(b) && aligned16(dinv) && (!q || aligned16(q));
-  if (clear_q)
+  if (q && q_perm)
+  {
+    v = aligned16(r) && aligned16(z) && aligned16(b) && aligned16(dinv) && aligned8(q_perm);
+    if (streams(n))
+      ew_launch(n, v, ChebInitF<double, true, true>{r, z, b, q, dinv, c0, {q_perm}}, s);
+    else
+      ew_launch(n, v, ChebInitF<double, false, true>{r, z, b, q, dinv, c0, {q_perm}}, s);
+  }
+  else if (clear_q)
   {
     if (streams(n))
       ew_launch_clear(n, n_total, v, ChebInitF<double, true>{r, z, b, q, dinv, c0}, clear_q, s);
@@ -587,10 +638,27 @@
     ew_launch(n, v, ChebInitF<double, false>{r, z, b, q, dinv, c0}, s);
 }
 void launch_cheb_step(int n, double* x, double* r, double* z, const double* q, const double* dinv,
-                      double c1, double c2, bool both, int x_final, hipStream_t s, double* clear_q, int n_total)
+                      double c1, double c2, bool both, int x_final, hipStream_t s, double* clear_q, int n_total,
+                      const int32_t* q_perm)
 {
   bool v = aligned16(x) && aligned16(r) && aligned16(z) && aligned16(q) && aligned16(dinv);
   const int xf = x_final;
+  if (q_perm)
+  {
+    v = aligned16(x) && aligned16(r) && aligned16(z) && aligned16(dinv) && aligned8(q_perm);
+    if (streams(n))
+    {
+      if (both)
+        ew_launch(n, v, ChebStepF<double, true, true, true>{x, r, z, q, dinv, c1, c2, xf, {q_perm}}, s);
+      else
+        ew_launch(n, v, ChebStepF<double, true, false, true>{x, r, z, q, dinv, c1, c2, xf, {q_perm}}, s);
+    }
+    else if (both)
+      ew_launch(n, v, ChebStepF<double, false, true, true>{x, r, z, q, dinv, c1, c2, xf, {q_perm}}, s);
+    else
+      ew_launch(n, v, ChebStepF<double, false, false, true>{x, r, z, q, dinv, c1, c2, xf, {q_perm}}, s);
+    return;
+  }
   if (clear_q)
   {
     if (both)
@@ -611,19 +679,35 @@
   else
     ew_launch(n, v, ChebStepF<double, false, false>{x, r, z, q, dinv, c1, c2, xf}, s);
 }
-void launch_cheb_residual(int n, double* r, const double* q, hipStream_t s)
-{
-  if (streams(n))
+void launch_cheb_residual(int n, double* r, const double* q, hipStream_t s, const int32_t* q_perm)
+{
+  if (q_perm)
+  {
+    if (streams(n))
+      ew_launch(n, aligned16(r) && aligned8(q_perm), ChebResidualF<double, true, true>{r, q, {q_perm}}, s);
+    else
+      ew_launch(n, aligned16(r) && aligned8(q_perm), ChebResidualF<double, false, true>{r, q, {q_perm}}, s);
+  }
+  else if (streams(n))
     ew_launch(n, aligned16(r) && aligned16(q), ChebResidualF<double, true>{r, q}, s);
   else
     ew_launch(n, aligned16(r) && aligned16(q), ChebResidualF<double, false>{r, q}, s);
 }
 void launch_cheb_first(int n, double* x, double* r, double* z, const double* q, const double* dinv,
-                       double c1, double c2, int x_final, hipStream_t s, double* clear_q, int n_total)
+                       double c1, double c2, int x_final, hipStream_t s, double* clear_q, int n_total,
+                       const int32_t* q_perm)
 {
   bool v = aligned16(x) && aligned16(r) && aligned16(z) && aligned16(q) && aligned16(dinv);
   const int xf = x_final;
-  if (clear_q)
+  if (q_perm)
+  {
+    v = aligned16(x) && aligned16(r) && aligned16(z) && aligned16(dinv) && aligned8(q_perm);
+    if (streams(n))
+      ew_launch(n, v, ChebFirstF<double, true, true>{x, r, z, q, dinv, c1, c2, xf, {q_perm}}, s);
+    else
+      ew_launch(n, v, ChebFirstF<double, false, true>{x, r, z, q, dinv, c1, c2, xf, {q_perm}}, s);
+  }
+  else if (clear_q)
     ew_launch_clear(n, n_total, v, ChebFirstF<double, false>{x, r, z, q, dinv, c1, c2, xf}, clear_q, s);
   else if (streams(n))
     ew_launch(n, v, ChebFirstF<double, true>{x, r, z, q, dinv, c1, c2, xf}, s);
@@ -631,10 +715,18 @@
     ew_launch(n, v, ChebFirstF<double, false>{x, r, z, q, dinv, c1, c2, xf}, s);
 }
 void launch_cheb_last(int n, double* x, double* r, const double* z, const double* q, bool assign,
-                      hipStream_t s)
+                      hipStream_t s, const int32_t* q_perm)
 {
   bool v = aligned16(x) && aligned16(r) && aligned16(z) && aligned16(q);
-  if (streams(n))
+  if (q_perm)
+  {
+    v = aligned16(x) && aligned16(r) && aligned16(z) && aligned8(q_perm);
+    if (streams(n))
+      ew_launch(n, v, ChebLastF<double, true, true>{x, r, z, q, assign ? 1 : 0, {q_perm}}, s);
+    else
+      ew_launch(n, v, ChebLastF<double, false, true>{x, r, z, q, assign ? 1 : 0, {q_perm}}, s);
+  }
+  else if (streams(n))
     ew_launch(n, v, ChebLastF<double, true>{x, r, z, q, assign ? 1 : 0}, s);
   else
     ew_launch(n, v, ChebLastF<double, false>{x, r, z, q, assign ? 1 : 0}, s);
@@ -651,41 +743,45 @@
 {
   ew_launch(n, true, MaskBcF<double>{b, bc}, s);
 }
-static void refuse_clear_q(const float* clear_q)
-{
-  if (clear_q)
-  {
-    std::fprintf(stderr, "pmg_amd: the FP32 smoother passes have no zeroed-output form (clear_q given)\n");
+static void refuse_clear_q(const float* clear_q, const int32_t* q_perm = nullptr)
+{
+  if (clear_q || q_perm)
+  {
+    std::fprintf(stderr, "pmg_amd: the FP32 smoother passes have no zeroed-output and no ordered form (%s given)\n",
+                 clear_q ? "clear_q" : "q_perm");
     std::abort();
   }
 }
 void launch_cheb_init(int n, float* r, float* z, const float* b, const float* q, const float* dinv, float c0,
-                      hipStream_t s, float* clear_q, int)
-{
-  refuse_clear_q(clear_q);
+                      hipStream_t s, float* clear_q, int, const int32_t* q_perm)
+{
+  refuse_clear_q(clear_q, q_perm);
   ew_launch1(n, ChebInitF<float, false>{r, z, b, q, dinv, c0}, s);
 }
 void launch_cheb_step(int n, float* x, float* r, float* z, const float* q, const float* dinv, float c1, float c2,
-                      bool both, int x_final, hipStream_t s, float* clear_q, int)
-{
-  refuse_clear_q(clear_q);
+                      bool both, int x_final, hipStream_t s, float* clear_q, int, const int32_t* q_perm)
+{
+  refuse_clear_q(clear_q, q_perm);
   if (both)
     ew_launch1(n, ChebStepF<float, false, true>{x, r, z, q, dinv, c1, c2, x_final}, s);
   else
     ew_launch1(n, ChebStepF<float, false, false>{x, r, z, q, dinv, c1, c2, x_final}, s);
 }
 void launch_cheb_first(int n, float* x, float* r, float* z, const float* q, const float* dinv, float c1, float c2,
-                       int x_final, hipStream_t s, float* clear_q, int)
-{
-  refuse_clear_q(clear_q);
+                       int x_final, hipStream_t s, float* clear_q, int, const int32_t* q_perm)
+{
+  refuse_clear_q(clear_q, q_perm);
   ew_launch1(n, ChebFirstF<float, false>{x, r, z, q, dinv, c1, c2, x_final}, s);
 }
-void launch_cheb_residual(int n, float* r, const float* q, hipStream_t s)
-{
+void launch_cheb_residual(int n, float* r, const float* q, hipStream_t s, const int32_t* q_perm)
+{
+  refuse_clear_q(nullptr, q_perm);
   ew_launch1(n, ChebResidualF<float, false>{r, q}, s);
 }
-void launch_cheb_last(int n, float* x, float* r, const float* z, const float* q, bool assign, hipStream_t s)
-{
+void launch_cheb_last(int n, float* x, float* r, const float* z, const float* q, bool assign, hipStream_t s,
+                      const int32_t* q_perm)
+{
+  refuse_clear_q(nullptr, q_perm);
   ew_launch1(n, ChebLastF<float, false>{x, r, z, q, assign ? 1 : 0}, s);
 }
 void launch_add(int n, float* x, const float* z, hipStream_t s) { ew_launch1(n, AddF<float, false>{x, z}, s); }
diff --git a/pmg-dolfinx_amd/laplacian.py b/pmg-dolfinx_amd/laplacian.py
--- a/pmg-dolfinx_amd/laplacian.py
+++ b/pmg-dolfinx_amd/laplacian.py
@@ -113,6 +113,26 @@
                 raise ValueError(f"{name} has {t.numel()} entries, the layout {n}")
         call("pmg_laplacian_apply_f32", self._handle, vp(x.data_ptr()), vp(y.data_ptr()), current_stream())
 
+    def ordered_output(self):
+        import torch
+
+        n = C.c_longlong()
+        perm = torch.empty(self.layout.size_local, dtype=torch.int32, device=self.kappa.device)
+        call("pmg_laplacian_ordered_output", self._handle, C.byref(n), vp(perm.data_ptr()), current_stream())
+        return (int(n.value), perm) if n.value > 0 else None
+
+    def apply_ordered(self, x: Vector, q):
+        import torch
+
+        order = self.ordered_output()
+        if order is None:
+            raise _lib.PmgError("this operator does not offer the ordered output")
+        if not isinstance(q, torch.Tensor) or q.dtype != torch.float64 or not q.is_contiguous():
+            raise TypeError("q must be a contiguous float64 torch tensor")
+        if q.numel() != order[0]:
+            raise ValueError(f"q has {q.numel()} entries, the ordered vector {order[0]}")
+        call("pmg_laplacian_apply_ordered", self._handle, ptr(x.data), vp(q.data_ptr()), current_stream())
+
     def get_diag_inverse(self, diag_inv: Vector):
         call("pmg_laplacian_get_diag_inverse", self._handle, ptr(diag_inv.data), current_stream())
 
diff --git a/pmg-dolfinx_amd/pmg.py b/pmg-dolfinx_amd/pmg.py
--- a/pmg-dolfinx_amd/pmg.py
+++ b/pmg-dolfinx_amd/pmg.py
@@ -100,6 +100,13 @@
     def fused_restrictions(self) -> int:
         return call("pmg_multigrid_fused_restrictions", self._handle)
 
+    def set_ordered_output(self, mode=None):
+        code = -1 if mode is None else int(mode)
+        call("pmg_multigrid_set_ordered_output", self._handle, code)
+
+    def ordered_levels(self) -> int:
+        return call("pmg_multigrid_ordered_levels", self._handle, current_stream())
+
     PRECISIONS = {"fp64": 0, "fp32": 1}
 
     def set_precision(self, precision: str):
```

Result: slower. 3.550 billion DoF/s (-2.9%).
